# oraclefina/MSPI

Hardware: AMD Instinct MI355X
Metric: clips_per_sec (higher is better)
Workload: dtype f32 storage/accumulate; GEMMs as f16x3 split products on the f16 MFMA pipe; 1 GPU; x3dl motion encoder + ConvNeXt-T + ResNet18 audio + SyncBlock + decoder (AudioVisualSaliencyModel forward), batch 8/GPU, clips 3x16x224x224, spectrogram 1x257x300, inputs resident in HBM; global_batch=8, launch=hipGraph replay (mspi_amd.runtime.GraphPipeline), 2 batches in flight, stream_layout=2, parallelism=single GPU

## Files before the change

### mspi_amd/_lib.py

```python
import ctypes as C
import os

_HERE = os.path.dirname(os.path.abspath(__file__))
LIB_PATH = os.environ.get("MSPI_LIB_PATH") or os.path.join(_HERE, "csrc", "libmspi_hip.so")

ACT_NONE, ACT_RELU, ACT_GELU, ACT_SIGMOID, ACT_SWISH = range(5)
PREC_F32, PREC_F16X3 = 0, 1


class MspiError(RuntimeError):
    pass


class ConvDesc(C.Structure):
    _fields_ = [
        ("N", C.c_int32), ("T", C.c_int32), ("H", C.c_int32), ("W", C.c_int32), ("C", C.c_int32),
        ("sN", C.c_int64), ("sT", C.c_int64), ("sH", C.c_int64), ("sW", C.c_int64), ("sC", C.c_int64),
        ("kT", C.c_int32), ("kH", C.c_int32), ("kW", C.c_int32),
        ("strT", C.c_int32), ("strH", C.c_int32), ("strW", C.c_int32),
        ("padT", C.c_int32), ("padH", C.c_int32), ("padW", C.c_int32),
        ("To", C.c_int32), ("Ho", C.c_int32), ("Wo", C.c_int32),
        ("Cout", C.c_int32),
        ("ldy", C.c_int64), ("ldw", C.c_int64), ("ldr", C.c_int64),
        ("act", C.c_int32),
        ("prec", C.c_int32),
        ("w_scale", C.c_float),
        ("tile", C.c_int32),
        ("w_blocked", C.c_void_p),
    ]


class DwConvDesc(C.Structure):
    _fields_ = [
        ("N", C.c_int32), ("T", C.c_int32), ("H", C.c_int32), ("W", C.c_int32), ("C", C.c_int32),
        ("ldx", C.c_int64), ("ldy", C.c_int64),
        ("kT", C.c_int32), ("kH", C.c_int32), ("kW", C.c_int32),
        ("strT", C.c_int32), ("strH", C.c_int32), ("strW", C.c_int32),
        ("padT", C.c_int32), ("padH", C.c_int32), ("padW", C.c_int32),
        ("To", C.c_int32), ("Ho", C.c_int32), ("Wo", C.c_int32),
        ("act", C.c_int32),
    ]


class AttnDesc(C.Structure):
    _fields_ = [
        ("B", C.c_int32), ("Hh", C.c_int32), ("Nq", C.c_int32), ("Nk", C.c_int32), ("D", C.c_int32),
        ("Dv", C.c_int32), ("nmask", C.c_int32), ("nwin", C.c_int32),
        ("q_sB", C.c_int64), ("q_sH", C.c_int64), ("q_sT", C.c_int64),
        ("k_sB", C.c_int64), ("k_sH", C.c_int64), ("k_sT", C.c_int64),
        ("v_sB", C.c_int64), ("v_sH", C.c_int64), ("v_sT", C.c_int64),
        ("o_sB", C.c_int64), ("o_sH", C.c_int64), ("o_sT", C.c_int64),
        ("scale", C.c_float), ("prec", C.c_int32),
    ]


class MvitAugDesc(C.Structure):
    _fields_ = [
        ("B", C.c_int32), ("heads", C.c_int32), ("Dh", C.c_int32), ("DA", C.c_int32),
        ("qT", C.c_int32), ("qH", C.c_int32), ("qW", C.c_int32), ("kT", C.c_int32), ("kH", C.c_int32), ("kW", C.c_int32),
        ("ldq", C.c_int64), ("ldk", C.c_int64),
        ("scale", C.c_float),
    ]


class MlpDesc(C.Structure):
    _fields_ = [
        ("M", C.c_int64), ("C", C.c_int32), ("hidden", C.c_int32),
        ("ldx", C.c_int64), ("ldr", C.c_int64), ("ldy", C.c_int64),
        ("ln", C.c_int32), ("act", C.c_int32), ("eps", C.c_float),
        ("w1_scale", C.c_float), ("w2_scale", C.c_float),
    ]


class RowGemmDesc(C.Structure):
    _fields_ = [
        ("M", C.c_int64), ("K", C.c_int32), ("N", C.c_int32),
        ("ldx", C.c_int64), ("ldr", C.c_int64), ("ldy", C.c_int64), ("ldg", C.c_int64),
        ("act", C.c_int32), ("rows_per_sample", C.c_int32), ("w_scale", C.c_float),
    ]


class X3dCaDesc(C.Structure):
    _fields_ = [
        ("M", C.c_int64), ("D", C.c_int32), ("Cx", C.c_int32),
        ("ldu", C.c_int64), ("ldr", C.c_int64), ("ldy", C.c_int64), ("ldt", C.c_int64), ("ldg", C.c_int64),
        ("rows_per_sample", C.c_int32), ("wc_scale", C.c_float), ("wa_scale", C.c_float),
    ]


class X3dAbDesc(C.Structure):
    _fields_ = [
        ("N", C.c_int32), ("T", C.c_int32), ("H", C.c_int32), ("W", C.c_int32),
        ("Cin", C.c_int32), ("Cmid", C.c_int32),
        ("ldx", C.c_int64), ("ldu", C.c_int64),
        ("act", C.c_int32), ("wa_scale", C.c_float),
    ]


class X3dAbS2Desc(C.Structure):
    _fields_ = list(X3dAbDesc._fields_)


class X3dStemDesc(C.Structure):
    _fields_ = [
        ("N", C.c_int32), ("T", C.c_int32), ("H", C.c_int32), ("W", C.c_int32),
        ("sN", C.c_int64), ("sC", C.c_int64), ("sT", C.c_int64), ("sH", C.c_int64), ("sW", C.c_int64),
        ("ldy", C.c_int64),
    ]


class PermuteDesc(C.Structure):
    _fields_ = [("dims", C.c_int32 * 6), ("strides", C.c_int64 * 6), ("src_elems", C.c_int64)]


class JpegDesc(C.Structure):
    _fields_ = [
        ("B", C.c_int32), ("H", C.c_int32), ("W", C.c_int32), ("quality", C.c_int32),
        ("pitch", C.c_int64), ("map_stride", C.c_int64), ("file_stride", C.c_int64), ("cap", C.c_int64),
        ("div", C.c_uint16 * 64),
        ("header", C.c_void_p), ("header_len", C.c_int32),
    ]


class JpegDecTables(C.Structure):
    _fields_ = [
        ("scan_len", C.c_int32), ("reserved", C.c_int32),
        ("quant", (C.c_uint16 * 64) * 3),
        ("comp_dc", C.c_uint8 * 4), ("comp_ac", C.c_uint8 * 4),
        ("counts", (C.c_uint8 * 16) * 4),
        ("vals", (C.c_uint8 * 256) * 4),
    ]


class JpegDecInfo(C.Structure):
    _fields_ = [
        ("H", C.c_int32), ("W", C.c_int32), ("ncomp", C.c_int32), ("hs", C.c_int32), ("vs", C.c_int32),
        ("scan_off", C.c_int32), ("scan_len", C.c_int32), ("reserved", C.c_int32),
        ("tables", JpegDecTables),
    ]


class JpegDecDesc(C.Structure):
    _fields_ = [
        ("B", C.c_int32), ("H", C.c_int32), ("W", C.c_int32), ("ncomp", C.c_int32), ("hs", C.c_int32), ("vs", C.c_int32),
        ("S", C.c_int32), ("reserved", C.c_int32),
        ("scan_stride", C.c_int64), ("scan_cap", C.c_int64), ("pitch", C.c_int64), ("img_stride", C.c_int64),
    ]


_P = C.c_void_p
_SIGNATURES = {
    "mspi_version": (C.c_int, []),
    "mspi_last_error": (C.c_char_p, []),
    "mspi_device_count": (C.c_int, []),
    "mspi_set_status_word": (C.c_int, [_P]),
    "mspi_conv_splitk_ws_bytes": (C.c_size_t, [C.POINTER(ConvDesc), C.c_int32]),
    "mspi_conv_splitk_fwd": (C.c_int, [C.POINTER(ConvDesc), _P, _P, _P, _P, _P, _P, C.c_int32, _P]),
    "mspi_conv_fwd": (C.c_int, [C.POINTER(ConvDesc), _P, _P, _P, _P, _P, _P, _P]),
    "mspi_conv_variant": (C.c_int, [C.POINTER(ConvDesc), _P, _P, C.c_int32]),
    "mspi_conv_halo_fwd": (C.c_int, [C.POINTER(ConvDesc), _P, _P, _P, _P, _P, _P]),
    "mspi_conv_halo_supported": (C.c_int, [C.POINTER(ConvDesc)]),
    "mspi_conv_halo_variant": (C.c_int, [C.POINTER(ConvDesc), _P]),
    "mspi_dwconv_fwd": (C.c_int, [C.POINTER(DwConvDesc), _P, _P, _P, _P, _P, _P]),
    "mspi_dwconv_pool_rows": (C.c_int, [C.POINTER(DwConvDesc)]),
    "mspi_dwconv_variant": (C.c_int, [C.POINTER(DwConvDesc)]),
    "mspi_se_gate": (C.c_int, [_P, C.c_int32, C.c_float, _P, _P, _P, _P, _P, C.c_int32, C.c_int32, C.c_int32, _P]),
    "mspi_se_gate_variant": (C.c_int, [C.c_int32, C.c_int32]),
    "mspi_layernorm_variant": (C.c_int, [C.c_int32, C.c_int32]),
    "mspi_layernorm_fwd": (C.c_int, [_P, C.c_int64, C.c_int64, _P, C.c_int64, C.c_int64, _P, _P, C.c_float, C.c_int32,
                                      C.c_int32, C.c_int32, C.c_int32, _P, _P]),
    "mspi_attn_fwd": (C.c_int, [C.POINTER(AttnDesc), _P, _P, _P, _P, _P, _P, _P, _P, _P]),
    "mspi_attn_ws_bytes": (C.c_size_t, [C.POINTER(AttnDesc)]),
    "mspi_attn_fwd_ws": (C.c_int, [C.POINTER(AttnDesc), _P, _P, _P, _P, _P, _P, _P, _P, _P, _P]),
    "mspi_attn_variant": (C.c_int, [C.POINTER(AttnDesc), C.c_int32, C.c_int32, C.c_int32, C.c_int32]),
    "mspi_space_to_depth": (C.c_int, [_P, C.c_int64, _P, C.c_int64, C.c_int32, C.c_int32, C.c_int32, C.c_int32, _P]),
    "mspi_mvit_qk_augment": (C.c_int, [C.POINTER(MvitAugDesc), _P, _P, _P, _P, _P, _P, _P, _P]),
    "mspi_mvit_qk_augment_p": (C.c_int, [C.POINTER(MvitAugDesc), _P, _P, _P, C.c_int64, _P, _P, _P, _P, _P, _P]),
    "mspi_maxpool_fwd": (C.c_int, [C.POINTER(DwConvDesc), _P, _P, _P]),
    "mspi_upsample_fwd": (C.c_int, [_P, C.c_int64, _P, C.c_int64, C.c_int32, C.c_int32, C.c_int32, C.c_int32,
                                     C.c_int32, C.c_int32, C.c_int32, _P]),
    "mspi_upsample_sum_fwd": (C.c_int, [_P, _P, _P, C.c_int32, _P, C.c_int64, C.c_int32, C.c_int32, C.c_int32, C.c_int32,
                                         C.c_int32, C.c_int32, _P]),
    "mspi_rowgate": (C.c_int, [_P, C.c_int64, _P, C.c_int64, C.c_int32, _P]),
    "mspi_logsumexp_sub": (C.c_int, [_P, C.c_int32, C.c_int32, _P]),
    "mspi_mean_rows": (C.c_int, [_P, C.c_int64, C.c_int64, _P, C.c_int32, C.c_int32, C.c_int32, _P]),
    "mspi_mean_rows_slices": (C.c_int, [C.c_int32]),
    "mspi_mean_rows_ws": (C.c_int, [_P, C.c_int64, C.c_int64, _P, _P, C.c_int32, C.c_int32, C.c_int32, _P]),
    "mspi_neg_cosine": (C.c_int, [_P, _P, _P, C.c_int32, C.c_int32, C.c_float, C.c_int32, _P]),
    "mspi_add": (C.c_int, [_P, _P, _P, C.c_int64, _P]),
    "mspi_permute_fwd": (C.c_int, [C.POINTER(PermuteDesc), _P, _P, _P]),
    "mspi_permute_variant": (C.c_int, [C.POINTER(PermuteDesc), _P, _P]),
    "mspi_gated_sum_fwd": (C.c_int, [_P, _P, _P, _P, _P, C.c_int32, C.c_int64, C.c_int32, C.c_int32, _P]),
    "mspi_logspec_fwd": (C.c_int, [_P, C.c_int64, _P, _P, C.c_int32, _P, _P, C.c_int32, _P]),
    "mspi_resize_norm_fwd": (C.c_int, [_P, C.c_int32, C.c_int32, _P, _P, C.c_int64, C.c_int32, C.c_int32, _P, _P, C.c_int32,
                                        _P, _P, C.c_int32, _P, _P, _P]),
    "mspi_clip_resize_plan": (C.c_int, [_P, C.c_int32, C.c_int32, C.c_int32, C.c_int32, C.c_int32, _P]),
    "mspi_clip_resize_norm_fwd": (C.c_int, [_P, C.c_int32, C.c_int32, C.c_int32, _P, _P, _P, C.c_int32, C.c_int32, C.c_int64,
                                             C.c_int64, C.c_int64, C.c_int64, C.c_int32, C.c_int32, _P, _P, _P, C.c_int32, _P, _P,
                                             _P, C.c_int32, _P, _P, _P]),
    "mspi_layernorm_sp_fwd": (C.c_int, [_P, C.c_int64, C.c_int64, _P, C.c_int64, C.c_int64, _P, _P, C.c_float, C.c_int32,
                                         C.c_int32, C.c_int32, C.c_int32, _P]),
    "mspi_split_planes_fwd": (C.c_int, [_P, C.c_int64, C.c_int64, C.c_int32, _P, C.c_int64, C.c_int64, _P]),
    "mspi_join_planes_fwd": (C.c_int, [_P, C.c_int64, C.c_int64, C.c_int64, C.c_int32, _P, C.c_int64, _P]),
    "mspi_gemm_sp_fwd": (C.c_int, [C.POINTER(ConvDesc), _P, C.c_int64, C.c_int64, _P, _P, _P, _P, _P, C.c_int64, C.c_int64, _P]),
    "mspi_gemm_sp_variant": (C.c_int, [C.POINTER(ConvDesc), _P]),
    "mspi_saliency_metrics": (C.c_int, [_P, _P, _P, _P, C.c_int32, C.c_int32, C.c_int32, _P]),
    "mspi_saliency_auc_ws_bytes": (C.c_size_t, [C.c_int32, C.c_int32]),
    "mspi_saliency_auc_judd": (C.c_int, [_P, C.c_int32, _P, _P, _P, _P, C.c_int32, C.c_int32, _P]),
    "mspi_saliency_sauc_counts": (C.c_int, [_P, _P, _P, _P, C.c_int32, C.c_int32, C.c_int32, _P]),
    "mspi_saliency_ig": (C.c_int, [_P, _P, _P, _P, C.c_int32, C.c_int32, _P]),
    "mspi_saliency_loss_ws_bytes": (C.c_size_t, [C.c_int32, C.c_int32]),
    "mspi_saliency_loss_fwd": (C.c_int, [_P, _P, _P, _P, _P, C.c_int32, C.c_int32, _P]),
    "mspi_saliency_loss_bwd": (C.c_int, [_P, _P, _P, _P, _P, C.c_float, C.c_float, C.c_float, _P, C.c_int32, C.c_int32, _P]),
    "mspi_logsumexp_sub_bwd": (C.c_int, [_P, _P, _P, C.c_int32, C.c_int32, _P]),
    "mspi_conv_c1_bwd_ws_bytes": (C.c_size_t, [C.c_int32, C.c_int32, C.c_int32]),
    "mspi_conv_c1_bwd": (C.c_int, [_P, C.c_int64, _P, _P, _P, C.c_int64, _P, _P, _P, C.c_int32, C.c_int32, C.c_int32, C.c_int32, _P]),
    "mspi_conv_wgrad_supported": (C.c_int, [C.POINTER(ConvDesc)]),
    "mspi_conv_wgrad_ws_bytes": (C.c_size_t, [C.POINTER(ConvDesc)]),
    "mspi_conv_wgrad_variant": (C.c_int, [C.POINTER(ConvDesc), _P, _P]),
    "mspi_conv_wgrad_fwd": (C.c_int, [C.POINTER(ConvDesc), _P, _P, _P, _P, _P, _P]),
    "mspi_upsample_bwd": (C.c_int, [_P, C.c_int64, _P, C.c_int64, _P, C.c_int64, C.c_int32, C.c_int32, C.c_int32, C.c_int32,
                                     C.c_int32, C.c_int32, _P]),
    "mspi_conv_wgrad_wide_supported": (C.c_int, [C.POINTER(ConvDesc)]),
    "mspi_conv_wgrad_wide_ws_bytes": (C.c_size_t, [C.POINTER(ConvDesc)]),
    "mspi_conv_wgrad_wide_variant": (C.c_int, [C.POINTER(ConvDesc), _P, _P]),
    "mspi_conv_wgrad_wide_fwd": (C.c_int, [C.POINTER(ConvDesc), _P, _P, _P, _P, _P, _P]),
    "mspi_bn_ws_bytes": (C.c_size_t, [C.c_int64, C.c_int32]),
    "mspi_bn_stats": (C.c_int, [_P, C.c_int64, C.c_int64, C.c_int32, C.c_float, _P, _P, _P, _P, _P]),
    "mspi_bn_apply": (C.c_int, [_P, C.c_int64, _P, _P, _P, _P, _P, C.c_int64, C.c_int64, C.c_int32, C.c_int32, _P]),
    "mspi_bn_bwd": (C.c_int, [_P, C.c_int64, _P, C.c_int64, _P, C.c_int64, _P, _P, _P, _P, C.c_int64, _P, _P, _P, C.c_int64,
                              C.c_int32, _P]),
    "mspi_resize_bilinear_fwd": (C.c_int, [_P, C.c_int32, _P, C.c_int32, C.c_int32, C.c_int32, C.c_int32, C.c_int32, _P]),
    "mspi_resize_fixation_fwd": (C.c_int, [_P, _P, C.c_int32, C.c_int32, C.c_int32, C.c_int32, C.c_int32, _P]),
    "mspi_rowgemm_packed_bytes": (C.c_size_t, [C.c_int32, C.c_int32]),
    "mspi_rowgemm_supported": (C.c_int, [C.c_int32, C.c_int32]),
    "mspi_rowgemm_fwd": (C.c_int, [C.POINTER(RowGemmDesc), _P, _P, _P, _P, _P, _P, _P]),
    "mspi_rowgemm_variant": (C.c_int, [C.POINTER(RowGemmDesc), C.c_int32]),
    "mspi_x3d_ca_packed_bytes": (C.c_size_t, [C.c_int32, C.c_int32]),
    "mspi_x3d_ca_supported": (C.c_int, [C.c_int32, C.c_int32]),
    "mspi_x3d_ca_fwd": (C.c_int, [C.POINTER(X3dCaDesc), _P, _P, _P, _P, _P, _P, _P, _P, _P]),
    "mspi_x3d_ca_variant": (C.c_int, [C.POINTER(X3dCaDesc), C.c_int32]),
    "mspi_x3d_ab_supported": (C.c_int, [C.POINTER(X3dAbDesc)]),
    "mspi_x3d_ab_pool_rows": (C.c_int, [C.POINTER(X3dAbDesc)]),
    "mspi_x3d_ab_packed_bytes": (C.c_size_t, [C.c_int32, C.c_int32]),
    "mspi_x3d_ab_fwd": (C.c_int, [C.POINTER(X3dAbDesc), _P, _P, _P, _P, _P, _P, _P, _P]),
    "mspi_x3d_ab_variant": (C.c_int, [C.POINTER(X3dAbDesc)]),
    "mspi_x3d_ab_s2_supported": (C.c_int, [C.POINTER(X3dAbS2Desc)]),
    "mspi_x3d_ab_s2_pool_rows": (C.c_int, [C.POINTER(X3dAbS2Desc)]),
    "mspi_x3d_ab_s2_fwd": (C.c_int, [C.POINTER(X3dAbS2Desc), _P, _P, _P, _P, _P, _P, _P, _P]),
    "mspi_x3d_ab_s2_variant": (C.c_int, [C.POINTER(X3dAbS2Desc)]),
    "mspi_x3d_stem_supported": (C.c_int, [C.POINTER(X3dStemDesc)]),
    "mspi_x3d_stem_variant": (C.c_int, [C.POINTER(X3dStemDesc)]),
    "mspi_x3d_stem_fwd": (C.c_int, [C.POINTER(X3dStemDesc), _P, _P, _P, _P, _P, _P]),
    "mspi_mlp_packed_bytes": (C.c_size_t, [C.c_int32, C.c_int32]),
    "mspi_mlp_fwd": (C.c_int, [C.POINTER(MlpDesc), _P, _P, _P, _P, _P, _P, _P, _P, _P]),
    "mspi_mlp_variant": (C.c_int, [C.POINTER(MlpDesc)]),
    "mspi_postprocess_workspace": (C.c_size_t, [C.c_int32, C.c_int32, C.c_int32, C.c_int32, C.c_int32]),
    "mspi_postprocess_u8": (C.c_int, [_P, _P, _P, C.c_int32, C.c_int32, C.c_int32, C.c_int32, C.c_int32, _P]),
    "mspi_jpeg_gray_header": (C.c_int, [C.c_int32, C.c_int32, C.c_int32, _P, C.c_int64]),
    "mspi_jpeg_gray_bound": (C.c_size_t, [C.c_int32, C.c_int32]),
    "mspi_jpeg_gray_ws_bytes": (C.c_size_t, [C.c_int32, C.c_int32, C.c_int32]),
    "mspi_jpeg_gray_fwd": (C.c_int, [C.POINTER(JpegDesc), _P, _P, _P, _P, _P]),
    "mspi_jpeg_dec_parse": (C.c_int, [_P, C.c_int64, C.POINTER(JpegDecInfo)]),
    "mspi_jpeg_dec_ws_bytes": (C.c_size_t, [C.POINTER(JpegDecDesc)]),
    "mspi_jpeg_dec_fwd": (C.c_int, [C.POINTER(JpegDecDesc), _P, _P, _P, _P, _P, _P, _P]),
}

EXPORTS = tuple(_SIGNATURES)

_TRAIN_SIGNATURES = {
    "mspi_rowgate_bwd": (C.c_int, [_P, C.c_int64, _P, C.c_int64, _P, _P, C.c_int64, _P, C.c_int64, C.c_int32, _P]),
    "mspi_upsample_sum_bwd": (C.c_int, [_P, _P, _P, C.c_int32, _P, C.c_int64, C.c_int32, C.c_int32, C.c_int32, C.c_int32,
                                         C.c_int32, _P]),
}

TRAIN_EXPORTS = tuple(_TRAIN_SIGNATURES)

_BLOCK_SIGNATURES = {
    "mspi_gelu_bwd": (C.c_int, [_P, C.c_int64, _P, C.c_int64, _P, C.c_int64, _P, C.c_int64, C.c_int64, C.c_int32, _P]),
    "mspi_layernorm_bwd_ws_bytes": (C.c_size_t, [C.c_int64, C.c_int32]),
    "mspi_layernorm_bwd": (C.c_int, [_P, C.c_int64, _P, C.c_int64, _P, C.c_float, _P, C.c_int64, _P, _P, _P, C.c_int64, C.c_int32, _P]),
    "mspi_dwconv_wgrad_supported": (C.c_int, [C.POINTER(DwConvDesc)]),
    "mspi_dwconv_wgrad_ws_bytes": (C.c_size_t, [C.POINTER(DwConvDesc)]),
    "mspi_dwconv_wgrad": (C.c_int, [C.POINTER(DwConvDesc), _P, _P, _P, _P, _P, _P]),
}

BLOCK_EXPORTS = tuple(_BLOCK_SIGNATURES)

_ENTRY_SIGNATURES = {
    "mspi_conv_wgrad_entry_supported": (C.c_int, [C.POINTER(ConvDesc)]),
    "mspi_conv_wgrad_entry_ws_bytes": (C.c_size_t, [C.POINTER(ConvDesc)]),
    "mspi_conv_wgrad_entry_variant": (C.c_int, [C.POINTER(ConvDesc), _P, _P]),
    "mspi_conv_wgrad_entry": (C.c_int, [C.POINTER(ConvDesc), _P, _P, _P, _P, _P, _P]),
}

ENTRY_EXPORTS = tuple(_ENTRY_SIGNATURES)

_ADAPTER_SIGNATURES = {
    "mspi_conv_wgrad_t16_supported": (C.c_int, [C.POINTER(ConvDesc)]),
    "mspi_conv_wgrad_t16_ws_bytes": (C.c_size_t, [C.POINTER(ConvDesc)]),
    "mspi_conv_wgrad_t16_variant": (C.c_int, [C.POINTER(ConvDesc), _P, _P]),
    "mspi_conv_wgrad_t16": (C.c_int, [C.POINTER(ConvDesc), _P, _P, _P, _P, _P, _P]),
}

ADAPTER_EXPORTS = tuple(_ADAPTER_SIGNATURES)

_SYNC_SIGNATURES = {
    "mspi_attn_bwd_ws_bytes": (C.c_size_t, [C.POINTER(AttnDesc)]),
    "mspi_attn_bwd_variant": (C.c_int, [C.POINTER(AttnDesc)]),
    "mspi_attn_bwd": (C.c_int, [C.POINTER(AttnDesc), _P, _P, _P, _P, _P, _P, _P, _P, _P, _P]),
    "mspi_layernorm_bwd_wide_ws_bytes": (C.c_size_t, [C.c_int64, C.c_int32]),
    "mspi_layernorm_bwd_wide": (C.c_int, [_P, C.c_int64, _P, C.c_int64, _P, C.c_float, _P, C.c_int64, _P, _P, _P, C.c_int64, C.c_int32,
                                          _P]),
}

SYNC_EXPORTS = tuple(_SYNC_SIGNATURES)

_LINEAR_SIGNATURES = {
    "mspi_linear_wgrad_ws_bytes": (C.c_size_t, [C.c_int64, C.c_int32, C.c_int32]),
    "mspi_linear_wgrad_variant": (C.c_int, [_P, C.c_int64, _P, C.c_int64, C.c_int64, C.c_int32, C.c_int32]),
    "mspi_linear_wgrad": (C.c_int, [_P, C.c_int64, _P, C.c_int64, _P, _P, _P, C.c_int64, C.c_int32, C.c_int32, _P]),
}

LINEAR_EXPORTS = tuple(_LINEAR_SIGNATURES)

_CONTRAST_SIGNATURES = {
    "mspi_neg_cosine_bwd": (C.c_int, [_P, _P, _P, _P, C.c_int32, C.c_int32, C.c_float, _P]),
    "mspi_layernorm_act_bwd_ws_bytes": (C.c_size_t, [C.c_int64, C.c_int32]),
    "mspi_layernorm_act_bwd": (C.c_int, [_P, C.c_int64, _P, C.c_int64, _P, C.c_int64, _P, C.c_float, _P, C.c_int64, _P, _P, _P, C.c_int64,
                                         C.c_int32, _P]),
    "mspi_mean_rows_bwd": (C.c_int, [_P, _P, C.c_int64, C.c_int64, C.c_int32, C.c_int32, C.c_int32, C.c_int32, _P]),
}

CONTRAST_EXPORTS = tuple(_CONTRAST_SIGNATURES)

_X3D_SIGNATURES = {
    "mspi_dwconv3_wgrad_supported": (C.c_int, [C.POINTER(DwConvDesc)]),
    "mspi_dwconv3_wgrad_ws_bytes": (C.c_size_t, [C.POINTER(DwConvDesc)]),
    "mspi_dwconv3_wgrad": (C.c_int, [C.POINTER(DwConvDesc), _P, _P, _P, _P, _P, _P]),
    "mspi_bn_gate_act_fwd": (C.c_int, [_P, C.c_int64, _P, _P, _P, _P, _P, _P, C.c_int64, _P, C.c_int64, C.c_int64, C.c_int32, C.c_int32,
                                       C.c_int32, _P]),
    "mspi_gate_swish_bwd_ws_bytes": (C.c_size_t, [C.c_int32, C.c_int32, C.c_int32]),
    "mspi_gate_swish_bwd": (C.c_int, [_P, C.c_int64, _P, C.c_int64, _P, _P, _P, _P, _P, _P, C.c_int64, _P, _P, C.c_int32, C.c_int32,
                                      C.c_int32, _P]),
    "mspi_se_train_fwd": (C.c_int, [_P, _P, _P, _P, _P, _P, _P, _P, _P, _P, _P, _P, C.c_int32, C.c_int32, C.c_int32, _P]),
    "mspi_se_train_bwd_ws_bytes": (C.c_size_t, [C.c_int32, C.c_int32, C.c_int32]),
    "mspi_se_train_bwd": (C.c_int, [_P, _P, _P, _P, _P, _P, _P, _P, _P, _P, _P, _P, C.c_int32, C.c_int32, C.c_int32, _P]),
    "mspi_relu_mask_add": (C.c_int, [_P, C.c_int64, _P, C.c_int64, _P, C.c_int64, C.c_int64, C.c_int32, _P]),
}

X3D_EXPORTS = tuple(_X3D_SIGNATURES)

_lib = None


def load():
    global _lib
    if _lib is not None:
        return _lib
    if not os.path.exists(LIB_PATH):
        raise MspiError(
            "libmspi_hip.so not found at %s -- run `python -c 'import __graft_entry__ as g; g.build()'` "
            "(mspi_amd has no CPU fallback)" % LIB_PATH)
    import torch
    lib = C.CDLL(LIB_PATH)
    for name, (res, args) in list(_SIGNATURES.items()) + list(_TRAIN_SIGNATURES.items()) + list(_BLOCK_SIGNATURES.items()) + \
            list(_ENTRY_SIGNATURES.items()) + list(_ADAPTER_SIGNATURES.items()) + list(_SYNC_SIGNATURES.items()) + list(_LINEAR_SIGNATURES.items()) + \
            list(_CONTRAST_SIGNATURES.items()) + list(_X3D_SIGNATURES.items()):
        fn = getattr(lib, name)
        fn.restype = res
        fn.argtypes = args
    if lib.mspi_version() != 2:
        raise MspiError("libmspi_hip.so ABI version %d != 2" % lib.mspi_version())
    _lib = lib
    return lib


def check(rc, what):
    if rc != 0:
        msg = load().mspi_last_error().decode("utf-8", "replace")
        raise MspiError("%s failed (%d): %s" % (what, rc, msg))
```

### mspi_amd/backbones/convnext.py

```python
import torch
import torch.nn as nn

from .. import engine as E
from ..module import HipModule

DEPTHS = (3, 3, 9, 3)
DIMS = (96, 192, 384, 768)


class _Mlp(nn.Module):
    def __init__(self, dim):
        super().__init__()
        self.fc1 = nn.Linear(dim, 4 * dim)
        self.act = nn.GELU()
        self.fc2 = nn.Linear(4 * dim, dim)


class ConvNeXtBlock(HipModule):
    def __init__(self, dim, ls_init_value=1e-6):
        super().__init__()
        self.conv_dw = nn.Conv2d(dim, dim, 7, 1, 3, groups=dim)
        self.norm = nn.LayerNorm(dim, eps=1e-6)
        self.mlp = _Mlp(dim)
        self.gamma = nn.Parameter(ls_init_value * torch.ones(dim))

    def _pack(self):
        return {"dw": E.pack_dwconv(self.conv_dw.weight, self.conv_dw.bias, None, (1, 1, 1), (0, 3, 3)),
                "ln": (self.norm.weight.detach().float().contiguous(), self.norm.bias.detach().float().contiguous()),
                "mlp": E.pack_mlp_tail(self.mlp.fc1, self.mlp.fc2, out_scale=self.gamma)}

    def run(self, x):
        pk = self.pk
        return E.mlp_tail(E.dwconv(x, pk["dw"]), pk["mlp"], pk["ln"], 1e-6, res=x)


class ConvNeXtStage(HipModule):
    def __init__(self, dim_in, dim_out, depth, downsample):
        super().__init__()
        if downsample:
            self.downsample = nn.Sequential(nn.LayerNorm(dim_in, eps=1e-6), nn.Conv2d(dim_in, dim_out, 2, 2))
        else:
            self.downsample = nn.Identity()
        self.blocks = nn.Sequential(*[ConvNeXtBlock(dim_out) for _ in range(depth)])

    def _pack(self):
        if isinstance(self.downsample, nn.Identity):
            return None
        ln, cv = self.downsample[0], self.downsample[1]
        return (ln.weight.detach().float().contiguous(), ln.bias.detach().float().contiguous(),
                E.pack_conv(cv.weight, cv.bias, None, (1, 2, 2), (0, 0, 0)))

    def run(self, x):
        if self.pk is not None:
            g, b, cv = self.pk
            x = E.conv(E.layernorm(x, g, b, 1e-6), cv)
        for blk in self.blocks:
            x = blk.run(x)
        return x


class ConvNeXtTinyFeatures(HipModule):

    def __init__(self):
        super().__init__()
        self.stem_0 = nn.Conv2d(3, DIMS[0], 4, 4)
        self.stem_1 = nn.LayerNorm(DIMS[0], eps=1e-6)
        prev = DIMS[0]
        for i, (d, n) in enumerate(zip(DIMS, DEPTHS)):
            self.add_module("stages_%d" % i, ConvNeXtStage(prev, d, n, downsample=i > 0))
            prev = d
        for m in self.modules():
            if isinstance(m, (nn.Conv2d, nn.Linear)):
                nn.init.trunc_normal_(m.weight, std=0.02)
                nn.init.zeros_(m.bias)

    def _pack(self):
        return (E.pack_conv(self.stem_0.weight, self.stem_0.bias, None, (1, 4, 4), (0, 0, 0)),
                self.stem_1.weight.detach().float().contiguous(), self.stem_1.bias.detach().float().contiguous())

    @torch.no_grad()
    def forward_cl(self, clips):
        self._check_eval()
        stem, g, b = self.pk
        x = E.conv(clips, stem)
        x = x.reshape(x.N * x.T, 1, x.H, x.W)
        x = E.layernorm(x, g, b, 1e-6)
        outs = []
        for i in range(4):
            x = getattr(self, "stages_%d" % i).run(x)
            outs.append(x)
        return outs

    def forward(self, x):
        return [o.as_ncdhw().squeeze(2) for o in self.forward_cl(x)]
```

### mspi_amd/csrc/mlp_fused.hip

```cpp
#include "common.h"
#include <stdlib.h>
#include <type_traits>

namespace mspi {

typedef _Float16 v8h __attribute__((ext_vector_type(8)));
typedef float v16f __attribute__((ext_vector_type(16)));
typedef __attribute__((address_space(3))) void lds_void;

struct MlpArgs {
  const float* x; const float* gamma; const float* beta; const unsigned char* wp; const float* b1; const float* b2;
  const float* res; float* y;
  long M, ldx, ldr, ldy;
  int nch;
  int ln, act;
  float eps, inv_s1, inv_s2;
  int* status;
};

template <int C, int TM, int NS, int NWV = 4>
__global__ __launch_bounds__(64 * NWV, (C == 96 && TM == 1 && NWV == 4) ? 2 : 1) void mlp_fused_kernel(const MlpArgs p) {
  constexpr int KS = C / 16, CT = C / 32;
  constexpr int W1B = KS * 2048, W2B = 2 * CT * 2048, SB = W1B + W2B;
  constexpr int DPW = SB / (1024 * NWV);
  constexpr int BM = NWV * 32 * TM;
  static_assert(SB % (1024 * NWV) == 0, "a stage is dealt in whole 1-KB pieces to the waves");
  static_assert(C % 32 == 0 && SB % 4096 == 0, "C: multiple of 32");
  __shared__ __attribute__((aligned(16))) unsigned char smem[NS * SB + (C == 96 ? 2048 : 4096)];
  float* b1s = reinterpret_cast<float*>(smem + NS * SB);

  const int tid = threadIdx.x, lane = tid & 63, wave = tid >> 6;
  const int li = lane & 31, lh = lane >> 5;
  const long row0 = (long)blockIdx.x * BM + wave * (32 * TM);

  static_assert(W1B % (DPW * 1024) == 0, "the W1 / W2 boundary of a stage falls between waves");
  auto issue_stage = [&](int j) {
    const bool w1 = wave * DPW * 1024 < W1B;
    const int jc = w1 ? (j + 2 < p.nch ? j + 2 : 0) : j;
    const unsigned char* src = p.wp + (long)jc * SB + (wave * DPW) * 1024 + lane * 16;
    unsigned char* dst = smem + (j % NS) * SB + (wave * DPW) * 1024;
#pragma unroll
    for (int d = 0; d < DPW; ++d)
      __builtin_amdgcn_global_load_lds(reinterpret_cast<const float*>(src + d * 1024), (lds_void*)(dst + d * 1024), 16, 0, 0);
  };
  static_assert(W1B == W2B, "the prologue parks W1 of chunk 1 in a W2 half");
  constexpr int DP0 = W1B / (1024 * NWV);
  static_assert(W1B % (1024 * NWV) == 0, "W1 of a chunk is dealt in whole pieces");
  auto issue_w1_01 = [&]() {
#pragma unroll
    for (int c = 0; c < 2; ++c) {
      const int jc = c < p.nch ? c : 0;
#pragma unroll
      for (int d = 0; d < DP0; ++d)
        __builtin_amdgcn_global_load_lds(reinterpret_cast<const float*>(p.wp + (long)jc * SB + (wave * DP0 + d) * 1024 + lane * 16),
                                         (lds_void*)(smem + (NS - 1) * SB + c * W1B + (wave * DP0 + d) * 1024), 16, 0, 0);
    }
  };

  float xr[TM][KS][8];
#pragma unroll
  for (int t = 0; t < TM; ++t) {
    long row = row0 + t * 32 + li;
    if (row >= p.M) row = p.M - 1;
    const float* xp = p.x + row * p.ldx + 8 * lh;
#pragma unroll
    for (int ks = 0; ks < KS; ++ks) {
      const float4 a = *reinterpret_cast<const float4*>(xp + 16 * ks);
      const float4 b = *reinterpret_cast<const float4*>(xp + 16 * ks + 4);
      xr[t][ks][0] = a.x; xr[t][ks][1] = a.y; xr[t][ks][2] = a.z; xr[t][ks][3] = a.w;
      xr[t][ks][4] = b.x; xr[t][ks][5] = b.y; xr[t][ks][6] = b.z; xr[t][ks][7] = b.w;
    }
  }
  static_assert(NS >= 3, "the pipeline keeps stage j-1 in use while stage j is in flight and the prologue's slot is live");
  issue_w1_01();
  for (int j = 0; j < NS - 1; ++j) issue_stage(j < p.nch ? j : 0);
  for (int i = tid; i < p.nch * 32; i += 64 * NWV) b1s[i] = p.b1[i];

  if (p.ln) {
#pragma unroll
    for (int t = 0; t < TM; ++t) {
      float s = 0.f;
#pragma unroll
      for (int ks = 0; ks < KS; ++ks)
#pragma unroll
        for (int e = 0; e < 8; ++e) s += xr[t][ks][e];
      s += __shfl_xor(s, 32, 64);
      const float mean = s / (float)C;
      float q = 0.f;
#pragma unroll
      for (int ks = 0; ks < KS; ++ks)
#pragma unroll
        for (int e = 0; e < 8; ++e) { const float d = xr[t][ks][e] - mean; q = fmaf(d, d, q); }
      q += __shfl_xor(q, 32, 64);
      const float rstd = rsqrtf(q / (float)C + p.eps);
#pragma unroll
      for (int ks = 0; ks < KS; ++ks)
#pragma unroll
        for (int e = 0; e < 8; ++e) xr[t][ks][e] = (xr[t][ks][e] - mean) * rstd;
    }
#pragma unroll
    for (int ks = 0; ks < KS; ++ks) {
      const float4 g0 = *reinterpret_cast<const float4*>(p.gamma + 16 * ks + 8 * lh);
      const float4 g1 = *reinterpret_cast<const float4*>(p.gamma + 16 * ks + 8 * lh + 4);
      const float4 c0 = *reinterpret_cast<const float4*>(p.beta + 16 * ks + 8 * lh);
      const float4 c1 = *reinterpret_cast<const float4*>(p.beta + 16 * ks + 8 * lh + 4);
      const float g8[8] = {g0.x, g0.y, g0.z, g0.w, g1.x, g1.y, g1.z, g1.w};
      const float c8[8] = {c0.x, c0.y, c0.z, c0.w, c1.x, c1.y, c1.z, c1.w};
#pragma unroll
      for (int t = 0; t < TM; ++t)
#pragma unroll
        for (int e = 0; e < 8; ++e) xr[t][ks][e] = fmaf(xr[t][ks][e], g8[e], c8[e]);
    }
  }
  v8h xh[TM][KS], xl[TM][KS];
#pragma unroll
  for (int t = 0; t < TM; ++t)
#pragma unroll
    for (int ks = 0; ks < KS; ++ks)
#pragma unroll
      for (int e = 0; e < 8; ++e) {
        _Float16 h, l;
        split_f16(xr[t][ks][e], h, l);
        xh[t][ks][e] = h; xl[t][ks][e] = l;
      }

  v16f o[TM][CT];
#pragma unroll
  for (int t = 0; t < TM; ++t)
#pragma unroll
    for (int ct = 0; ct < CT; ++ct)
#pragma unroll
      for (int i = 0; i < 16; ++i) o[t][ct][i] = 0.f;

  auto phase1 = [&](const unsigned char* w1, v16f (&h)[TM]) {
#pragma unroll
    for (int t = 0; t < TM; ++t)
#pragma unroll
      for (int i = 0; i < 16; ++i) h[t][i] = 0.f;
#pragma unroll
    for (int ks = 0; ks < KS; ++ks) {
      const v8h wh = *reinterpret_cast<const v8h*>(w1 + (ks * 2 + 0) * 1024);
      const v8h wl = *reinterpret_cast<const v8h*>(w1 + (ks * 2 + 1) * 1024);
#pragma unroll
      for (int t = 0; t < TM; ++t) {
        if (!kSingleProduct) {
          h[t] = __builtin_amdgcn_mfma_f32_32x32x16_f16(wl, xh[t][ks], h[t], 0, 0, 0);
          h[t] = __builtin_amdgcn_mfma_f32_32x32x16_f16(wh, xl[t][ks], h[t], 0, 0, 0);
        }
        h[t] = __builtin_amdgcn_mfma_f32_32x32x16_f16(wh, xh[t][ks], h[t], 0, 0, 0);
      }
    }
  };
  v16f h[TM], hn[TM];
  v8h hh[TM][2], hl[TM][2], gh[TM][2], gl[TM][2];
  auto body = [&](auto has_p2, auto has_p1, int j, const unsigned char* st) {
    constexpr bool P2 = decltype(has_p2)::value, P1 = decltype(has_p1)::value;
    constexpr int T0 = P2 ? 0 : 2 * CT, T1 = P1 ? 2 * CT + KS : 2 * CT, NTR = T1 - T0;
    auto frag = [&](int tr, int plane) {
      const unsigned char* base = tr < 2 * CT ? st + W1B + (tr * 2) * 1024 : st + ((tr - 2 * CT) * 2) * 1024;
      return *reinterpret_cast<const v8h*>(base + plane * 1024);
    };
    float bv[16];
#pragma unroll
    for (int q = 0; q < 4; ++q) {
      const float4 b = *reinterpret_cast<const float4*>(b1s + j * 32 + q * 8 + 4 * lh);
      bv[q * 4 + 0] = b.x; bv[q * 4 + 1] = b.y; bv[q * 4 + 2] = b.z; bv[q * 4 + 3] = b.w;
    }
    v8h wh, wl, nh, nl;
    if (NTR > 0) { wh = frag(T0, 0); wl = frag(T0, 1); }
#pragma unroll
    for (int g = 0; g < 16; ++g) {
#pragma unroll
      for (int tr = T0 + g * NTR / 16; tr < T0 + (g + 1) * NTR / 16; ++tr) {
        if (tr + 1 < T1) { nh = frag(tr + 1, 0); nl = frag(tr + 1, 1); }
        __builtin_amdgcn_sched_barrier(0);
#pragma unroll
        for (int t = 0; t < TM; ++t) {
          if (tr < 2 * CT) {
            const int s = tr / CT, ct = tr % CT;
            if (!kSingleProduct) {
              o[t][ct] = __builtin_amdgcn_mfma_f32_32x32x16_f16(wl, hh[t][s], o[t][ct], 0, 0, 0);
              o[t][ct] = __builtin_amdgcn_mfma_f32_32x32x16_f16(wh, hl[t][s], o[t][ct], 0, 0, 0);
            }
            o[t][ct] = __builtin_amdgcn_mfma_f32_32x32x16_f16(wh, hh[t][s], o[t][ct], 0, 0, 0);
          } else {
            const int ks = tr - 2 * CT;
            const v16f zero = {0.f, 0.f, 0.f, 0.f, 0.f, 0.f, 0.f, 0.f, 0.f, 0.f, 0.f, 0.f, 0.f, 0.f, 0.f, 0.f};
            if (!kSingleProduct) {
              hn[t] = __builtin_amdgcn_mfma_f32_32x32x16_f16(wl, xh[t][ks], ks == 0 ? zero : hn[t], 0, 0, 0);
              hn[t] = __builtin_amdgcn_mfma_f32_32x32x16_f16(wh, xl[t][ks], hn[t], 0, 0, 0);
              hn[t] = __builtin_amdgcn_mfma_f32_32x32x16_f16(wh, xh[t][ks], hn[t], 0, 0, 0);
            } else {
              hn[t] = __builtin_amdgcn_mfma_f32_32x32x16_f16(wh, xh[t][ks], ks == 0 ? zero : hn[t], 0, 0, 0);
            }
          }
        }
        wh = nh; wl = nl;
      }
#pragma unroll
      for (int t = 0; t < TM; ++t) {
        const float u = fmaf(h[t][g], p.inv_s1, bv[g]);
        const float v = gelu_erf(u);
        _Float16 f, l;
        split_f16(v, f, l);
        gh[t][g >> 3][g & 7] = f;
        gl[t][g >> 3][g & 7] = l;
      }
      __builtin_amdgcn_sched_barrier(0);
    }
#pragma unroll
    for (int t = 0; t < TM; ++t) {
      if (P1) h[t] = hn[t];
#pragma unroll
      for (int s = 0; s < 2; ++s) { hh[t][s] = gh[t][s]; hl[t][s] = gl[t][s]; }
    }
  };
  using yes = std::true_type;
  using no = std::false_type;

  asm volatile("s_waitcnt vmcnt(%0)" ::"n"((NS - 1) * DPW) : "memory");
  asm volatile("s_waitcnt lgkmcnt(0)" ::: "memory");
  __builtin_amdgcn_s_barrier();
  phase1(smem + (NS - 1) * SB + lane * 16, h);
  if (p.nch > 1) body(no(), yes(), 0, smem + (NS - 1) * SB + W1B + lane * 16);
  else body(no(), no(), 0, smem + lane * 16);

  auto top = [&](int j) {
    if (j + NS - 3 < p.nch) asm volatile("s_waitcnt vmcnt(%0)" ::"n"((NS - 2) * DPW) : "memory");
    else asm volatile("s_waitcnt vmcnt(0)" ::: "memory");
    asm volatile("s_waitcnt lgkmcnt(0)" ::: "memory");
    __builtin_amdgcn_s_barrier();
    if (j + NS - 2 < p.nch) issue_stage(j + NS - 2);
  };
  int j = 1;
  for (; j + 1 < p.nch; ++j) {
    top(j);
    body(yes(), yes(), j, smem + ((j - 1) % NS) * SB + lane * 16);
  }
  if (j < p.nch) {
    top(j);
    body(yes(), no(), j, smem + ((j - 1) % NS) * SB + lane * 16);
    ++j;
  }
  top(j);
  {
    const unsigned char* w2 = smem + ((j - 1) % NS) * SB + lane * 16 + W1B;
#pragma unroll
    for (int s = 0; s < 2; ++s)
#pragma unroll
      for (int ct = 0; ct < CT; ++ct) {
        const v8h wh = *reinterpret_cast<const v8h*>(w2 + ((s * CT + ct) * 2 + 0) * 1024);
        const v8h wl = *reinterpret_cast<const v8h*>(w2 + ((s * CT + ct) * 2 + 1) * 1024);
#pragma unroll
        for (int t = 0; t < TM; ++t) {
          if (!kSingleProduct) {
            o[t][ct] = __builtin_amdgcn_mfma_f32_32x32x16_f16(wl, hh[t][s], o[t][ct], 0, 0, 0);
            o[t][ct] = __builtin_amdgcn_mfma_f32_32x32x16_f16(wh, hl[t][s], o[t][ct], 0, 0, 0);
          }
          o[t][ct] = __builtin_amdgcn_mfma_f32_32x32x16_f16(wh, hh[t][s], o[t][ct], 0, 0, 0);
        }
      }
  }

  bool bad = false;
#pragma unroll
  for (int t = 0; t < TM; ++t) {
    const long row = row0 + t * 32 + li;
    const bool ok = row < p.M;
    const long rr = ok ? row : 0;
#pragma unroll
    for (int ct = 0; ct < CT; ++ct) {
      float4 rv[4];
#pragma unroll
      for (int q = 0; q < 4; ++q) {
        const int c = ct * 32 + q * 8 + 4 * lh;
        rv[q] = p.res ? *reinterpret_cast<const float4*>(p.res + rr * p.ldr + c) : make_float4(0.f, 0.f, 0.f, 0.f);
      }
#pragma unroll
      for (int q = 0; q < 4; ++q) {
        const int c = ct * 32 + q * 8 + 4 * lh;
        const float4 b = *reinterpret_cast<const float4*>(p.b2 + c);
        float4 v;
        v.x = fmaf(o[t][ct][q * 4 + 0], p.inv_s2, b.x) + rv[q].x;
        v.y = fmaf(o[t][ct][q * 4 + 1], p.inv_s2, b.y) + rv[q].y;
        v.z = fmaf(o[t][ct][q * 4 + 2], p.inv_s2, b.z) + rv[q].z;
        v.w = fmaf(o[t][ct][q * 4 + 3], p.inv_s2, b.w) + rv[q].w;
        bad |= nonfinite(v.x) | nonfinite(v.y) | nonfinite(v.z) | nonfinite(v.w);
        if (ok) *reinterpret_cast<float4*>(p.y + row * p.ldy + c) = v;
      }
    }
  }
  report_nonfinite(p.status, bad);
}

template <int C, int TM, int NS, int NWV = 4>
static int launch_mlp(const MlpArgs& a, hipStream_t s) {
  constexpr int BM = 32 * NWV * TM;
  const long nb = (a.M + BM - 1) / BM;
  hipLaunchKernelGGL((mlp_fused_kernel<C, TM, NS, NWV>), dim3((unsigned)nb), dim3(64 * NWV), 0, s, a);
  return 0;
}

}

using namespace mspi;

extern "C" size_t mspi_mlp_packed_bytes(int C, int hidden) {
  return (size_t)(hidden / 32) * ((size_t)(C / 16) * 2048 + 2 * (size_t)(C / 32) * 2048);
}

static int mlp_select(const MspiMlpDesc* d, bool ln_params) {
  MSPI_REQUIRE(d->C == 96 || d->C == 192, "mspi_mlp_fwd: C = %d not supported (96, 192)", d->C);
  MSPI_REQUIRE(d->hidden % 32 == 0 && d->hidden >= 32 && d->hidden <= 1024, "mspi_mlp_fwd: hidden = %d", d->hidden);
  MSPI_REQUIRE(d->M >= 1 && d->M < (1L << 31), "mspi_mlp_fwd: M = %ld", (long)d->M);
  MSPI_REQUIRE(d->ldx >= d->C && d->ldy >= d->C && d->ldx % 4 == 0 && d->ldy % 4 == 0,
               "mspi_mlp_fwd: row strides must be >= C and multiples of 4 floats");
  MSPI_REQUIRE(d->act == MSPI_ACT_GELU, "mspi_mlp_fwd: only MSPI_ACT_GELU between the layers (act = %d)", d->act);
  MSPI_REQUIRE(!d->ln || ln_params, "mspi_mlp_fwd: LayerNorm needs gamma and beta");
  MSPI_REQUIRE(d->w1_scale > 0.f && d->w2_scale > 0.f, "mspi_mlp_fwd: weight scales must be positive");
  MSPI_REQUIRE(d->C != 96 || d->hidden <= 512, "mspi_mlp_fwd: hidden = %d > 512 with C = 96", d->hidden);
  static const int variant = getenv("MSPI_MLP_TM") ? atoi(getenv("MSPI_MLP_TM")) : 0;
  if (d->C == 96) return variant == 2 ? 96244 : 96134;
  return (variant == 8 || (variant != 4 && d->M >= 256L * 256)) ? 192138 : 192134;
}

extern "C" int mspi_mlp_variant(const MspiMlpDesc* d) {
  MSPI_REQUIRE(d, "mspi_mlp_variant: null descriptor");
  return mlp_select(d, true);
}

extern "C" int mspi_mlp_fwd(const MspiMlpDesc* d, const void* x, const void* gamma, const void* beta, const void* w_packed,
                            const void* b1, const void* b2, const void* res, void* y, void* stream) {
  MSPI_REQUIRE(d && x && w_packed && b1 && b2 && y, "mspi_mlp_fwd: null argument");
  const int variant = mlp_select(d, gamma && beta);
  if (variant < 0) return variant;
  MSPI_REQUIRE(!res || (d->ldr >= d->C && d->ldr % 4 == 0), "mspi_mlp_fwd: row strides must be >= C and multiples of 4 floats");
  MlpArgs a;
  a.x = (const float*)x; a.gamma = (const float*)gamma; a.beta = (const float*)beta; a.wp = (const unsigned char*)w_packed;
  a.b1 = (const float*)b1; a.b2 = (const float*)b2; a.res = (const float*)res; a.y = (float*)y;
  a.M = d->M; a.ldx = d->ldx; a.ldr = d->ldr; a.ldy = d->ldy;
  a.nch = d->hidden / 32; a.ln = d->ln; a.act = d->act; a.eps = d->eps;
  a.inv_s1 = 1.0f / d->w1_scale; a.inv_s2 = 1.0f / d->w2_scale;
  a.status = g_status_word;
  hipStream_t s = (hipStream_t)stream;
  switch (variant) {
    case 96244: launch_mlp<96, 2, 4>(a, s); break;
    case 96134: launch_mlp<96, 1, 3>(a, s); break;
    case 192138: launch_mlp<192, 1, 3, 8>(a, s); break;
    default: launch_mlp<192, 1, 3>(a, s); break;
  }
  return check_launch("mspi_mlp_fwd");
}

namespace mspi {

struct RowGemmArgs {
  const float* x; const unsigned char* wp; const float* bias; const float* res; const float* gate; float* y;
  long M, ldx, ldr, ldy, ldg;
  int K, N;
  int nch;
  int cps;
  int act;
  float inv_s;
  int rows_per_sample;
  int* status;
};

constexpr int RG_LDS = 64 * 1024;

template <int KSB, bool GATE>
__global__ __launch_bounds__(256, 2) void rowgemm_kernel(const RowGemmArgs p) {
  constexpr int SB = KSB * 2048;
  extern __shared__ __attribute__((aligned(16))) unsigned char rg_smem[];
  const int j0 = blockIdx.y * p.cps;
  const int nj = min(p.cps, p.nch - j0);
  float* bs = reinterpret_cast<float*>(rg_smem + (size_t)p.cps * SB);
  const int tid = threadIdx.x, lane = tid & 63, wave = tid >> 6;
  const int li = lane & 31, lh = lane >> 5;
  const long row = (long)blockIdx.x * 128 + wave * 32 + li;
  const bool rok = row < p.M;
  const long rr = rok ? row : p.M - 1;

  const int pieces = nj * (SB / 1024);
  for (int i = wave; i < pieces; i += 4)
    __builtin_amdgcn_global_load_lds(reinterpret_cast<const float*>(p.wp + (long)j0 * SB + (long)i * 1024 + lane * 16),
                                     (lds_void*)(rg_smem + (long)i * 1024), 16, 0, 0);
  float xr[KSB][8];
  const float* xp = p.x + rr * p.ldx + 8 * lh;
#pragma unroll
  for (int ks = 0; ks < KSB; ++ks) {
    const int k = 16 * ks + 8 * lh;
    const bool k0 = k < p.K, k1 = k + 4 < p.K;
    const float4 a = *reinterpret_cast<const float4*>(xp + (k0 ? 16 * ks : -8 * lh));
    const float4 b = *reinterpret_cast<const float4*>(xp + (k1 ? 16 * ks + 4 : -8 * lh));
    xr[ks][0] = k0 ? a.x : 0.f; xr[ks][1] = k0 ? a.y : 0.f; xr[ks][2] = k0 ? a.z : 0.f; xr[ks][3] = k0 ? a.w : 0.f;
    xr[ks][4] = k1 ? b.x : 0.f; xr[ks][5] = k1 ? b.y : 0.f; xr[ks][6] = k1 ? b.z : 0.f; xr[ks][7] = k1 ? b.w : 0.f;
  }
  if (GATE) {
    const float* gp = p.gate + (long)((unsigned)rr / (unsigned)p.rows_per_sample) * p.ldg + 8 * lh;
#pragma unroll
    for (int ks = 0; ks < KSB; ++ks) {
      const int k = 16 * ks + 8 * lh;
      const bool k0 = k < p.K, k1 = k + 4 < p.K;
      const float4 a = *reinterpret_cast<const float4*>(gp + (k0 ? 16 * ks : -8 * lh));
      const float4 b = *reinterpret_cast<const float4*>(gp + (k1 ? 16 * ks + 4 : -8 * lh));
      const float g8[8] = {a.x, a.y, a.z, a.w, b.x, b.y, b.z, b.w};
#pragma unroll
      for (int e = 0; e < 8; ++e) {
        const float v = xr[ks][e] * g8[e];
        xr[ks][e] = fast_swish(v);
      }
    }
  }
  for (int i = tid; i < nj * 32; i += 256) bs[i] = (p.bias && j0 * 32 + i < p.N) ? p.bias[j0 * 32 + i] : 0.f;
  v8h xh[KSB], xl[KSB];
#pragma unroll
  for (int ks = 0; ks < KSB; ++ks)
#pragma unroll
    for (int e = 0; e < 8; ++e) {
      _Float16 h, l;
      split_f16(xr[ks][e], h, l);
      xh[ks][e] = h; xl[ks][e] = l;
    }
  asm volatile("s_waitcnt vmcnt(0)" ::: "memory");
  __syncthreads();

  bool bad = false;
  for (int jl = 0; jl < nj; ++jl) {
    const int j = j0 + jl;
    const unsigned char* st = rg_smem + (long)jl * SB + lane * 16;
    v16f h;
#pragma unroll
    for (int i = 0; i < 16; ++i) h[i] = 0.f;
#pragma unroll
    for (int ks = 0; ks < KSB; ++ks) {
      const v8h wh = *reinterpret_cast<const v8h*>(st + (ks * 2 + 0) * 1024);
      const v8h wl = *reinterpret_cast<const v8h*>(st + (ks * 2 + 1) * 1024);
      if (!kSingleProduct) {
        h = __builtin_amdgcn_mfma_f32_32x32x16_f16(wl, xh[ks], h, 0, 0, 0);
        h = __builtin_amdgcn_mfma_f32_32x32x16_f16(wh, xl[ks], h, 0, 0, 0);
      }
      h = __builtin_amdgcn_mfma_f32_32x32x16_f16(wh, xh[ks], h, 0, 0, 0);
    }
    float4 rv[4];
#pragma unroll
    for (int q = 0; q < 4; ++q) {
      const int c = j * 32 + q * 8 + 4 * lh;
      rv[q] = (p.res && c < p.N) ? *reinterpret_cast<const float4*>(p.res + rr * p.ldr + c) : make_float4(0.f, 0.f, 0.f, 0.f);
    }
#pragma unroll
    for (int q = 0; q < 4; ++q) {
      const int c = j * 32 + q * 8 + 4 * lh;
      const float4 b = *reinterpret_cast<const float4*>(bs + c - j0 * 32);
      float4 v;
      v.x = fmaf(h[q * 4 + 0], p.inv_s, b.x) + rv[q].x;
      v.y = fmaf(h[q * 4 + 1], p.inv_s, b.y) + rv[q].y;
      v.z = fmaf(h[q * 4 + 2], p.inv_s, b.z) + rv[q].z;
      v.w = fmaf(h[q * 4 + 3], p.inv_s, b.w) + rv[q].w;
      bad |= nonfinite(v.x) | nonfinite(v.y) | nonfinite(v.z) | nonfinite(v.w);
      if (p.act == MSPI_ACT_RELU) {
        v.x = fmaxf(v.x, 0.f); v.y = fmaxf(v.y, 0.f); v.z = fmaxf(v.z, 0.f); v.w = fmaxf(v.w, 0.f);
      } else if (p.act != MSPI_ACT_NONE) {
        v.x = act_apply(v.x, p.act); v.y = act_apply(v.y, p.act); v.z = act_apply(v.z, p.act); v.w = act_apply(v.w, p.act);
      }
      if (rok && c < p.N) *reinterpret_cast<float4*>(p.y + row * p.ldy + c) = v;
    }
  }
  report_nonfinite(p.status, bad);
}

template <int KSB>
static int launch_rowgemm(const RowGemmArgs& a, size_t lds, hipStream_t s) {
  const dim3 grid((unsigned)((a.M + 127) / 128), (unsigned)((a.nch + a.cps - 1) / a.cps));
  if (a.gate) hipLaunchKernelGGL((rowgemm_kernel<KSB, true>), grid, dim3(256), lds, s, a);
  else hipLaunchKernelGGL((rowgemm_kernel<KSB, false>), grid, dim3(256), lds, s, a);
  return 0;
}

}

static int rowgemm_ksb(int K) { return K <= 32 ? 2 : K <= 64 ? 4 : K <= 128 ? 8 : K <= 224 ? 14 : 0; }

extern "C" size_t mspi_rowgemm_packed_bytes(int32_t K, int32_t N) {
  const int ksb = rowgemm_ksb(K);
  return ksb ? (size_t)((N + 31) / 32) * ksb * 2048 : 0;
}

static int rowgemm_cps(long M, int nch, int ksb) {
  const long row_tiles = (M + 127) / 128;
  int split = 1;
  if (row_tiles < 512) split = (int)((512 + row_tiles - 1) / row_tiles);
  if (split > nch) split = nch;
  int cps = (nch + split - 1) / split;
  const int cap = RG_LDS / (ksb * 2048 + 128);
  if (cps > cap) cps = cap;
  return cps < 1 ? 1 : cps;
}

extern "C" int mspi_rowgemm_supported(int32_t K, int32_t N) {
  return rowgemm_ksb(K) != 0 && N >= 4 && N <= 1024;
}

static int rowgemm_select(const MspiRowGemmDesc* d, bool gate) {
  MSPI_REQUIRE(d->M >= 1 && d->M < (1L << 31) && d->K >= 4 && d->N >= 4 && d->K % 4 == 0 && d->N % 4 == 0,
               "mspi_rowgemm_fwd: M = %ld, K = %d, N = %d (K, N: storage columns, multiples of 4)", (long)d->M, d->K, d->N);
  MSPI_REQUIRE(mspi_rowgemm_supported(d->K, d->N), "mspi_rowgemm_fwd: K = %d / N = %d outside the thin-GEMM range", d->K, d->N);
  MSPI_REQUIRE(d->ldx >= d->K && d->ldy >= d->N && d->ldx % 4 == 0 && d->ldy % 4 == 0,
               "mspi_rowgemm_fwd: row strides must cover the row and be multiples of 4 floats");
  MSPI_REQUIRE(!gate || (d->rows_per_sample > 0 && d->ldg >= d->K && d->ldg % 4 == 0), "mspi_rowgemm_fwd: gate needs rows_per_sample and ldg");
  MSPI_REQUIRE(d->w_scale > 0.f, "mspi_rowgemm_fwd: w_scale must be positive");
  return rowgemm_ksb(d->K) * 10 + (gate ? 1 : 0);
}

extern "C" int mspi_rowgemm_variant(const MspiRowGemmDesc* d, int32_t has_gate) {
  MSPI_REQUIRE(d, "mspi_rowgemm_variant: null descriptor");
  return rowgemm_select(d, has_gate != 0);
}

extern "C" int mspi_rowgemm_fwd(const MspiRowGemmDesc* d, const void* x, const void* w_packed, const void* bias, const void* res,
                                const void* gate, void* y, void* stream) {
  MSPI_REQUIRE(d && x && w_packed && y, "mspi_rowgemm_fwd: null argument");
  const int variant = rowgemm_select(d, gate != nullptr);
  if (variant < 0) return variant;
  MSPI_REQUIRE(!res || (d->ldr >= d->N && d->ldr % 4 == 0), "mspi_rowgemm_fwd: row strides must cover the row and be multiples of 4 floats");
  RowGemmArgs a;
  a.x = (const float*)x; a.wp = (const unsigned char*)w_packed; a.bias = (const float*)bias; a.res = (const float*)res;
  a.gate = (const float*)gate; a.y = (float*)y;
  a.M = d->M; a.ldx = d->ldx; a.ldr = d->ldr; a.ldy = d->ldy; a.ldg = d->ldg;
  a.K = d->K; a.N = d->N; a.nch = (d->N + 31) / 32; a.act = d->act; a.inv_s = 1.0f / d->w_scale;
  a.rows_per_sample = d->rows_per_sample;
  a.status = g_status_word;
  const int ksb = variant / 10;
  a.cps = rowgemm_cps(d->M, a.nch, ksb);
  const size_t lds = (size_t)a.cps * (ksb * 2048 + 128);
  int rc;
  switch (ksb) {
    case 2: rc = launch_rowgemm<2>(a, lds, (hipStream_t)stream); break;
    case 4: rc = launch_rowgemm<4>(a, lds, (hipStream_t)stream); break;
    case 8: rc = launch_rowgemm<8>(a, lds, (hipStream_t)stream); break;
    default: rc = launch_rowgemm<14>(a, lds, (hipStream_t)stream); break;
  }
  MSPI_REQUIRE(rc == 0, "mspi_rowgemm_fwd: could not reserve %zu bytes of LDS", lds);
  return check_launch("mspi_rowgemm_fwd");
}

namespace mspi {

struct CaArgs {
  const float* u; const float* gate; const unsigned char* wp; const float* b1; const float* b2; const float* res;
  float* y; float* t;
  long M, ldu, ldg, ldr, ldy, ldt;
  int D, Cx;
  int nch;
  int rows_per_sample;
  float inv_s1, inv_s2;
  int* status;
};

template <int C, bool GATE>
__global__ __launch_bounds__(256, 1) void x3d_ca_kernel(const CaArgs p) {
  constexpr int NS = 2;
  constexpr int KS = C / 16, CT = C / 32;
  constexpr int W1B = KS * 2048, W2B = 2 * CT * 2048, SB = W1B + W2B;
  constexpr int DPW = SB / 4096;
  static_assert(C % 32 == 0 && SB % 4096 == 0, "C: multiple of 32");
  __shared__ __attribute__((aligned(16))) unsigned char smem[NS * SB + 1024];
  float* b1s = reinterpret_cast<float*>(smem + NS * SB);

  const int tid = threadIdx.x, lane = tid & 63, wave = tid >> 6;
  const int li = lane & 31, lh = lane >> 5;
  const long row = (long)blockIdx.x * 128 + wave * 32 + li;
  const bool rok = row < p.M;
  const long rr = rok ? row : p.M - 1;

  auto issue_stage = [&](int j) {
    const unsigned char* src = p.wp + (long)j * SB + (wave * DPW) * 1024 + lane * 16;
    unsigned char* dst = smem + (j % NS) * SB + (wave * DPW) * 1024;
#pragma unroll
    for (int d = 0; d < DPW; ++d)
      __builtin_amdgcn_global_load_lds(reinterpret_cast<const float*>(src + d * 1024), (lds_void*)(dst + d * 1024), 16, 0, 0);
  };
  for (int j = 0; j < NS - 1 && j < p.nch; ++j) issue_stage(j);

  float xr[KS][8];
  const float* xp = p.u + rr * p.ldu + 8 * lh;
#pragma unroll
  for (int ks = 0; ks < KS; ++ks) {
    const int k = 16 * ks + 8 * lh;
    const bool k0 = k < p.D, k1 = k + 4 < p.D;
    const float4 a = *reinterpret_cast<const float4*>(xp + (k0 ? 16 * ks : -8 * lh));
    const float4 b = *reinterpret_cast<const float4*>(xp + (k1 ? 16 * ks + 4 : -8 * lh));
    xr[ks][0] = k0 ? a.x : 0.f; xr[ks][1] = k0 ? a.y : 0.f; xr[ks][2] = k0 ? a.z : 0.f; xr[ks][3] = k0 ? a.w : 0.f;
    xr[ks][4] = k1 ? b.x : 0.f; xr[ks][5] = k1 ? b.y : 0.f; xr[ks][6] = k1 ? b.z : 0.f; xr[ks][7] = k1 ? b.w : 0.f;
  }
  if (GATE) {
    const float* gp = p.gate + (long)((unsigned)rr / (unsigned)p.rows_per_sample) * p.ldg + 8 * lh;
#pragma unroll
    for (int ks = 0; ks < KS; ++ks) {
      const int k = 16 * ks + 8 * lh;
      const bool k0 = k < p.D, k1 = k + 4 < p.D;
      const float4 a = *reinterpret_cast<const float4*>(gp + (k0 ? 16 * ks : -8 * lh));
      const float4 b = *reinterpret_cast<const float4*>(gp + (k1 ? 16 * ks + 4 : -8 * lh));
      const float g8[8] = {a.x, a.y, a.z, a.w, b.x, b.y, b.z, b.w};
#pragma unroll
      for (int e = 0; e < 8; ++e) {
        const float v = xr[ks][e] * g8[e];
        xr[ks][e] = fast_swish(v);
      }
    }
  }
  for (int i = tid; i < p.nch * 32; i += 256) b1s[i] = i < p.Cx ? p.b1[i] : 0.f;
  v8h xh[KS], xl[KS];
#pragma unroll
  for (int ks = 0; ks < KS; ++ks)
#pragma unroll
    for (int e = 0; e < 8; ++e) {
      _Float16 h, l;
      split_f16(xr[ks][e], h, l);
      xh[ks][e] = h; xl[ks][e] = l;
    }

  v16f o[CT];
#pragma unroll
  for (int ct = 0; ct < CT; ++ct)
#pragma unroll
    for (int i = 0; i < 16; ++i) o[ct][i] = 0.f;

  bool bad = false;
  for (int j = 0; j < p.nch; ++j) {
    asm volatile("s_waitcnt vmcnt(0)" ::: "memory");
    asm volatile("s_waitcnt lgkmcnt(0)" ::: "memory");
    __builtin_amdgcn_s_barrier();
    if (j + NS - 1 < p.nch) issue_stage(j + NS - 1);
    float4 rv[4];
#pragma unroll
    for (int q = 0; q < 4; ++q) {
      const int c = j * 32 + q * 8 + 4 * lh;
      rv[q] = c < p.Cx ? *reinterpret_cast<const float4*>(p.res + rr * p.ldr + c) : make_float4(0.f, 0.f, 0.f, 0.f);
    }

// ... 122 lines not shown
```

### mspi_amd/engine.py

```python
import ctypes as C
import os as _os
from functools import partial

import numpy as np
import torch

from . import _lib
from ._lib import (ACT_GELU, ACT_NONE, ACT_RELU, ACT_SIGMOID, ACT_SWISH, PREC_F16X3, PREC_F32, AttnDesc, ConvDesc,
                   DwConvDesc, MspiError, MvitAugDesc, check)
from .packs import (DEFAULT_PREC, SP_ENABLED, PackedConv, PackedDw, PackedMlp, PackedX3dAb, PackedX3dCa, PackedX3dStem,
                    _pack_rowgemm, _pad_vec, fold_bn, mlp_supported, pack_conv, pack_dwconv, pack_mlp, pack_mlp_tail,
                    pack_x3d_ab, pack_x3d_ab_s2, pack_x3d_ca, pack_x3d_stem, rowgemm_ksb, rowgemm_supported, rup4,
                    sp_supported, sp_weights, x3d_ca_supported)

__all__ = ["CL", "SP", "alloc", "alloc_sp", "pack_conv", "pack_dwconv", "PackedConv", "PackedDw", "conv", "dwconv", "maxpool",
           "layernorm", "attention", "upsample", "upsample_sum", "rowgate", "logsumexp_sub", "mean_rows", "neg_cosine", "se_gate",
           "add", "fold_bn", "conv_wgrad", "conv_c1_bwd", "upsample_bwd", "logsumexp_sub_bwd", "conv_wgrad_wide",
           "conv_wgrad_wide_variant", "bn_stats", "bn_apply", "bn_bwd", "rowgate_bwd", "upsample_sum_bwd", "gelu_bwd",
           "layernorm_bwd", "dwconv_wgrad", "conv_wgrad_entry", "conv_wgrad_entry_variant", "conv_wgrad_t16",
           "conv_wgrad_t16_variant", "attention_bwd", "layernorm_bwd_wide", "linear_wgrad",
           "linear_wgrad_variant", "neg_cosine_bwd", "layernorm_act_bwd", "mean_rows_bwd", "dwconv3_wgrad", "bn_gate_act",
           "gate_swish_bwd", "se_train_fwd", "se_train_bwd", "relu_mask_add", "ACT_NONE", "ACT_RELU", "ACT_GELU", "ACT_SIGMOID", "ACT_SWISH"]


AUTOTUNE = {"on": _os.environ.get("MSPI_AUTOTUNE", "0") == "1", "cache": {}, "reps": 3}


def autotune(on=True):
    AUTOTUNE["on"] = bool(on)


def save_autotune(path):
    import json
    with open(path, "w") as f:
        json.dump({repr(k): v for k, v in AUTOTUNE["cache"].items()}, f, indent=0, sort_keys=True)


def load_autotune(path):
    import ast
    import json
    with open(path) as f:
        AUTOTUNE["cache"].update({ast.literal_eval(k): int(v) for k, v in json.load(f).items()})
    return len(AUTOTUNE["cache"])


THIN = 100
SPLITK = 200
SPLITK_ENABLED = _os.environ.get("MSPI_SPLITK", "1") != "0"
HALO = 300
HALO_ENABLED = _os.environ.get("MSPI_CONV_HALO", "1") != "0"
THIN_DEFAULT = True
THIN_ENABLED = _os.environ.get("MSPI_THIN", "1") != "0"


_TUNE_LOG = _os.environ.get("MSPI_TUNE_LOG") == "1"


def _tune_conv(launch, key, candidates):
    best, best_t, times = -1, float("inf"), []
    e0, e1 = torch.cuda.Event(enable_timing=True), torch.cuda.Event(enable_timing=True)
    for tile in candidates:
        if launch(tile) != 0:
            continue
        e0.record()
        for _ in range(AUTOTUNE["reps"]):
            launch(tile)
        e1.record()
        e1.synchronize()
        t = e0.elapsed_time(e1)
        times.append((tile, t / AUTOTUNE["reps"]))
        if t < best_t:
            best, best_t = tile, t
    AUTOTUNE["cache"][key] = best
    if _TUNE_LOG:
        import sys
        print("[tune] %s -> %d  %s" % (key, best, " ".join("%d:%.4f" % tt for tt in times)), file=sys.stderr)
    return best


def _choose(key, tile, default, candidates, launch, *call):
    if tile is not None:
        return tile
    choice = AUTOTUNE["cache"].get(key)
    if choice is None and AUTOTUNE["on"] and not torch.cuda.is_current_stream_capturing():
        return _tune_conv(launch, key, candidates(*call))
    return default if choice is None else choice


class Profiler:
    active = None

    def __init__(self):
        self.records = []

    def __enter__(self):
        Profiler.active = self
        return self

    def __exit__(self, *a):
        Profiler.active = None

    def summary(self):
        out = {}
        for name, fl, by, e0, e1, _ in self.records:
            d = out.setdefault(name, {"calls": 0, "ms": 0.0, "flops": 0.0, "bytes": 0.0})
            d["calls"] += 1
            d["ms"] += e0.elapsed_time(e1)
            d["flops"] += fl
            d["bytes"] += by
        return out


class _Timed:
    __slots__ = ("name", "flops", "bytes", "e0", "detail")

    def __init__(self, name, flops=0.0, nbytes=0.0, detail=""):
        self.name, self.flops, self.bytes, self.detail = name, flops, nbytes, detail

    def __enter__(self):
        if Profiler.active is not None:
            self.e0 = torch.cuda.Event(enable_timing=True)
            self.e0.record()
        return self

    def __exit__(self, *a):
        p = Profiler.active
        if p is not None:
            e1 = torch.cuda.Event(enable_timing=True)
            e1.record()
            p.records.append((self.name, self.flops, self.bytes, self.e0, e1, self.detail))


def _stream():
    return C.c_void_p(torch.cuda.current_stream().cuda_stream)


def _need_gpu(t):
    if not t.is_cuda:
        raise MspiError("mspi_amd runs on the GPU only (tensor on %s); there is no CPU fallback" % t.device)
    cur = torch.cuda.current_device()
    if t.device.index != cur:
        raise MspiError("tensor on %s, but the current device is cuda:%d: the launch would go to the wrong device's stream; "
                        "call under torch.cuda.device(%d)" % (t.device, cur, t.device.index))
    if _STATUS["word"] is None:
        _register_status_word()


_STATUS = {"word": None}
RANGE_CHECK = {"on": _os.environ.get("MSPI_RANGE_CHECK", "1") != "0", "lo": 2.0 ** -5, "hi": 2.0 ** 15, "moved": []}


def _register_status_word():
    w = torch.zeros(1, dtype=torch.int32).pin_memory()
    check(_lib.load().mspi_set_status_word(w.data_ptr()), "mspi_set_status_word")
    _STATUS["word"] = w


def range_flag(reset=True):
    w = _STATUS["word"]
    if w is None:
        return False
    bad = bool(int(w[0]))
    if bad and reset:
        w[0] = 0
    return bad


def check_range(sync=True):
    if sync and torch.cuda.is_available():
        torch.cuda.synchronize()
    if range_flag():
        raise MspiError("a GEMM or attention produced inf/NaN: an activation left the f16x3 range (|x| >= 65504; attention: "
                        "|q| >= 1023, |k|, |v| >= 4094) or the input was not finite; "
                        "let the first forward see representative data (engine.autotune(True): out-of-range layers move to the "
                        "fp32 path) or run with MSPI_GEMM_PREC=f32")


def _range_check(pk, amax_fn, what):
    if pk.checked:
        return
    pk.checked = True
    amax = float(amax_fn())
    if not (amax == amax) or amax >= RANGE_CHECK["hi"] or 0.0 < amax < RANGE_CHECK["lo"]:
        pk.w, pk.ldw, pk.prec, pk.thin, pk.w_scale = pk.w32, pk.ldw32, PREC_F32, None, 1.0
        RANGE_CHECK["moved"].append((what, amax))


class CL:
    __slots__ = ("buf", "off", "N", "T", "H", "W", "C", "ld", "sN")

    def __init__(self, buf, off, N, T, H, W, Cc, ld, sN=None):
        self.buf, self.off, self.N, self.T, self.H, self.W, self.C, self.ld = buf, off, N, T, H, W, Cc, ld
        self.sN = T * H * W * ld if sN is None else sN

    @property
    def dense(self):
        return self.sN == self.T * self.H * self.W * self.ld

    @property
    def Cs(self):
        return rup4(self.C) if self.C > 1 else 1

    @property
    def M(self):
        return self.N * self.T * self.H * self.W

    @property
    def ptr(self):
        return self.buf.data_ptr() + 4 * self.off

    def slice(self, c0, c):
        assert c0 % 4 == 0 and c0 + c <= self.ld
        return CL(self.buf, self.off + c0, self.N, self.T, self.H, self.W, c, self.ld, self.sN)

    def reshape(self, N, T, H, W):
        assert N * T * H * W == self.M and self.dense
        return CL(self.buf, self.off, N, T, H, W, self.C, self.ld)

    def tokens(self, r0, T, H, W):
        assert r0 + T * H * W <= self.T * self.H * self.W
        return CL(self.buf, self.off + r0 * self.ld, self.N, T, H, W, self.C, self.ld, self.sN)

    def as_ncdhw(self, channels=None):
        c = self.C if channels is None else channels
        ld, T, H, W = self.ld, self.T, self.H, self.W
        return self.buf.as_strided((self.N, c, T, H, W), (self.sN, 1, H * W * ld, W * ld, ld),
                                   self.buf.storage_offset() + self.off)

    def as_nthwc(self):
        ld, H, W = self.ld, self.H, self.W
        return self.buf.as_strided((self.N, self.T, H, W, self.C), (self.sN, H * W * ld, W * ld, ld, 1),
                                   self.buf.storage_offset() + self.off)

    def as_rows(self, channels=None):
        c = self.C if channels is None else channels
        assert self.dense
        return self.buf.as_strided((self.M, c), (self.ld, 1), self.buf.storage_offset() + self.off)


def alloc(N, T, H, W, Cc, device, ld=None):
    if ld is None:
        ld = rup4(Cc) if Cc > 1 else 1
    buf = torch.empty(N * T * H * W * ld, dtype=torch.float32, device=device)
    return CL(buf, 0, N, T, H, W, Cc, ld)


class SP:
    __slots__ = ("buf", "N", "T", "H", "W", "C", "ld")

    def __init__(self, buf, N, T, H, W, Cc, ld):
        self.buf, self.N, self.T, self.H, self.W, self.C, self.ld = buf, N, T, H, W, Cc, ld

    @property
    def M(self):
        return self.N * self.T * self.H * self.W

    @property
    def plane(self):
        return (self.M + 15) // 16 * 16 * self.ld

    @property
    def ptr(self):
        return self.buf.data_ptr()


def alloc_sp(N, T, H, W, Cc, device):
    assert Cc % 32 == 0
    m = N * T * H * W
    mp = (m + 15) // 16 * 16
    buf = torch.empty(2 * mp * Cc, dtype=torch.float16, device=device)
    if mp != m:
        buf.view(2, mp * Cc)[:, (mp - 16) * Cc:].zero_()
    return SP(buf, N, T, H, W, Cc, Cc)


def join_planes(sp):
    out = alloc(sp.N, sp.T, sp.H, sp.W, sp.C, sp.buf.device)
    check(_lib.load().mspi_join_planes_fwd(sp.ptr, sp.ld, sp.plane, sp.M, sp.C, out.ptr, out.ld, _stream()), "mspi_join_planes_fwd")
    return out


def from_rows(t2d):
    assert t2d.dim() == 2 and t2d.stride(1) == 1 and t2d.stride(0) % 4 == 0
    return CL(t2d, 0, t2d.shape[0], 1, 1, 1, t2d.shape[1], t2d.stride(0))


def _tuning():
    return AUTOTUNE["on"] and RANGE_CHECK["on"] and DEFAULT_PREC == PREC_F16X3 and not torch.cuda.is_current_stream_capturing()


def range_check_input(pk, x):
    if _tuning() and pk.prec == PREC_F16X3:
        _range_check(pk, lambda: (x.as_rows()[:, : x.C] if x.dense else x.buf).abs().max(), "conv %s %d -> %d" % (pk.k, pk.cin, pk.cout))
    return pk.prec == PREC_F16X3


def _x3d_ab_desc(x, pk, out_ld, act, cls=_lib.X3dAbDesc):
    d = cls()
    d.N, d.T, d.H, d.W = x.N, x.T, x.H, x.W
    d.Cin, d.Cmid, d.ldx, d.ldu, d.act, d.wa_scale = pk.cin_s, pk.cmid_s, x.ld, out_ld, act, pk.wa_scale
    return d


_x3d_ab_s2_desc = partial(_x3d_ab_desc, cls=_lib.X3dAbS2Desc)


def x3d_ab_supported(x, pk):
    return pk is not None and x.dense and x.Cs == pk.cin_s and bool(_lib.load().mspi_x3d_ab_supported(C.byref(_x3d_ab_desc(x, pk, pk.cmid_s, ACT_NONE))))


def x3d_ab_s2_supported(x, pk):
    return pk is not None and x.dense and x.Cs == pk.cin_s and bool(_lib.load().mspi_x3d_ab_s2_supported(C.byref(_x3d_ab_s2_desc(x, pk, pk.cmid_s, ACT_NONE))))


_AB = (1, _lib.X3dAbDesc, "x3d_ab", "x3d_ab_pool", "mspi_x3d_ab_fwd")
_AB_S2 = (2, _lib.X3dAbS2Desc, "x3d_ab_s2", "x3d_ab_s2_pool", "mspi_x3d_ab_s2_fwd")


def _x3d_ab(rec, fwd, pool_rows, x, pk, pool, out):
    s, desc, name, pooled, entry = rec
    _need_gpu(x.buf)
    if out is None:
        out = alloc(x.N, x.T, x.H // s, x.W // s, pk.cmid, x.buf.device)
    elif (out.N, out.T, out.H, out.W, out.Cs) != (x.N, x.T, x.H // s, x.W // s, pk.cmid_s) or not out.dense:
        raise MspiError("%s: the output tensor does not match the layer" % name)
# ... 163 lines not shown
    return cands


def conv(x, pk, out=None, res=None, gate=None, act=None, tile=None, sp_out=False):
    lib = _lib.load()
    tuning = AUTOTUNE["on"] and RANGE_CHECK["on"] and pk.prec == PREC_F16X3 and not torch.cuda.is_current_stream_capturing()
    if isinstance(x, SP):
        if tuning:
            _range_check(pk, lambda: x.buf[: x.plane].abs().max(), "planes -> %dx%d" % (pk.cin, pk.cout))
        if pk.prec == PREC_F16X3:
            return _conv_sp(x, pk, out, res, act, tile, sp_out)
        x, sp_out = join_planes(x), False
    if tuning:
        _range_check(pk, (lambda: (x.as_rows()[:, : x.C] if x.dense else x.buf).abs().max()) if isinstance(x, CL) else (lambda: x.abs().max()),
                     "conv %s %d -> %d" % (pk.k, pk.cin, pk.cout))
    if sp_out:
        raise MspiError("conv: split-plane output needs a split-plane input (mspi_gemm_sp_fwd)")
    d = ConvDesc()
    if isinstance(x, CL):
        _need_gpu(x.buf)
        N, T, H, W, Cin = x.N, x.T, x.H, x.W, x.Cs
        d.sN, d.sT, d.sH, d.sW, d.sC = x.sN, H * W * x.ld, W * x.ld, x.ld, 1
        xptr, dev = x.ptr, x.buf.device
    else:
        _need_gpu(x)
        if x.dim() == 4:
            x = x[:, :, None]
        if x.dtype != torch.float32:
            raise MspiError("conv: input must be fp32")
        N, Cin, T, H, W = x.shape
        sN, sC, sT, sH, sW = x.stride()
        d.sN, d.sT, d.sH, d.sW, d.sC = sN, sT, sH, sW, sC
        xptr, dev = x.data_ptr(), x.device
    if Cin != pk.cin_s:
        raise MspiError("conv: input has %d stored channels, weights were packed for %d" % (Cin, pk.cin_s))
    if pk.w.device != dev:
        raise MspiError("conv: packed weights live on %s, the input on %s" % (pk.w.device, dev))
    To, Ho, Wo = _out_extent(T, H, W, pk.k, pk.stride, pk.pad)
    if out is None:
        out = alloc(N, To, Ho, Wo, pk.cout, dev)
    if (out.N, out.T, out.H, out.W) != (N, To, Ho, Wo) or out.Cs != pk.cout_s or not out.dense:
        raise MspiError("conv: output CL %s does not match %s" % ((out.N, out.T, out.H, out.W, out.C), (N, To, Ho, Wo, pk.cout)))
    d.N, d.T, d.H, d.W, d.C = N, T, H, W, Cin
    d.kT, d.kH, d.kW = pk.k
    d.strT, d.strH, d.strW = pk.stride
    d.padT, d.padH, d.padW = pk.pad
    d.To, d.Ho, d.Wo = To, Ho, Wo
    d.Cout = pk.cout_s
    d.ldy, d.ldw = out.ld, pk.ldw
    d.ldr = res.ld if res is not None else 0
    d.act = pk.act if act is None else act
    d.prec, d.w_scale = pk.prec, pk.w_scale
    d.w_blocked = sp_weights(pk).data_ptr() if (pk.prec == PREC_F16X3 and W_BLOCKED) else None
    if res is not None and (res.M != out.M or not res.dense):
        raise MspiError("conv: residual rows %d != output rows %d (or residual not dense)" % (res.M, out.M))
    M = N * To * Ho * Wo
    taps = pk.k[0] * pk.k[1] * pk.k[2]
    tm = _Timed("conv_gemm", 2.0 * M * taps * pk.cin * pk.cout,
                4.0 * (N * T * H * W * pk.cin + M * pk.cout * (2 if res is not None else 1) + pk.cout * taps * pk.cin),
                "M=%d K=%d(%dx%d) N=%d s=%s%s%s" % (M, taps * pk.cin, taps, pk.cin, pk.cout, pk.stride,
                                                  " +res" if res is not None else "", " +gate" if gate is not None else ""))
    args = (xptr, pk.w.data_ptr(), pk.bias.data_ptr() if pk.bias is not None else None,
            res.ptr if res is not None else None, gate.data_ptr() if gate is not None else None, out.ptr, _stream())
    rg = None
    if THIN_ENABLED and pk.thin is not None and isinstance(x, CL) and x.dense:
        rg = _lib.RowGemmDesc()
        rg.M, rg.K, rg.N = M, pk.cin_s, pk.cout_s
        rg.ldx, rg.ldy, rg.ldr, rg.ldg = x.ld, out.ld, d.ldr, pk.cin_s
        rg.act, rg.rows_per_sample, rg.w_scale = d.act, To * Ho * Wo, pk.w_scale
        rg_args = (xptr, pk.thin.data_ptr(), args[2], args[3], args[4], out.ptr, args[6])

    halo = bool(HALO_ENABLED and gate is None and d.w_blocked and pk.k[1:] == (3, 3) and xptr % 16 == 0 and
                lib.mspi_conv_halo_supported(C.byref(d)))

    def launch(t):
        if t == THIN:
            return lib.mspi_rowgemm_fwd(C.byref(rg), *rg_args)
        if t == HALO:
            return lib.mspi_conv_halo_fwd(C.byref(d), args[0], args[2], args[3], None, out.ptr, args[6])
        if t >= SPLITK:
            S = t - SPLITK
            ws = torch.empty(S * M * pk.cout_s, dtype=torch.float32, device=dev)
            d.tile = 3
            return lib.mspi_conv_splitk_fwd(C.byref(d), args[0], args[1], args[2], args[3], args[5], ws.data_ptr(), S, args[6])
        d.tile = t
        return lib.mspi_conv_fwd(C.byref(d), *args)

    key = (M, taps * pk.cin_s, pk.cout_s, pk.k, pk.stride, pk.prec, d.sC == 1, res is not None, gate is not None, rg is not None, halo)
    choice = _choose(key, tile, None, _conv_kernels, launch, pk, d, M, rg, halo, gate)
    if choice is None:
        choice = THIN if rg is not None and THIN_DEFAULT else -1
    if choice == THIN and rg is None:
        raise MspiError("conv: the thin-GEMM kernel does not cover this call")
    if choice == HALO and not halo:
        raise MspiError("conv: the halo-staged kernel does not cover this call")
    with tm:
        check(launch(choice), "mspi_rowgemm_fwd" if choice == THIN else "mspi_conv_halo_fwd" if choice == HALO else
              "mspi_conv_splitk_fwd" if choice >= SPLITK else "mspi_conv_fwd")
        if Profiler.active is not None:
            if choice == THIN:
                tm.name = "rowgemm<%d,f16x3>" % rowgemm_ksb(pk.cin_s)
            elif choice == HALO:
                v = lib.mspi_conv_halo_variant(C.byref(d), xptr)
                tm.name = "conv_halo<%d,%d,f16x3>" % (v // 1000, v % 1000)
            elif choice >= SPLITK:
                tm.name = "conv_gemm<64,64,splitk%d>" % (choice - SPLITK)
            else:
                tm.name = gemm_kernel_name(lib.mspi_conv_variant(C.byref(d), xptr, args[4], 1))
    return out


def _dw_desc(x, k, s, p, out_ld):
    d = DwConvDesc()
    assert x.dense
    d.N, d.T, d.H, d.W, d.C = x.N, x.T, x.H, x.W, x.Cs
    d.ldx, d.ldy = x.ld, out_ld
    d.kT, d.kH, d.kW = k
    d.strT, d.strH, d.strW = s
    d.padT, d.padH, d.padW = p
    d.To, d.Ho, d.Wo = _out_extent(x.T, x.H, x.W, k, s, p)
    return d


def dwconv_variant(x, pk):
    return _lib.load().mspi_dwconv_variant(C.byref(_dw_desc(x, pk.k, pk.stride, pk.pad, x.ld)))


def dwconv(x, pk, out=None, pool=False, act=None):
    lib = _lib.load()
    _need_gpu(x.buf)
    if x.Cs != pk.c_s:
        raise MspiError("dwconv: input has %d channels, weights packed for %d" % (x.C, pk.c_s))
    if pk.w.device != x.buf.device:
        raise MspiError("dwconv: packed weights live on %s, the input on %s" % (pk.w.device, x.buf.device))
    To, Ho, Wo = _out_extent(x.T, x.H, x.W, pk.k, pk.stride, pk.pad)
    if out is None:
        out = alloc(x.N, To, Ho, Wo, x.C, x.buf.device)
    d = _dw_desc(x, pk.k, pk.stride, pk.pad, out.ld)
    d.act = pk.act if act is None else act
    part = None
    if pool:
        rows = lib.mspi_dwconv_pool_rows(C.byref(d))
        if rows <= 0:
            raise MspiError("dwconv: squeeze-excite pooling is not supported for kernel %s stride %s" % (pk.k, pk.stride))
        part = torch.empty(x.N, rows, pk.c_s, dtype=torch.float32, device=x.buf.device)
    taps = pk.k[0] * pk.k[1] * pk.k[2]
    with _Timed("dwconv_pool" if pool else "dwconv", 2.0 * out.M * taps * pk.c, 4.0 * (x.M + out.M) * pk.c,
                "in=%s C=%d k=%s s=%s" % ((x.N, x.T, x.H, x.W), pk.c, pk.k, pk.stride)):
        check(lib.mspi_dwconv_fwd(C.byref(d), x.ptr, pk.w.data_ptr(), pk.bias.data_ptr(), out.ptr,
                                  part.data_ptr() if pool else None, _stream()), "mspi_dwconv_fwd")
    return (out, part) if pool else out


def maxpool(x, k, s, p, out=None):
    lib = _lib.load()
    _need_gpu(x.buf)
    To, Ho, Wo = _out_extent(x.T, x.H, x.W, k, s, p)
    if out is None:
        out = alloc(x.N, To, Ho, Wo, x.C, x.buf.device)
    d = _dw_desc(x, k, s, p, out.ld)
    d.act = ACT_NONE
    with _Timed("maxpool", 0.0, 4.0 * (x.M + x.N * To * Ho * Wo) * x.C):
        check(lib.mspi_maxpool_fwd(C.byref(d), x.ptr, out.ptr, _stream()), "mspi_maxpool_fwd")
    return out


def se_gate(pool, inv_count, w1, b1, w2, b2, gate=None):
    lib = _lib.load()
    N, rows, Cc = pool.shape
    if gate is None:
        gate = torch.empty(N, Cc, dtype=torch.float32, device=pool.device)
    check(lib.mspi_se_gate(pool.data_ptr(), rows, float(inv_count), w1.data_ptr(), b1.data_ptr(), w2.data_ptr(),
                           b2.data_ptr(), gate.data_ptr(), N, Cc, w1.shape[0], _stream()), "mspi_se_gate")
    return gate


def layernorm(x, gamma, beta, eps, out=None, act=ACT_NONE, table=None, sp=False):
    lib = _lib.load()
    _need_gpu(x.buf)
    if sp:
        assert out is None and table is None and x.C % 32 == 0
        o = alloc_sp(x.N, x.T, x.H, x.W, x.C, x.buf.device)
        with _Timed("layernorm", 8.0 * x.M * x.C, 8.0 * x.M * x.C, "M=%d C=%d ->planes" % (x.M, x.C)):
            check(lib.mspi_layernorm_sp_fwd(x.ptr, x.ld, x.sN, o.ptr, o.ld, o.plane, gamma.data_ptr(), beta.data_ptr(), float(eps),
                                            x.N, x.T * x.H * x.W, x.C, act, _stream()), "mspi_layernorm_sp_fwd")
        return o
    if out is None:
        out = alloc(x.N, x.T, x.H, x.W, x.C, x.buf.device)
    R = x.T * x.H * x.W
    assert out.N == x.N and out.T * out.H * out.W == R and out.C == x.C
    P = 0 if table is None else table.shape[0]
    assert table is None or P == R
    with _Timed("layernorm", 8.0 * x.M * x.C, 8.0 * x.M * x.C, "M=%d C=%d" % (x.M, x.C)):
        check(lib.mspi_layernorm_fwd(x.ptr, x.ld, x.sN, out.ptr, out.ld, out.sN, gamma.data_ptr(), beta.data_ptr(),
                                     float(eps), x.N, R, x.C, act, table.data_ptr() if table is not None else None,
                                     _stream()), "mspi_layernorm_fwd")
    return out


def attention(qkv, B, Ntok, heads, hd, scale, out=None, biasT=None, maskT=None, tok_idx=None, rows_per_sample=None, slot=None):
    lib = _lib.load()
    _need_gpu(qkv.buf)
    Cc = heads * hd
    assert qkv.C == 3 * Cc and qkv.dense and (rows_per_sample is not None or qkv.M == B * Ntok)
    if out is None:
        out = alloc(qkv.N, qkv.T, qkv.H, qkv.W, Cc, qkv.buf.device)
    d = AttnDesc()
    d.B, d.Hh, d.Nq, d.Nk, d.D, d.Dv = B, heads, Ntok, Ntok, hd, hd
    d.nmask = 0 if maskT is None else maskT.shape[0]
    d.nwin = 0 if tok_idx is None else tok_idx.shape[0]
    if rows_per_sample is None:
        rows_per_sample = Ntok * max(d.nwin, 1)
    d.q_sB = d.k_sB = d.v_sB = rows_per_sample * qkv.ld
    d.q_sH = d.k_sH = d.v_sH = hd
    d.q_sT = d.k_sT = d.v_sT = qkv.ld
    d.o_sB, d.o_sH, d.o_sT = rows_per_sample * out.ld, hd, out.ld
    d.scale = float(scale)
    d.prec = _attn_prec(("qkv", heads, hd, Ntok, d.nwin), lambda: qkv.as_rows()[:, :Cc].abs().max() * abs(float(scale)),
                        lambda: qkv.as_rows()[:, Cc:].abs().max(), slot)
    base = qkv.ptr
    with _Timed("attention", 4.0 * B * heads * Ntok * Ntok * hd, 16.0 * B * Ntok * Cc, "B=%d h=%d N=%d d=%d" % (B, heads, Ntok, hd)):
        _attn_launch(lib, d, base, base + 4 * Cc, base + 8 * Cc, None,
                     biasT.data_ptr() if biasT is not None else None, maskT.data_ptr() if maskT is not None else None,
                     tok_idx.data_ptr() if tok_idx is not None else None, out.ptr, qkv.buf.device)
    return out


ATTN_PLANES = _os.environ.get("MSPI_ATTN_PLANES", "1") != "0"
ATTN_PREC = {}
LAST_ATTN = [None]


def attn_slot(pk):
    return pk.setdefault("attn_prec", {})


def _attn_prec(key, amax_q, amax_kv, slot=None):
    if DEFAULT_PREC != PREC_F16X3:
        return DEFAULT_PREC
    table = ATTN_PREC if slot is None else slot
    prec = table.get(key)
    if prec is None:
        if not _tuning():
            return PREC_F16X3
        aq, akv = float(amax_q()), float(amax_kv())
        bad = not (aq == aq and akv == akv) or aq >= 256.0 or akv >= 1024.0
        prec = table[key] = PREC_F32 if bad else PREC_F16X3
        if bad:
            RANGE_CHECK["moved"].append(("attention %s" % (key,), max(aq, akv)))
    return prec


def attn_variant():
    if LAST_ATTN[0] is None:
        return None
    return _lib.load().mspi_attn_variant(C.byref(LAST_ATTN[0][0]), *LAST_ATTN[0][1:])


def _attn_launch(lib, d, q, k, v, res, biasT, maskT, tok_idx, o, dev):
    nbytes = lib.mspi_attn_ws_bytes(C.byref(d)) if ATTN_PLANES else 0
    LAST_ATTN[0] = (d, biasT is not None, maskT is not None, tok_idx is not None, nbytes > 0)
    if nbytes:
        ws = torch.empty(nbytes, dtype=torch.uint8, device=dev)
        check(lib.mspi_attn_fwd_ws(C.byref(d), q, k, v, res, biasT, maskT, tok_idx, o, ws.data_ptr(), _stream()), "mspi_attn_fwd_ws")
    else:
        check(lib.mspi_attn_fwd(C.byref(d), q, k, v, res, biasT, maskT, tok_idx, o, _stream()), "mspi_attn_fwd")


def mlp(x, pk, res=None, ln=None, eps=1e-6, out=None, split=None):
    lib = _lib.load()
    _need_gpu(x.buf)
    if pk.fallback is None and not pk.checked and _tuning():
        pk.checked = True
        if split is None:
            w1, b1, w2, b2, osc = pk.src
            split = (pack_conv(w1, b1, act=pk.act, device=pk.w.device), pack_conv(w2, b2, out_scale=osc, device=pk.w.device))
        y = conv(conv(layernorm(x, ln[0], ln[1], eps) if ln is not None else x, split[0]), split[1], res=res, out=out)
        if split[0].prec != PREC_F16X3 or split[1].prec != PREC_F16X3:
            pk.fallback = split
        return y
    if pk.fallback is not None:
        return conv(conv(layernorm(x, ln[0], ln[1], eps) if ln is not None else x, pk.fallback[0]), pk.fallback[1], res=res, out=out)
    if x.C != pk.c or not x.dense:
        raise MspiError("mlp: input has %d channels (dense=%s), packed for %d" % (x.C, x.dense, pk.c))
    if pk.w.device != x.buf.device:
        raise MspiError("mlp: packed weights live on %s, the input on %s" % (pk.w.device, x.buf.device))
    if out is None:
        out = alloc(x.N, x.T, x.H, x.W, pk.c, x.buf.device)
    if res is not None and (res.M != x.M or not res.dense):
        raise MspiError("mlp: residual rows %d != rows %d (or residual not dense)" % (res.M, x.M))
    d = _lib.MlpDesc()
    d.M, d.C, d.hidden = x.M, pk.c, pk.hidden
    d.ldx, d.ldy, d.ldr = x.ld, out.ld, (res.ld if res is not None else 0)
    d.ln, d.act, d.eps = (1 if ln is not None else 0), pk.act, eps
    d.w1_scale, d.w2_scale = pk.s1, pk.s2
    with _Timed("mlp_fused", 4.0 * x.M * pk.c * pk.hidden, 4.0 * x.M * pk.c * (3 if res is not None else 2),
                "M=%d C=%d hidden=%d" % (x.M, pk.c, pk.hidden)):
        check(lib.mspi_mlp_fwd(C.byref(d), x.ptr, ln[0].data_ptr() if ln is not None else None,
                               ln[1].data_ptr() if ln is not None else None, pk.w.data_ptr(), pk.b1.data_ptr(),
                               pk.b2.data_ptr(), res.ptr if res is not None else None, out.ptr, _stream()), "mspi_mlp_fwd")
    return out


def layernorm_for_gemm(x, gamma, beta, eps, *packs):
    if sp_supported(x.C) and x.C >= 256 and all(p.k == (1, 1, 1) and p.stride == (1, 1, 1) and p.ldw == x.C and p.prec == PREC_F16X3
                                                 for p in packs):
        return layernorm(x, gamma, beta, eps, sp=True)
    return layernorm(x, gamma, beta, eps)


def mlp_tail(x, packed, ln, eps, res):
    if packed[0] == "fused":
        return mlp(x, packed[1], res=res, ln=ln, eps=eps)
    if sp_supported(x.C) and sp_supported(packed[1].cout_s) and packed[1].ldw == x.C and packed[2].ldw == packed[1].cout_s \
            and packed[1].prec == PREC_F16X3 and packed[2].prec == PREC_F16X3:
        return conv(conv(layernorm(x, ln[0], ln[1], eps, sp=True), packed[1], sp_out=True), packed[2], res=res)
    return conv(conv(layernorm(x, ln[0], ln[1], eps), packed[1]), packed[2], res=res)


def space_to_depth(x, out=None):
    lib = _lib.load()
    assert x.dense and x.C % 4 == 0
    if out is None:
        out = alloc(x.N, x.T, x.H // 2, x.W // 2, 4 * x.C, x.buf.device)
    with _Timed("space_to_depth", 0.0, 8.0 * x.M * x.C):
        check(lib.mspi_space_to_depth(x.ptr, x.ld, out.ptr, out.ld, x.N * x.T, x.H, x.W, x.C, _stream()), "mspi_space_to_depth")
    return out


def mvit_attention(q, k, v, B, heads, hd, scale, q_thw, k_thw, Rh, Rw, Rt, out=None, rel_gemm=None, slot=None):
    lib = _lib.load()
    _need_gpu(q.buf)
    Nq, Nk = q_thw[0] * q_thw[1] * q_thw[2], k_thw[0] * k_thw[1] * k_thw[2]
    J = k_thw[0] + k_thw[1] + k_thw[2]
    DA = 128 if hd + J <= 128 else (144 if hd + J <= 144 else 160)
    if hd != 96 or hd + J > DA:
        raise MspiError("mvit_attention: head_dim %d with %d relative-position columns is not instantiated" % (hd, J))
    dev = q.buf.device
    qa = torch.empty(B * heads * Nq * DA, dtype=torch.float32, device=dev)
    ka = torch.empty(B * heads * Nk * DA, dtype=torch.float32, device=dev)
    a = MvitAugDesc()
    a.B, a.heads, a.Dh, a.DA = B, heads, hd, DA
    a.qT, a.qH, a.qW = q_thw
    a.kT, a.kH, a.kW = k_thw
    a.ldq, a.ldk, a.scale = q.ld, k.ld, float(scale)
    if rel_gemm is not None and q.dense and q.ld == heads * hd:
        pkT, idx_h, idx_w, idx_t = rel_gemm
        rows = CL(q.buf, q.off, q.M * heads, 1, 1, 1, hd, hd)
        P = conv(rows, pkT)
        with _Timed("mvit_qk_augment", 0.0, 4.0 * B * heads * (Nq + Nk) * (hd + DA)):
            check(lib.mspi_mvit_qk_augment_p(C.byref(a), q.ptr, k.ptr, P.ptr, P.ld, idx_h.data_ptr(), idx_w.data_ptr(),
                                             idx_t.data_ptr(), qa.data_ptr(), ka.data_ptr(), _stream()), "mspi_mvit_qk_augment_p")
    else:
        with _Timed("mvit_qk_augment", 2.0 * B * heads * Nq * J * hd, 4.0 * B * heads * (Nq + Nk) * (hd + DA)):
            check(lib.mspi_mvit_qk_augment(C.byref(a), q.ptr, k.ptr, Rh.data_ptr(), Rw.data_ptr(), Rt.data_ptr(),
                                           qa.data_ptr(), ka.data_ptr(), _stream()), "mspi_mvit_qk_augment")
    if out is None:
        out = alloc(q.N, q.T, q.H, q.W, heads * hd, dev)
    d = AttnDesc()
    d.B, d.Hh, d.Nq, d.Nk, d.D, d.Dv, d.nmask = B, heads, Nq, Nk, DA, hd, 0
    d.q_sB, d.q_sH, d.q_sT = heads * Nq * DA, Nq * DA, DA
    d.k_sB, d.k_sH, d.k_sT = heads * Nk * DA, Nk * DA, DA
    d.v_sB, d.v_sH, d.v_sT = Nk * v.ld, hd, v.ld
    d.o_sB, d.o_sH, d.o_sT = Nq * out.ld, hd, out.ld
    d.scale = 1.0
    d.prec = _attn_prec(("mvit", heads, hd, Nq, Nk), lambda: qa.abs().max(), lambda: torch.maximum(ka.abs().max(), v.buf.abs().max()),
                        slot)
    assert q.ld == out.ld and q.dense and out.dense
    with _Timed("attention", 2.0 * B * heads * Nq * Nk * (DA + hd), 4.0 * B * heads * (Nq * (DA + 2 * hd) + Nk * (DA + hd)),
                "B=%d h=%d Nq=%d Nk=%d d=%d+%d" % (B, heads, Nq, Nk, DA, hd)):
        _attn_launch(lib, d, qa.data_ptr(), ka.data_ptr(), v.ptr, q.ptr, None, None, None, out.ptr, dev)
    return out


def upsample(src, factor, dst=None, accumulate=False, act=ACT_NONE):
    lib = _lib.load()
    assert src.dense
    if dst is None:
        assert not accumulate
        dst = alloc(src.N, src.T, src.H * factor, src.W * factor, src.C, src.buf.device)
    assert (dst.N, dst.T, dst.H, dst.W) == (src.N, src.T, src.H * factor, src.W * factor) and dst.C == src.C
    assert dst.dense
    with _Timed("upsample", 0.0, 4.0 * (src.M + dst.M * (2 if accumulate else 1)) * src.C):
        check(lib.mspi_upsample_fwd(src.ptr, src.ld, dst.ptr, dst.ld, src.N * src.T, src.H, src.W, src.Cs, factor,
                                    1 if accumulate else 0, act, _stream()), "mspi_upsample_fwd")
    return dst


def upsample_sum(dst, srcs, accumulate=True, act=ACT_NONE):
    lib = _lib.load()
    J = len(srcs)
    for s, k in srcs:
        assert s.dense and s.C == dst.C and (dst.N, dst.T) == (s.N, s.T)
        assert k >= 1 and (dst.H, dst.W) == (s.H * k, s.W * k)
    assert dst.dense
    ptrs = (C.c_void_p * max(J, 1))(*[s.ptr for s, _ in srcs])
    lds = (C.c_int64 * max(J, 1))(*[s.ld for s, _ in srcs])
    ks = (C.c_int32 * max(J, 1))(*[k for _, k in srcs])
    with _Timed("upsample_sum", 0.0, 4.0 * (sum(s.M for s, _ in srcs) + dst.M * (2 if accumulate else 1)) * dst.C):
        check(lib.mspi_upsample_sum_fwd(ptrs, lds, ks, J, dst.ptr, dst.ld, dst.N * dst.T, dst.H, dst.W, dst.Cs,
                                        1 if accumulate else 0, act, _stream()), "mspi_upsample_sum_fwd")
    return dst


def rowgate(x, mask):
    lib = _lib.load()
    assert mask.M == x.M and mask.ld == 1
    assert x.dense and mask.dense
    with _Timed("rowgate", 0.0, 8.0 * x.M * x.C):
        check(lib.mspi_rowgate(x.ptr, x.ld, mask.ptr, x.M, x.Cs, _stream()), "mspi_rowgate")
    return x


def logsumexp_sub(t, N, L):
    lib = _lib.load()
    check(lib.mspi_logsumexp_sub(t.data_ptr(), N, L, _stream()), "mspi_logsumexp_sub")
    return t


WGRAD_SLICES = (256, 2048)
WGRAD_BIG_M = 65536
C1_BWD_ROWS = 1024


def logsumexp_sub_bwd(logp, g, dz=None):
    lib = _lib.load()
    _need_gpu(logp)
    if logp.shape != g.shape or logp.dim() < 2 or logp.dtype != torch.float32 or g.dtype != torch.float32 or g.device != logp.device:
        raise MspiError("logsumexp_sub_bwd: logp %s / g %s must be fp32 tensors of one shape on one device" % (tuple(logp.shape), tuple(g.shape)))
    logp, g = logp.contiguous(), g.contiguous()
    N = logp.shape[0]
    if dz is None:
        dz = torch.empty_like(logp)
    with _Timed("logsumexp_sub_bwd", 0.0, 12.0 * logp.numel()):
        check(lib.mspi_logsumexp_sub_bwd(logp.data_ptr(), g.data_ptr(), dz.data_ptr(), N, logp.numel() // N, _stream()),
              "mspi_logsumexp_sub_bwd")
    return dz


def conv_c1_bwd(y, dz, weight):
    lib = _lib.load()
    _need_gpu(y.buf)
    Cc = y.Cs
    if y.T != 1 or not y.dense or tuple(dz.shape) != (y.N, y.H, y.W) or dz.dtype != torch.float32 or dz.device != y.buf.device:
        raise MspiError("conv_c1_bwd: y %s and dz %s do not match" % ((y.N, y.T, y.H, y.W, y.C), tuple(dz.shape)))
    if tuple(weight.shape) != (1, y.C, 1, 3, 3) or Cc != y.C or Cc > 64:
        raise MspiError("conv_c1_bwd: weight %s is not a (1,3,3) conv from %d channels (a multiple of 4, at most 64) to 1"
                        % (tuple(weight.shape), y.C))
    dev = y.buf.device
    dz = dz.contiguous()
    w = weight.detach().float().reshape(Cc, 9).t().contiguous().to(dev)
    d = alloc(y.N, 1, y.H, y.W, y.C, dev)
    dW = torch.empty(9, Cc, dtype=torch.float32, device=dev)
    db = torch.empty(1, dtype=torch.float32, device=dev)
    ws = torch.empty(lib.mspi_conv_c1_bwd_ws_bytes(y.N, y.H, y.W) // 4, dtype=torch.float32, device=dev)
    with _Timed("conv_c1_bwd", 4.0 * y.M * 9 * Cc, 8.0 * y.M * Cc, "M=%d C=%d" % (y.M, Cc)):
        check(lib.mspi_conv_c1_bwd(y.ptr, y.ld, dz.data_ptr(), w.data_ptr(), d.ptr, d.ld, dW.data_ptr(), db.data_ptr(),
                                   ws.data_ptr(), y.N, y.H, y.W, Cc, _stream()), "mspi_conv_c1_bwd")
    return d, dW.t().reshape(1, Cc, 1, 3, 3), db


def _wgrad_desc(x, dy, pk):
    To, Ho, Wo = _out_extent(x.T, x.H, x.W, pk.k, pk.stride, pk.pad)
    d = ConvDesc()
    d.N, d.T, d.H, d.W, d.C = x.N, x.T, x.H, x.W, x.Cs
    d.sN, d.sT, d.sH, d.sW, d.sC = x.sN, x.H * x.W * x.ld, x.W * x.ld, x.ld, 1
    d.kT, d.kH, d.kW = pk.k
    d.strT, d.strH, d.strW = pk.stride
    d.padT, d.padH, d.padW = pk.pad
    d.To, d.Ho, d.Wo = To, Ho, Wo
    d.Cout, d.ldy = pk.cout_s, dy.ld
    return d


def conv_wgrad_variant(x, dy, pk):
    return _lib.load().mspi_conv_wgrad_variant(C.byref(_wgrad_desc(x, dy, pk)), x.ptr, dy.ptr)


def conv_wgrad(x, dy, pk):
    lib = _lib.load()
    _need_gpu(x.buf)
    if x.Cs != pk.cin_s or dy.Cs != pk.cout_s:
        raise MspiError("conv_wgrad: x has %d / dy %d stored channels, the layer %d -> %d" % (x.Cs, dy.Cs, pk.cin_s, pk.cout_s))
    d = _wgrad_desc(x, dy, pk)
    if not dy.dense or dy.M != x.N * d.To * d.Ho * d.Wo or dy.buf.device != x.buf.device:
        raise MspiError("conv_wgrad: dy has %d rows, the layer's output %d (or dy is not dense)" % (dy.M, x.N * d.To * d.Ho * d.Wo))
    if lib.mspi_conv_wgrad_variant(C.byref(d), x.ptr, dy.ptr) < 0:
        raise MspiError("conv_wgrad: %s" % lib.mspi_last_error().decode("utf-8", "replace"))
    dev = x.buf.device
    kt, kh, kw = pk.k
    dW = torch.empty(pk.cout_s, kt, kh, kw, pk.cin_s, dtype=torch.float32, device=dev)
    db = torch.empty(pk.cout_s, dtype=torch.float32, device=dev)
    ws = torch.empty(lib.mspi_conv_wgrad_ws_bytes(C.byref(d)) // 4, dtype=torch.float32, device=dev)
    taps = kt * kh * kw
    with _Timed("conv_wgrad", 2.0 * dy.M * taps * pk.cin * pk.cout, 4.0 * (x.M * pk.cin + dy.M * pk.cout),
                "M=%d K=%d(%dx%d) N=%d" % (dy.M, taps * pk.cin, taps, pk.cin, pk.cout)):
        check(lib.mspi_conv_wgrad_fwd(C.byref(d), x.ptr, dy.ptr, dW.data_ptr(), db.data_ptr(), ws.data_ptr(), _stream()),
              "mspi_conv_wgrad_fwd")
    return dW[:pk.cout, :, :, :, :pk.cin].permute(0, 4, 1, 2, 3), db[:pk.cout]


def upsample_bwd(dy, factor, u=None, act=ACT_NONE, dx=None):
    lib = _lib.load()
    _need_gpu(dy.buf)
    if factor not in (2, 4, 8) or dy.H % factor or dy.W % factor or not dy.dense:
        raise MspiError("upsample_bwd: factor %s must be 2, 4 or 8 and divide the dense gradient's %d x %d" % (factor, dy.H, dy.W))
    if act not in (ACT_NONE, ACT_RELU) or (act == ACT_RELU) != (u is not None):
        raise MspiError("upsample_bwd: act is ACT_NONE without u, or ACT_RELU with the forward's output u")
    if u is not None and ((u.N, u.T, u.H, u.W, u.Cs) != (dy.N, dy.T, dy.H, dy.W, dy.Cs) or not u.dense or u.buf.device != dy.buf.device):
        raise MspiError("upsample_bwd: u does not match the gradient")
    if dx is None:
        dx = alloc(dy.N, dy.T, dy.H // factor, dy.W // factor, dy.C, dy.buf.device)
    elif (dx.N, dx.T, dx.H, dx.W, dx.C) != (dy.N, dy.T, dy.H // factor, dy.W // factor, dy.C) or not dx.dense or dx.buf.device != dy.buf.device:
        raise MspiError("upsample_bwd: dx does not match the gradient divided by the factor")
    with _Timed("upsample_bwd", 0.0, 4.0 * (dx.M + dy.M * (2 if u is not None else 1)) * dy.C):
        check(lib.mspi_upsample_bwd(dy.ptr, dy.ld, u.ptr if u is not None else None, u.ld if u is not None else 0, dx.ptr, dx.ld,
                                    dy.N * dy.T, dx.H, dx.W, dy.Cs, factor, act, _stream()), "mspi_upsample_bwd")
    return dx


WGRAD_WIDE_BOX_ROWS = 128
WGRAD_WIDE_SLICES = (4, 32)
WGRAD_WIDE_BIG_BOXES = 512
BN_ROWS = 512


def conv_wgrad_wide_variant(x, dy, pk):
    return _lib.load().mspi_conv_wgrad_wide_variant(C.byref(_wgrad_desc(x, dy, pk)), x.ptr, dy.ptr)


def conv_wgrad_wide(x, dy, pk):
    lib = _lib.load()
    _need_gpu(x.buf)
    if x.Cs != pk.cin_s or dy.Cs != pk.cout_s:
        raise MspiError("conv_wgrad_wide: x has %d / dy %d stored channels, the layer %d -> %d" % (x.Cs, dy.Cs, pk.cin_s, pk.cout_s))
    d = _wgrad_desc(x, dy, pk)
    if not dy.dense or dy.M != x.N * d.To * d.Ho * d.Wo or dy.buf.device != x.buf.device:
        raise MspiError("conv_wgrad_wide: dy has %d rows, the layer's output %d (or dy is not dense)"
                        % (dy.M, x.N * d.To * d.Ho * d.Wo))
    if lib.mspi_conv_wgrad_wide_variant(C.byref(d), x.ptr, dy.ptr) < 0:
        raise MspiError("conv_wgrad_wide: %s" % lib.mspi_last_error().decode("utf-8", "replace"))
    dev = x.buf.device
    kt, kh, kw = pk.k
    dW = torch.empty(pk.cout_s, kt, kh, kw, pk.cin_s, dtype=torch.float32, device=dev)
    db = torch.empty(pk.cout_s, dtype=torch.float32, device=dev)
    ws = torch.empty(lib.mspi_conv_wgrad_wide_ws_bytes(C.byref(d)) // 4, dtype=torch.float32, device=dev)
    taps = kt * kh * kw
    with _Timed("conv_wgrad_wide", 2.0 * dy.M * taps * pk.cin * pk.cout, 4.0 * (x.M * pk.cin + dy.M * pk.cout),
                "M=%d K=%d(%dx%d) N=%d" % (dy.M, taps * pk.cin, taps, pk.cin, pk.cout)):
        check(lib.mspi_conv_wgrad_wide_fwd(C.byref(d), x.ptr, dy.ptr, dW.data_ptr(), db.data_ptr(), ws.data_ptr(), _stream()),
              "mspi_conv_wgrad_wide_fwd")
    return dW[:pk.cout, :, :, :, :pk.cin].permute(0, 4, 1, 2, 3), db[:pk.cout]


def _bn_rows(name, x):
    if not x.dense or x.Cs != x.C:
        raise MspiError("%s: rows must be dense with a channel count that is a multiple of 4" % name)
    return x.M, x.C


def _bn_vec(name, what, t, Cc, dev):
    if t.dtype != torch.float32 or t.numel() != Cc or t.device != dev or not t.is_contiguous():
        raise MspiError("%s: %s must be a contiguous fp32 [%d] tensor on %s" % (name, what, Cc, dev))
    return t.data_ptr()


def bn_stats(x, eps=1e-5):
    lib = _lib.load()
    _need_gpu(x.buf)
    M, Cc = _bn_rows("bn_stats", x)
    dev = x.buf.device
    out = torch.empty(3, Cc, dtype=torch.float32, device=dev)
    ws = torch.empty(lib.mspi_bn_ws_bytes(M, Cc) // 4, dtype=torch.float32, device=dev)
    with _Timed("bn_stats", 4.0 * M * Cc, 4.0 * M * Cc, "M=%d C=%d" % (M, Cc)):
        check(lib.mspi_bn_stats(x.ptr, x.ld, M, Cc, eps, out[0].data_ptr(), out[1].data_ptr(), out[2].data_ptr(), ws.data_ptr(),
                                _stream()), "mspi_bn_stats")
    return out[0], out[1], out[2]


def bn_apply(x, mean, rstd, gamma, beta, act=ACT_NONE, out=None):
    lib = _lib.load()
    _need_gpu(x.buf)
    M, Cc = _bn_rows("bn_apply", x)
    dev = x.buf.device
    if out is None:
        out = alloc(x.N, x.T, x.H, x.W, x.C, dev)
    ptrs = [_bn_vec("bn_apply", n, t, Cc, dev) for n, t in (("mean", mean), ("rstd", rstd), ("gamma", gamma), ("beta", beta))]
    with _Timed("bn_apply", 3.0 * M * Cc, 8.0 * M * Cc, "M=%d C=%d" % (M, Cc)):
        check(lib.mspi_bn_apply(x.ptr, x.ld, ptrs[0], ptrs[1], ptrs[2], ptrs[3], out.ptr, out.ld, M, Cc, act, _stream()),
              "mspi_bn_apply")
    return out


def bn_bwd(dy, x, mean, rstd, gamma, y=None, dx=None):
    lib = _lib.load()
    _need_gpu(x.buf)
    M, Cc = _bn_rows("bn_bwd", x)
    dev = x.buf.device
    for t in (dy, y):
        if t is not None and ((t.M, t.C) != (M, Cc) or not t.dense or t.buf.device != dev):
            raise MspiError("bn_bwd: dy and y must match x (%d rows x %d channels, dense)" % (M, Cc))
    ptrs = [_bn_vec("bn_bwd", n, t, Cc, dev) for n, t in (("mean", mean), ("rstd", rstd), ("gamma", gamma))]
    if dx is None:
        dx = alloc(x.N, x.T, x.H, x.W, x.C, dev)
    elif (dx.M, dx.C) != (M, Cc) or not dx.dense or dx.buf.device != dev:
        raise MspiError("bn_bwd: dx must match x (%d rows x %d channels, dense)" % (M, Cc))
# ... 657 lines not shown
```

### mspi_amd/model/model_utils.py

```python
import os

import numpy as np
import torch
import torch.nn as nn

from .. import engine as E
from .._lib import MspiError
from ..autograd import Adapter as AdapterTrain
from ..autograd import (STAGE_NAMES, STAGES, SYNC_PREFIXES, ContrastHead, Fusion, LateralBlock, LateralEntry, ReadoutHead,
                        ReadoutTail, compose_lateral, convnext_block_forward, pack_convnext_block, pack_lateral_entry,
                        pack_readout_tail, r0_parts, reaches, readout_tail_forward, stage_rank, stages_upto, sync_block)
from ..backbones.convnext import ConvNeXtTinyFeatures
from ..backbones.resnet import get_resnet18
from ..module import HipModule, to_cl
from .get_video_backbones import video_motion_extractor


def get_sinusoid_encoding_table(n_position, d_hid):
    pos = np.arange(n_position, dtype=np.float64).reshape(-1, 1)
    hid = np.arange(d_hid).reshape(1, -1)
    ang = pos / np.power(10000, 2 * (hid // 2) / d_hid)
    ang[:, 0::2] = np.sin(ang[:, 0::2])
    ang[:, 1::2] = np.cos(ang[:, 1::2])
    return torch.tensor(ang, dtype=torch.float, requires_grad=False).unsqueeze(0)


def _f(t):
    return t.detach().float().contiguous()


class Mlp(nn.Module):
    def __init__(self, in_features, hidden_features):
        super().__init__()
        self.fc1 = nn.Linear(in_features, hidden_features)
        self.act = nn.GELU()
        self.fc2 = nn.Linear(hidden_features, in_features)


class Attention(nn.Module):
    def __init__(self, dim, num_heads=8, qkv_bias=False):
        super().__init__()
        assert dim % num_heads == 0, "dim should be divisible by num_heads"
        self.num_heads = num_heads
        self.scale = (dim // num_heads) ** -0.5
        self.qkv = nn.Linear(dim, dim * 3, bias=qkv_bias)
        self.proj = nn.Linear(dim, dim)


class Block(HipModule):

    def __init__(self, dim, num_heads, mlp_ratio=4.0):
        super().__init__()
        self.norm1 = nn.LayerNorm(dim)
        self.attn = Attention(dim, num_heads=num_heads)
        self.norm2 = nn.LayerNorm(dim)
        self.mlp = Mlp(dim, int(dim * mlp_ratio))

    def _pack(self):
        a, m = self.attn, self.mlp
        return {"n1": (_f(self.norm1.weight), _f(self.norm1.bias)), "n2": (_f(self.norm2.weight), _f(self.norm2.bias)),
                "qkv": E.pack_conv(a.qkv.weight, a.qkv.bias), "proj": E.pack_conv(a.proj.weight, a.proj.bias),
                "fc1": E.pack_conv(m.fc1.weight, m.fc1.bias, act=E.ACT_GELU), "fc2": E.pack_conv(m.fc2.weight, m.fc2.bias)}

    def run(self, x, B, R):
        pk = self.pk
        dim = self.norm1.normalized_shape[0]
        h = E.layernorm_for_gemm(x, *pk["n1"], 1e-5, pk["qkv"])
        o = E.attention(E.conv(h, pk["qkv"]), B, R, self.attn.num_heads, dim // self.attn.num_heads, self.attn.scale,
                        slot=E.attn_slot(pk))
        x = E.conv(o, pk["proj"], res=x)
        return E.mlp_tail(x, ("split", pk["fc1"], pk["fc2"]), pk["n2"], 1e-5, res=x)

    def tensors(self):
        a, m = self.attn, self.mlp
        return (self.norm1.weight, self.norm1.bias, a.qkv.weight, a.proj.weight, a.proj.bias, self.norm2.weight, self.norm2.bias,
                m.fc1.weight, m.fc1.bias, m.fc2.weight, m.fc2.bias)


class SyncBlock(HipModule):
    def __init__(self, num_blocks=3, num_vis_tokens=336, num_aud_tokens=36, vis_in_embed=1024, embed_dim=512):
        super().__init__()
        self.vis_pos_embed = get_sinusoid_encoding_table(num_vis_tokens, 512)
        self.aud_pos_embed = get_sinusoid_encoding_table(num_aud_tokens, 512)
        self.vis_proj = nn.Linear(vis_in_embed, 512)
        self.vis_norm = nn.LayerNorm(512)
        self.aud_norm = nn.LayerNorm(512)
        self.blocks = nn.ModuleList([Block(dim=embed_dim, num_heads=4) for _ in range(num_blocks)])
        for m in self.modules():
            if isinstance(m, nn.Linear):
                nn.init.xavier_uniform_(m.weight)
                if m.bias is not None:
                    nn.init.constant_(m.bias, 0)
            elif isinstance(m, nn.LayerNorm):
                nn.init.constant_(m.bias, 0)
                nn.init.constant_(m.weight, 1.0)

    def _pack(self):
        dev = self.vis_proj.weight.device
        return {"proj": E.pack_conv(self.vis_proj.weight, self.vis_proj.bias),
                "vn": (_f(self.vis_norm.weight), _f(self.vis_norm.bias)),
                "an": (_f(self.aud_norm.weight), _f(self.aud_norm.bias)),
                "vpos": self.vis_pos_embed[0].to(dev).contiguous(), "apos": self.aud_pos_embed[0].to(dev).contiguous()}

    def run(self, vis, aud):
        pk = self.pk
        B, Rv, Ra = vis.N, vis.T * vis.H * vis.W, aud.T * aud.H * aud.W
        if Rv != pk["vpos"].shape[0] or Ra != pk["apos"].shape[0]:
            raise MspiError("SyncBlock: got %d visual / %d audio tokens but the positional tables hold %d / %d rows "
                            "-- set cfg.MODEL.NUM_VIS_TOKENS[name] / cfg.MODEL.NUM_AUD_TOKENS (reference: the add at "
                            "model/model_utils.py:273-274 fails the same way)" % (Rv, Ra, pk["vpos"].shape[0], pk["apos"].shape[0]))
        x = E.alloc(B, Rv + Ra, 1, 1, 512, vis.buf.device)
        E.layernorm(E.conv(vis, pk["proj"]), *pk["vn"], 1e-5, out=x.tokens(0, vis.T, vis.H, vis.W), table=pk["vpos"])
        E.layernorm(aud, *pk["an"], 1e-5, out=x.tokens(Rv, aud.T, aud.H, aud.W), table=pk["apos"])
        for blk in self.blocks:
            x = blk.run(x, B, Rv + Ra)
        return x

    def tensors(self):
        return (self.vis_proj.weight, self.vis_proj.bias, self.vis_norm.weight, self.vis_norm.bias, self.aud_norm.weight,
                self.aud_norm.bias)

    def forward(self, vis_fea, aud_fea):
        a = aud_fea[:, :, None] if aud_fea.dim() == 4 else aud_fea
        x = self.run(to_cl(vis_fea), to_cl(a))
        return x.as_rows().view(x.N, x.T, 512)


class BasicConv3d(nn.Module):
    def __init__(self, in_planes, out_planes, kernel_size, stride, padding=0):
        super().__init__()
        self.conv = nn.Conv3d(in_planes, out_planes, kernel_size=kernel_size, stride=stride, padding=padding, bias=False)
        self.bn = nn.BatchNorm3d(out_planes, eps=1e-3, momentum=0.001, affine=True)
        self.relu = nn.ReLU()

    def packed(self):
        c = self.conv
        return E.pack_conv(c.weight, None, self.bn, c.stride, c.padding, E.ACT_RELU)


class SepConv3d(nn.Module):
    def __init__(self, in_planes, out_planes, kernel_size, stride, padding=0):
        super().__init__()
        k, s, p = kernel_size, stride, padding
        self.conv_s = nn.Conv3d(in_planes, out_planes, (1, k, k), (1, s, s), (0, p, p), bias=False)
        self.bn_s = nn.BatchNorm3d(out_planes, eps=1e-3, momentum=0.001, affine=True)
        self.relu_s = nn.ReLU()
        self.conv_t = nn.Conv3d(out_planes, out_planes, (k, 1, 1), (s, 1, 1), (p, 0, 0), bias=False)
        self.bn_t = nn.BatchNorm3d(out_planes, eps=1e-3, momentum=0.001, affine=True)
        self.relu_t = nn.ReLU()

    def packed(self):
        cs, ct = self.conv_s, self.conv_t
        return (E.pack_conv(cs.weight, None, self.bn_s, cs.stride, cs.padding, E.ACT_RELU),
                E.pack_conv(ct.weight, None, self.bn_t, ct.stride, ct.padding, E.ACT_RELU))


class SA(HipModule):

    def __init__(self, in_embed_dim=512, k=2):
        super().__init__()
        self.k = k
        self.up = nn.Upsample(scale_factor=(1, k, k), align_corners=False, mode="trilinear") if k != 1 else nn.Identity()
        self.conv_mask = nn.Sequential(
            BasicConv3d(in_embed_dim, in_embed_dim // 16, kernel_size=3, stride=1, padding=1),
            self.up,
            nn.Conv3d(in_embed_dim // 16, 1, kernel_size=(1, 3, 3), stride=1, padding=(0, 1, 1)),
            nn.Sigmoid(),
        )

    def tensors(self):
        b, c = self.conv_mask[0], self.conv_mask[2]
        return [b.conv.weight, b.bn.weight, b.bn.bias, c.weight, c.bias], (b.bn.running_mean, b.bn.running_var, b.bn.num_batches_tracked)

    def _pack(self):
        c = self.conv_mask[2]
        return self.conv_mask[0].packed(), E.pack_conv(c.weight, c.bias, None, (1, 1, 1), (0, 1, 1), E.ACT_SIGMOID)

    def run(self, x, mask, premask=None):
        p0, p2 = self.pk
        m = E.conv(mask, p0) if premask is None else premask
        if self.k != 1:
            m = E.upsample(m, self.k)
        return E.rowgate(x, E.conv(m, p2))


class Inception(HipModule):
    def __init__(self, embed_dim=320 + 96):
        super().__init__()
        self.branch0 = nn.Sequential(BasicConv3d(embed_dim, 192, kernel_size=1, stride=1))
        self.branch1 = nn.Sequential(BasicConv3d(embed_dim, 96, kernel_size=1, stride=1),
                                     SepConv3d(96, 208, kernel_size=3, stride=1, padding=1))
        self.branch2 = nn.Sequential(BasicConv3d(embed_dim, 16, kernel_size=1, stride=1),
                                     SepConv3d(16, 48, kernel_size=3, stride=1, padding=1))
        self.branch3 = nn.Sequential(nn.MaxPool3d(kernel_size=(3, 3, 3), stride=1, padding=1),
                                     BasicConv3d(embed_dim, 64, kernel_size=1, stride=1))

    def _pack(self):
        return {"b0": self.branch0[0].packed(), "b1": (self.branch1[0].packed(),) + self.branch1[1].packed(),
                "b2": (self.branch2[0].packed(),) + self.branch2[1].packed(), "b3": self.branch3[1].packed()}

    def run(self, x):
        pk = self.pk
        out = E.alloc(x.N, x.T, x.H, x.W, 512, x.buf.device)
        E.conv(x, pk["b0"], out=out.slice(0, 192))
        E.conv(E.conv(E.conv(x, pk["b1"][0]), pk["b1"][1]), pk["b1"][2], out=out.slice(192, 208))
        E.conv(E.conv(E.conv(x, pk["b2"][0]), pk["b2"][1]), pk["b2"][2], out=out.slice(400, 48))
        E.conv(E.maxpool(x, (3, 3, 3), (1, 1, 1), (1, 1, 1)), pk["b3"], out=out.slice(448, 64))
        return out


class Adapter(HipModule):
    def __init__(self, embed_dim=320 + 96, num_frames=32, stride=8):
        super().__init__()
        self.num_frames = num_frames
        self.stride = stride
        self.pool_time = nn.MaxPool3d(kernel_size=(stride, 1, 1), stride=(stride, 1, 1))
        self.conv = Inception(embed_dim=embed_dim)
        self.up = nn.Upsample(scale_factor=(1, 2, 2), align_corners=False, mode="trilinear")

    def tensors(self):
        ts, bns = [], []
        for conv, bn in self.layers().values():
            ts += [conv.weight, bn.weight, bn.bias]
            bns.append((bn.running_mean, bn.running_var, bn.num_batches_tracked))
        return ts, bns

    def layers(self):
        c = self.conv
        b1, b2 = c.branch1, c.branch2
        return {"conv.branch0.0.bn": (c.branch0[0].conv, c.branch0[0].bn), "conv.branch1.0.bn": (b1[0].conv, b1[0].bn),
                "conv.branch1.1.bn_s": (b1[1].conv_s, b1[1].bn_s), "conv.branch1.1.bn_t": (b1[1].conv_t, b1[1].bn_t),
                "conv.branch2.0.bn": (b2[0].conv, b2[0].bn), "conv.branch2.1.bn_s": (b2[1].conv_s, b2[1].bn_s),
                "conv.branch2.1.bn_t": (b2[1].conv_t, b2[1].bn_t), "conv.branch3.1.bn": (c.branch3[1].conv, c.branch3[1].bn)}

    def run(self, o3, o2, features=False):
        T, s = self.num_frames, self.stride
        B = o3.N // T
        o3 = o3.reshape(B, T, o3.H, o3.W)
        o2 = o2.reshape(B, T, o2.H, o2.W)
        cat = E.alloc(B, T // s, o3.H, o3.W, o3.C + o2.C, o3.buf.device)
        E.maxpool(o3, (s, 1, 1), (s, 1, 1), (0, 0, 0), out=cat.slice(0, o3.C))
        E.upsample(E.maxpool(o2, (s, 1, 1), (s, 1, 1), (0, 0, 0)), 2, dst=cat.slice(o3.C, o2.C))
        return cat if reaches(features, "adapter") else self.conv.run(cat)


class LayerNorm3d(nn.Module):
    def __init__(self, dim):
        super().__init__()
        self.norm = nn.LayerNorm(dim)


class ConvNextBlock(HipModule):

    def __init__(self, dim, drop_path=0.0):
        super().__init__()
        self.dwconv_t = nn.Conv3d(dim, dim, kernel_size=(7, 1, 1), padding=(3, 0, 0), groups=dim)
        self.dwconv_s = nn.Conv3d(dim, dim, kernel_size=(1, 7, 7), padding=(0, 3, 3), groups=dim)
        self.norm = LayerNorm3d(dim)
        self.pwconv1 = nn.Conv3d(dim, 4 * dim, 1)
        self.act = nn.GELU()
        self.pwconv2 = nn.Conv3d(4 * dim, dim, 1)
        self.drop_path = nn.Identity()
        for m in self.modules():
            if isinstance(m, (nn.Conv3d, nn.Linear)):
                nn.init.trunc_normal_(m.weight, std=0.02)
                nn.init.constant_(m.bias, 0)

    def tensors(self):
        return (self.dwconv_t.weight, self.dwconv_t.bias, self.dwconv_s.weight, self.dwconv_s.bias, self.norm.norm.weight,
                self.norm.norm.bias, self.pwconv1.weight, self.pwconv1.bias, self.pwconv2.weight, self.pwconv2.bias)

    def _pack(self):
        return pack_convnext_block(*self.tensors())

    def run(self, x, out=None):
        return convnext_block_forward(x, self.pk, out=out)[0]


class StaticSaliencyModelConvNext(HipModule):

    def __init__(self):
        super().__init__()
        self.encoder = ConvNeXtTinyFeatures()
        self.up = nn.Upsample(scale_factor=2, mode="bilinear", align_corners=False)
        self.up4 = nn.Upsample(scale_factor=4, mode="bilinear", align_corners=False)
        self.up8 = nn.Upsample(scale_factor=8, mode="bilinear", align_corners=False)
        self.smooth_0 = nn.Sequential(nn.Conv2d(768, 320, 3, 1, 1), nn.BatchNorm2d(320), nn.ReLU())
        self.smooth_1 = nn.Sequential(nn.Conv2d(384, 96, 3, 1, 1), nn.BatchNorm2d(96), nn.ReLU())

    def _pack(self):
        return tuple(E.pack_conv(s[0].weight, s[0].bias, s[1], (1, 1, 1), (0, 1, 1), E.ACT_RELU)
                     for s in (self.smooth_0, self.smooth_1))

    def run(self, clips):
        s0, s1 = self.pk
        _, _, o1, o0 = self.encoder.forward_cl(clips)
        return E.conv(o1, s1), E.conv(o0, s0)

    def forward(self, x):
        o1, o0 = self.run(x)
        return o1.as_ncdhw().squeeze(2), o0.as_ncdhw().squeeze(2)


class _Fork:
    ENABLED = os.environ.get("MSPI_STREAMS", "1") != "0"

    def __init__(self, owner, device):
        self.main = torch.cuda.current_stream(device)
        d = owner.__dict__
        if "_side_streams" not in d or d["_side_streams"][0].device != device:
            d["_side_streams"] = [torch.cuda.Stream(device) for _ in range(2)]
        self.side = d["_side_streams"]
        self.used = []
        self.kept = []

    def __enter__(self):
        self.start = torch.cuda.Event()
        self.start.record(self.main)
        return self

    def branch(self, i, refork=False):
        if not self.ENABLED:
            return torch.cuda.stream(self.main)
        s = self.side[i]
        if refork:
            ev = torch.cuda.Event()
            ev.record(self.main)
            s.wait_event(ev)
        else:
            s.wait_event(self.start)
        if s not in self.used:
            self.used.append(s)
        return torch.cuda.stream(s)

    def keep(self, *objs):
        self.kept.extend(objs)

    def join(self, i):
        s = self.side[i]
        if self.ENABLED and s in self.used:
            ev = torch.cuda.Event()
            ev.record(s)
            self.main.wait_event(ev)
            self.used.remove(s)

    def __exit__(self, *exc):
        for s in list(self.used):
            ev = torch.cuda.Event()
            ev.record(s)
            self.main.wait_event(ev)
        self.used = []
        self.kept = []
        return False


DECODER_FUSED = os.environ.get("MSPI_DECODER_FUSED", "1") != "0"


def _compose_lateral(c0, c1):
    return compose_lateral(c0.weight, c0.bias, c1.weight)


class _SaliencyBase(HipModule):

    def _build_decoder(self, cfg, vis_embed_dims, extra_c4, de_embed_dim=192):
        d = de_embed_dim
        for k in range(4):
            cin = vis_embed_dims[k] + (extra_c4 if k == 3 else 0)
            layers = [nn.Conv3d(cin, d, 1, 1, 0)]
            if cfg.MODEL.LATERAL_BOOL[k]:
                s = cfg.MODEL.LATERAL_STRIDE[k]
                layers.append(nn.Conv3d(d, d, kernel_size=(s, 1, 1), stride=(s, 1, 1), bias=False))
            layers.append(ConvNextBlock(dim=d))
            setattr(self, "latlayer_%d" % k, nn.Sequential(*layers))
        self.upsample = nn.Upsample(scale_factor=(1, 2, 2), mode="trilinear", align_corners=False)
        self.upsample_4 = nn.Upsample(scale_factor=(1, 4, 4), mode="trilinear", align_corners=False)
        self.upsample_8 = nn.Upsample(scale_factor=(1, 8, 8), mode="trilinear", align_corners=False)
        self.readout = nn.Sequential(
            nn.Conv3d(d * 4, d, 1, 1, 0),
            nn.Conv3d(d, d, kernel_size=3, stride=1, padding=1),
            nn.BatchNorm3d(d),
            nn.ReLU(inplace=True),
            nn.Conv3d(d, 64, kernel_size=(1, 3, 3), stride=(1, 1, 1), padding=(0, 1, 1)),
            nn.BatchNorm3d(64),
            nn.ReLU(inplace=True),
            nn.Upsample(scale_factor=(1, 4, 4), mode="trilinear", align_corners=False),
            nn.Conv3d(64, 32, kernel_size=(4, 1, 1), stride=(4, 1, 1), padding=0),
            nn.ReLU(inplace=True),
            nn.Conv3d(32, 32, kernel_size=(1, 3, 3), stride=(1, 1, 1), padding=(0, 1, 1)),
            nn.ReLU(inplace=True),
            nn.Conv3d(32, 1, kernel_size=(1, 3, 3), stride=(1, 1, 1), padding=(0, 1, 1)),
        )
        self.adapter = Adapter(num_frames=cfg.DATA.NUM_FRAMES, stride=cfg.DATA.NUM_FRAMES // 4)
        self.sa_0 = SA(512, k=4)
        self.sa_1 = SA(512, k=2)
        self.sa_2 = SA(512, k=1)

    def _pack_lateral(self, k, split=None):
        seq = getattr(self, "latlayer_%d" % k)
        if len(seq) == 3:
            return pack_lateral_entry(seq[0].weight, seq[0].bias, seq[1].weight, tuple(seq[1].stride), split)
        return pack_lateral_entry(seq[0].weight, seq[0].bias, None, (1, 1, 1), split)

    def _pack_decoder(self, split=None):
        r = self.readout
        return {
            "sa_cat": self._pack_sa_cat(),
            "lat": [self._pack_lateral(k, split if k == 3 else None) for k in range(4)],
            "r0": E.pack_conv(r[0].weight, r[0].bias),
            "r0_parts": self._pack_r0_parts(r[0]),
            "r1": E.pack_conv(r[1].weight, r[1].bias, r[2], (1, 1, 1), (1, 1, 1), E.ACT_RELU),
            "r4": E.pack_conv(r[4].weight, r[4].bias, r[5], (1, 1, 1), (0, 1, 1), E.ACT_RELU),
            "r8": E.pack_conv(r[8].weight, r[8].bias, None, (4, 1, 1), (0, 0, 0), E.ACT_NONE),
            "r10": E.pack_conv(r[10].weight, r[10].bias, None, (1, 1, 1), (0, 1, 1), E.ACT_RELU),
            "r12": E.pack_conv(r[12].weight, r[12].bias, None, (1, 1, 1), (0, 1, 1), E.ACT_NONE),
            "tail_key": self._tail_key(),
            "head_key": self._head_key(),
            "sa_key": self._sa_key(),
        }

    def _pack_sa_cat(self):
        sa_w, sa_b = zip(*[E.fold_bn(m.conv_mask[0].conv.weight, None, m.conv_mask[0].bn) for m in (self.sa_0, self.sa_1, self.sa_2)])
        return E.pack_conv(torch.cat(sa_w, 0), torch.cat(sa_b, 0), None, (1, 1, 1), (1, 1, 1), E.ACT_RELU)

    _r0_parts = staticmethod(r0_parts)

    def _pack_r0_parts(self, conv):
        return [E.pack_conv(w, b) for w, b in self._r0_parts(conv.weight, conv.bias)]

    def _lateral(self, pk, k, xs, out=None, features=False):
        if reaches(features, "lateral_entries"):
            return [E.join_planes(x) if isinstance(x, E.SP) else x for x in xs]
        y = E.conv(xs[0], pk["lat"][k][0])
        if len(xs) == 2:
            y = E.conv(xs[1], pk["lat"][k][1], res=y)
        if reaches(features, "lateral_blocks"):
            return y
        return getattr(self, "latlayer_%d" % k)[-1].run(y, out=out)

    def _laterals_012(self, pk, v1, v2, v3, features=False):
        if DECODER_FUSED:
            return (None,) + tuple(self._lateral(pk, k, [v], features=features) for k, v in enumerate((v1, v2, v3)))
        B = v1.N
        cat = E.alloc(B, max(1, v1.T // (self.cfg.MODEL.LATERAL_STRIDE[0] if self.cfg.MODEL.LATERAL_BOOL[0] else 1)),
                      v1.H, v1.W, 4 * 192, v1.buf.device)
        s0 = self._lateral(pk, 0, [v1], out=cat.slice(0, 192))
        return cat, s0, self._lateral(pk, 1, [v2]), self._lateral(pk, 2, [v3])

    @torch.no_grad()
    def encode_frames(self, frames):
        self._check_eval()
        with self.plans_checked():
            o1, o0 = self.image_encoder.run(frames.float()[:, :, None])
        return (o1.buf.view(o1.N, o1.H, o1.W, o1.ld)[..., :o1.C], o0.buf.view(o0.N, o0.H, o0.W, o0.ld)[..., :o0.C])

    @staticmethod
    def _wrap_frame_feats(frame_feats):
        outs = []
        for f in frame_feats:
            f = f.float().contiguous()
            n, h, w, c = f.shape
            outs.append(E.CL(f.view(-1), 0, n, 1, h, w, c, c))
        return outs

    def _premask(self, pk, masks):
        self._refresh_sa(pk)
        return E.conv(masks, pk["sa_cat"])

    def _fuse_readout(self, pk, cat, s0, s1, s2, s3, masks, pm, features=False):
        if reaches(features, "fusion"):
            return s0, s1, s2, s3, masks
        if not reaches(features, "readout"):
            self._refresh_head(pk)
        self.sa_2.run(s2, masks, pm.slice(64, 32))
        E.upsample(s3, 2, dst=s2, accumulate=True)
        self.sa_1.run(s1, masks, pm.slice(32, 32))
        if cat is None:
            E.upsample_sum(s1, [(s2, 2), (s3, 4)])
            self.sa_0.run(s0, masks, pm.slice(0, 32))
            if reaches(features, "readout"):
                return s0, s1, s2, s3
            p0, p1, p2, p3 = pk["r0_parts"]
            y = E.conv(s0, p0)
            E.upsample_sum(y, [(E.conv(s1, p1), 2), (E.conv(s2, p2), 4), (E.conv(s3, p3), 8)])
        else:
            E.upsample(s2, 2, dst=s1, accumulate=True)
            E.upsample(s3, 4, dst=s1, accumulate=True)
            self.sa_0.run(s0, masks, pm.slice(0, 32))
            E.upsample(s1, 2, dst=s0, accumulate=True)
            E.upsample(s2, 4, dst=s0, accumulate=True)
            E.upsample(s3, 8, dst=s0, accumulate=True)
            E.upsample(s1, 2, dst=cat.slice(192, 192))
            E.upsample(s2, 4, dst=cat.slice(384, 192))
            E.upsample(s3, 8, dst=cat.slice(576, 192))
            y = E.conv(cat, pk["r0"])
        y4 = E.conv(E.conv(y, pk["r1"]), pk["r4"])
        return y4 if features else self._readout_tail(pk, y4)

    def _readout_tail(self, pk, y4):
        self._refresh_tail(pk)
        return readout_tail_forward(y4, pk["r8"], pk["r10"], pk["r12"])[0]

    _PK_SELF_KEYED = ("readout", "sa_0", "sa_1", "sa_2")

    def _refresh_sa(self, pk):
        key = self._sa_key()
        if pk["sa_key"] != key:
            pk["sa_cat"] = self._pack_sa_cat()
            pk["sa_key"] = key

    def _refresh_head(self, pk):
        key = self._head_key()
        if pk["head_key"] != key:
            r = self.readout
            pk["r0"], pk["r0_parts"] = E.pack_conv(r[0].weight, r[0].bias), self._pack_r0_parts(r[0])
            pk["r1"] = E.pack_conv(r[1].weight, r[1].bias, r[2], (1, 1, 1), (1, 1, 1), E.ACT_RELU)
            pk["r4"] = E.pack_conv(r[4].weight, r[4].bias, r[5], (1, 1, 1), (0, 1, 1), E.ACT_RELU)
            pk["head_key"] = key

    def _refresh_tail(self, pk):
        key = self._tail_key()
        if pk["tail_key"] != key:
            r = self.readout
            pk["r8"], pk["r10"], pk["r12"] = pack_readout_tail(r[8].weight, r[8].bias, r[10].weight, r[10].bias,
                                                               r[12].weight, r[12].bias)
            pk["tail_key"] = key

    def _pk_refresh(self, pk):
        grad_tail = self._training_tail()
        if [p for p, _ in self._sa_key()] != [p for p, _ in pk["sa_key"]]:
            self.__dict__.pop("_pk", None)
            return
        with torch.no_grad():
            if not reaches(grad_tail, "fusion"):
                self._refresh_sa(pk)
            if not reaches(grad_tail, "readout"):
                self._refresh_head(pk)
            if not grad_tail:
                self._refresh_tail(pk)

    def _tail_key(self):
        r = self.readout
        return tuple((p.data_ptr(), p._version) for i in (8, 10, 12) for p in (r[i].weight, r[i].bias))

    def _head_key(self):
        r = self.readout
        ts = [t for i in (0, 1, 4) for t in (r[i].weight, r[i].bias)]
        ts += [t for i in (2, 5) for t in (r[i].weight, r[i].bias, r[i].running_mean, r[i].running_var)]
        return tuple((t.data_ptr(), t._version) for t in ts)

    def _sa_key(self):
        ts = []
        for m in (self.sa_0, self.sa_1, self.sa_2):
            b = m.conv_mask[0]
            ts += [b.conv.weight, b.bn.weight, b.bn.bias, b.bn.running_mean, b.bn.running_var]
        return tuple((t.data_ptr(), t._version) for t in ts)

    TAIL_PARAMS = STAGES[0].params

    def trainable(self, what, sync=False):
        d = self.__dict__
        if sync:
            if not hasattr(self, "aud_vis_sync_block"):
                raise MspiError("trainable(%r, sync=True): %s has neither a SyncBlock nor a contrastive head; sync=True is for "
                                "AudioVisualSaliencyModel" % (what, type(self).__name__))
            if what is None or (what in STAGE_NAMES and not reaches(what, "lateral_entries")):
                raise MspiError("trainable(%r, sync=True): the SyncBlock reaches the map only through latlayer_3's entry conv, so "
                                "sync=True needs a stage that trains it: %s" % (what, " or ".join(repr(n) for n in STAGE_NAMES[4:])))
        if what is None:
            for p, flag in d.pop("_trainable_saved", []):
                p.requires_grad_(flag)
            d["_trainable"] = None
            d["_trainable_sync"] = False
            return self
        if what not in STAGE_NAMES:
            raise MspiError("trainable: %r is not a trainable part of this model (only %s and %r are)"
                            % (what, ", ".join(repr(n) for n in STAGE_NAMES[:-1]), STAGE_NAMES[-1]))
        if reaches(what, "readout") and not DECODER_FUSED:
            raise MspiError("trainable(%r) needs the fused decoder path: it is switched off by MSPI_DECODER_FUSED=0" % (what,))
        if d.get("_trainable") is None:
            d["_trainable_saved"] = [(p, p.requires_grad) for p in self.parameters()]
        d["_trainable"] = what
        d["_trainable_sync"] = bool(sync)
        prefixes = tuple(p.format(k=k, last=len(getattr(self, "latlayer_%d" % k)) - 1)
                         for st in stages_upto(what) for p in st.params for k in range(4)) + (SYNC_PREFIXES if sync else ())
        for name, p in self.named_parameters():
            p.requires_grad_(name.startswith(prefixes))
        return self

    def _batch_stat_modules(self):
        return {n: self.get_submodule(n) for st in stages_upto(self.__dict__.get("_trainable")) for n in st.batch_stat}

    def _training_tail(self):
        what = self.__dict__.get("_trainable")
        return STAGES[stage_rank(what)].stop if what is not None and torch.is_grad_enabled() else False

    def _check_eval(self):
        super()._check_eval()
        what = self.__dict__.get("_trainable")
# ... 238 lines not shown
```

Before: 689.8 clips/s.

## Fuse the next stage's downsample LayerNorm into the last ConvNeXt block MLP

Adds an LN2 variant of the fused MLP kernel. At the end of ConvNeXt stages 0 and 1, it computes the downsample LayerNorm of the block output in the epilogue and writes the normalized tensor directly. When the caller does not need a stage's output (the static model only uses stages 2 and 3), the plain output write is skipped. This removes a separate LayerNorm launch and a full read/write pass of the activations at two stage seams, at the cost of extra register pressure in the epilogue.

```diff
diff --git a/include/mspi_cnx_hip.h b/include/mspi_cnx_hip.h
--- /dev/null
+++ b/include/mspi_cnx_hip.h
@@ -0,0 +1,26 @@
+#ifndef MSPI_CNX_HIP_H
+#define MSPI_CNX_HIP_H
+
+#include "mspi_hip.h"
+
+#ifdef __cplusplus
+extern "C" {
+#endif
+
+typedef struct {
+  int64_t M;
+  int32_t C, hidden;
+  int64_t ldx, ldr, ldy, ldn;
+  int32_t ln;
+  float eps, eps2;
+  float w1_scale, w2_scale;
+} MspiCnxMlpLnDesc;
+
+int mspi_cnx_mlp_ln_fwd(const MspiCnxMlpLnDesc* d, const void* x, const void* gamma, const void* beta, const void* w_packed,
+                        const void* b1, const void* b2, const void* res, const void* gamma2, const void* beta2, void* y,
+                        void* y_ln, mspi_stream_t stream);
+
+#ifdef __cplusplus
+}
+#endif
+#endif
diff --git a/mspi_amd/_lib.py b/mspi_amd/_lib.py
--- a/mspi_amd/_lib.py
+++ b/mspi_amd/_lib.py
@@ -106,6 +106,15 @@
         ("N", C.c_int32), ("T", C.c_int32), ("H", C.c_int32), ("W", C.c_int32),
         ("sN", C.c_int64), ("sC", C.c_int64), ("sT", C.c_int64), ("sH", C.c_int64), ("sW", C.c_int64),
         ("ldy", C.c_int64),
+    ]
+
+
+class CnxMlpLnDesc(C.Structure):
+    _fields_ = [
+        ("M", C.c_int64), ("C", C.c_int32), ("hidden", C.c_int32),
+        ("ldx", C.c_int64), ("ldr", C.c_int64), ("ldy", C.c_int64), ("ldn", C.c_int64),
+        ("ln", C.c_int32), ("eps", C.c_float), ("eps2", C.c_float),
+        ("w1_scale", C.c_float), ("w2_scale", C.c_float),
     ]
 
 
@@ -351,6 +360,12 @@
 
 X3D_EXPORTS = tuple(_X3D_SIGNATURES)
 
+_CNX_SIGNATURES = {
+    "mspi_cnx_mlp_ln_fwd": (C.c_int, [C.POINTER(CnxMlpLnDesc), _P, _P, _P, _P, _P, _P, _P, _P, _P, _P, _P, _P]),
+}
+
+CNX_EXPORTS = tuple(_CNX_SIGNATURES)
+
 _lib = None
 
 
@@ -366,7 +381,7 @@
     lib = C.CDLL(LIB_PATH)
     for name, (res, args) in list(_SIGNATURES.items()) + list(_TRAIN_SIGNATURES.items()) + list(_BLOCK_SIGNATURES.items()) + \
             list(_ENTRY_SIGNATURES.items()) + list(_ADAPTER_SIGNATURES.items()) + list(_SYNC_SIGNATURES.items()) + list(_LINEAR_SIGNATURES.items()) + \
-            list(_CONTRAST_SIGNATURES.items()) + list(_X3D_SIGNATURES.items()):
+            list(_CONTRAST_SIGNATURES.items()) + list(_X3D_SIGNATURES.items()) + list(_CNX_SIGNATURES.items()):
         fn = getattr(lib, name)
         fn.restype = res
         fn.argtypes = args
diff --git a/mspi_amd/backbones/convnext.py b/mspi_amd/backbones/convnext.py
--- a/mspi_amd/backbones/convnext.py
+++ b/mspi_amd/backbones/convnext.py
@@ -1,3 +1,5 @@
+import os
+
 import torch
 import torch.nn as nn
 
@@ -6,6 +8,10 @@
 
 DEPTHS = (3, 3, 9, 3)
 DIMS = (96, 192, 384, 768)
+
+
+def _seams():
+    return os.environ.get("MSPI_CNX_SEAMS", "1") != "0"
 
 
 class _Mlp(nn.Module):
@@ -33,6 +39,13 @@
         pk = self.pk
         return E.mlp_tail(E.dwconv(x, pk["dw"]), pk["mlp"], pk["ln"], 1e-6, res=x)
 
+    def run_ln(self, x, ln2, want_y):
+        pk = self.pk
+        if pk["mlp"][0] == "fused" and _seams():
+            return E.mlp_ln(E.dwconv(x, pk["dw"]), pk["mlp"][1], pk["ln"], ln2, res=x, want_y=want_y)
+        y = self.run(x)
+        return y, E.layernorm(y, ln2[0], ln2[1], 1e-6)
+
 
 class ConvNeXtStage(HipModule):
     def __init__(self, dim_in, dim_out, depth, downsample):
@@ -50,13 +63,14 @@
         return (ln.weight.detach().float().contiguous(), ln.bias.detach().float().contiguous(),
                 E.pack_conv(cv.weight, cv.bias, None, (1, 2, 2), (0, 0, 0)))
 
-    def run(self, x):
+    def run(self, x, x_ln=None, next_ln=None, want_y=True):
         if self.pk is not None:
             g, b, cv = self.pk
-            x = E.conv(E.layernorm(x, g, b, 1e-6), cv)
-        for blk in self.blocks:
+            x = E.conv(E.layernorm(x, g, b, 1e-6) if x_ln is None else x_ln, cv)
+        blocks = list(self.blocks)
+        for blk in blocks[:-1] if next_ln is not None else blocks:
             x = blk.run(x)
-        return x
+        return x if next_ln is None else blocks[-1].run_ln(x, next_ln, want_y)
 
 
 class ConvNeXtTinyFeatures(HipModule):
@@ -79,15 +93,20 @@
                 self.stem_1.weight.detach().float().contiguous(), self.stem_1.bias.detach().float().contiguous())
 
     @torch.no_grad()
-    def forward_cl(self, clips):
+    def forward_cl(self, clips, need=(True, True, True, True)):
         self._check_eval()
         stem, g, b = self.pk
         x = E.conv(clips, stem)
         x = x.reshape(x.N * x.T, 1, x.H, x.W)
         x = E.layernorm(x, g, b, 1e-6)
-        outs = []
-        for i in range(4):
-            x = getattr(self, "stages_%d" % i).run(x)
+        stages = [getattr(self, "stages_%d" % i) for i in range(4)]
+        outs, x_ln = [], None
+        for i, st in enumerate(stages):
+            if i < 2 and DIMS[i] in (96, 192):
+                nxt = stages[i + 1].pk
+                x, x_ln = st.run(x, x_ln, next_ln=(nxt[0], nxt[1]), want_y=bool(need[i]))
+            else:
+                x, x_ln = st.run(x, x_ln), None
             outs.append(x)
         return outs
 
diff --git a/mspi_amd/csrc/convnext_seams.hip b/mspi_amd/csrc/convnext_seams.hip
--- /dev/null
+++ b/mspi_amd/csrc/convnext_seams.hip
@@ -0,0 +1,43 @@
+#include "common.h"
+#include "../../include/mspi_cnx_hip.h"
+#include "mlp_fused_kernel.h"
+
+using namespace mspi;
+
+extern "C" int mspi_cnx_mlp_ln_fwd(const MspiCnxMlpLnDesc* d, const void* x, const void* gamma, const void* beta, const void* w_packed,
+                                   const void* b1, const void* b2, const void* res, const void* gamma2, const void* beta2, void* y,
+                                   void* y_ln, void* stream) {
+  MSPI_REQUIRE(d && x && w_packed && b1 && b2, "mspi_cnx_mlp_ln_fwd: null argument");
+  MSPI_REQUIRE(y_ln, "mspi_cnx_mlp_ln_fwd: y_ln is required (y alone: mspi_mlp_fwd)");
+  MSPI_REQUIRE(gamma2 && beta2, "mspi_cnx_mlp_ln_fwd: the second LayerNorm needs gamma2 and beta2");
+  MSPI_REQUIRE(d->C == 96 || d->C == 192, "mspi_cnx_mlp_ln_fwd: C = %d not supported (96, 192)", d->C);
+  MSPI_REQUIRE(d->hidden % 32 == 0 && d->hidden >= 32 && d->hidden <= (d->C == 96 ? 512 : 1024),
+               "mspi_cnx_mlp_ln_fwd: hidden = %d not supported with C = %d", d->hidden, d->C);
+  MSPI_REQUIRE(d->ldn >= d->C && d->ldn % 4 == 0 && (!y || (d->ldy >= d->C && d->ldy % 4 == 0)) &&
+               (!res || (d->ldr >= d->C && d->ldr % 4 == 0)),
+               "mspi_cnx_mlp_ln_fwd: row strides must be >= C and multiples of 4 floats");
+  MSPI_REQUIRE(!d->ln || (gamma && beta), "mspi_cnx_mlp_ln_fwd: LayerNorm needs gamma and beta");
+  MspiMlpDesc m;
+  m.M = d->M; m.C = d->C; m.hidden = d->hidden;
+  m.ldx = d->ldx; m.ldr = d->ldr; m.ldy = y ? d->ldy : d->ldn;
+  m.ln = d->ln; m.act = MSPI_ACT_GELU; m.eps = d->eps;
+  m.w1_scale = d->w1_scale; m.w2_scale = d->w2_scale;
+  const int variant = mspi_mlp_variant(&m);
+  if (variant < 0) return variant;
+  MlpArgs a = {};
+  a.x = (const float*)x; a.gamma = (const float*)gamma; a.beta = (const float*)beta; a.wp = (const unsigned char*)w_packed;
+  a.b1 = (const float*)b1; a.b2 = (const float*)b2; a.res = (const float*)res; a.y = (float*)y;
+  a.M = d->M; a.ldx = d->ldx; a.ldr = d->ldr; a.ldy = d->ldy;
+  a.nch = d->hidden / 32; a.ln = d->ln; a.act = MSPI_ACT_GELU; a.eps = d->eps;
+  a.inv_s1 = 1.0f / d->w1_scale; a.inv_s2 = 1.0f / d->w2_scale;
+  a.status = g_status_word;
+  a.gamma2 = (const float*)gamma2; a.beta2 = (const float*)beta2; a.y_ln = (float*)y_ln; a.ldn = d->ldn; a.eps2 = d->eps2;
+  hipStream_t s = (hipStream_t)stream;
+  switch (variant) {
+    case 96244: launch_mlp<96, 2, 4, 4, true>(a, s); break;
+    case 96134: launch_mlp<96, 1, 3, 4, true>(a, s); break;
+    case 192138: launch_mlp<192, 1, 3, 8, true>(a, s); break;
+    default: launch_mlp<192, 1, 3, 4, true>(a, s); break;
+  }
+  return check_launch("mspi_cnx_mlp_ln_fwd");
+}
diff --git a/mspi_amd/csrc/mlp_fused.hip b/mspi_amd/csrc/mlp_fused.hip
--- a/mspi_amd/csrc/mlp_fused.hip
+++ b/mspi_amd/csrc/mlp_fused.hip
@@ -1,307 +1,6 @@
 #include "common.h"
 #include <stdlib.h>
-#include <type_traits>
-
-namespace mspi {
-
-typedef _Float16 v8h __attribute__((ext_vector_type(8)));
-typedef float v16f __attribute__((ext_vector_type(16)));
-typedef __attribute__((address_space(3))) void lds_void;
-
-struct MlpArgs {
-  const float* x; const float* gamma; const float* beta; const unsigned char* wp; const float* b1; const float* b2;
-  const float* res; float* y;
-  long M, ldx, ldr, ldy;
-  int nch;
-  int ln, act;
-  float eps, inv_s1, inv_s2;
-  int* status;
-};
-
-template <int C, int TM, int NS, int NWV = 4>
-__global__ __launch_bounds__(64 * NWV, (C == 96 && TM == 1 && NWV == 4) ? 2 : 1) void mlp_fused_kernel(const MlpArgs p) {
-  constexpr int KS = C / 16, CT = C / 32;
-  constexpr int W1B = KS * 2048, W2B = 2 * CT * 2048, SB = W1B + W2B;
-  constexpr int DPW = SB / (1024 * NWV);
-  constexpr int BM = NWV * 32 * TM;
-  static_assert(SB % (1024 * NWV) == 0, "a stage is dealt in whole 1-KB pieces to the waves");
-  static_assert(C % 32 == 0 && SB % 4096 == 0, "C: multiple of 32");
-  __shared__ __attribute__((aligned(16))) unsigned char smem[NS * SB + (C == 96 ? 2048 : 4096)];
-  float* b1s = reinterpret_cast<float*>(smem + NS * SB);
-
-  const int tid = threadIdx.x, lane = tid & 63, wave = tid >> 6;
-  const int li = lane & 31, lh = lane >> 5;
-  const long row0 = (long)blockIdx.x * BM + wave * (32 * TM);
-
-  static_assert(W1B % (DPW * 1024) == 0, "the W1 / W2 boundary of a stage falls between waves");
-  auto issue_stage = [&](int j) {
-    const bool w1 = wave * DPW * 1024 < W1B;
-    const int jc = w1 ? (j + 2 < p.nch ? j + 2 : 0) : j;
-    const unsigned char* src = p.wp + (long)jc * SB + (wave * DPW) * 1024 + lane * 16;
-    unsigned char* dst = smem + (j % NS) * SB + (wave * DPW) * 1024;
-#pragma unroll
-    for (int d = 0; d < DPW; ++d)
-      __builtin_amdgcn_global_load_lds(reinterpret_cast<const float*>(src + d * 1024), (lds_void*)(dst + d * 1024), 16, 0, 0);
-  };
-  static_assert(W1B == W2B, "the prologue parks W1 of chunk 1 in a W2 half");
-  constexpr int DP0 = W1B / (1024 * NWV);
-  static_assert(W1B % (1024 * NWV) == 0, "W1 of a chunk is dealt in whole pieces");
-  auto issue_w1_01 = [&]() {
-#pragma unroll
-    for (int c = 0; c < 2; ++c) {
-      const int jc = c < p.nch ? c : 0;
-#pragma unroll
-      for (int d = 0; d < DP0; ++d)
-        __builtin_amdgcn_global_load_lds(reinterpret_cast<const float*>(p.wp + (long)jc * SB + (wave * DP0 + d) * 1024 + lane * 16),
-                                         (lds_void*)(smem + (NS - 1) * SB + c * W1B + (wave * DP0 + d) * 1024), 16, 0, 0);
-    }
-  };
-
-  float xr[TM][KS][8];
-#pragma unroll
-  for (int t = 0; t < TM; ++t) {
-    long row = row0 + t * 32 + li;
-    if (row >= p.M) row = p.M - 1;
-    const float* xp = p.x + row * p.ldx + 8 * lh;
-#pragma unroll
-    for (int ks = 0; ks < KS; ++ks) {
-      const float4 a = *reinterpret_cast<const float4*>(xp + 16 * ks);
-      const float4 b = *reinterpret_cast<const float4*>(xp + 16 * ks + 4);
-      xr[t][ks][0] = a.x; xr[t][ks][1] = a.y; xr[t][ks][2] = a.z; xr[t][ks][3] = a.w;
-      xr[t][ks][4] = b.x; xr[t][ks][5] = b.y; xr[t][ks][6] = b.z; xr[t][ks][7] = b.w;
-    }
-  }
-  static_assert(NS >= 3, "the pipeline keeps stage j-1 in use while stage j is in flight and the prologue's slot is live");
-  issue_w1_01();
-  for (int j = 0; j < NS - 1; ++j) issue_stage(j < p.nch ? j : 0);
-  for (int i = tid; i < p.nch * 32; i += 64 * NWV) b1s[i] = p.b1[i];
-
-  if (p.ln) {
-#pragma unroll
-    for (int t = 0; t < TM; ++t) {
-      float s = 0.f;
-#pragma unroll
-      for (int ks = 0; ks < KS; ++ks)
-#pragma unroll
-        for (int e = 0; e < 8; ++e) s += xr[t][ks][e];
-      s += __shfl_xor(s, 32, 64);
-      const float mean = s / (float)C;
-      float q = 0.f;
-#pragma unroll
-      for (int ks = 0; ks < KS; ++ks)
-#pragma unroll
-        for (int e = 0; e < 8; ++e) { const float d = xr[t][ks][e] - mean; q = fmaf(d, d, q); }
-      q += __shfl_xor(q, 32, 64);
-      const float rstd = rsqrtf(q / (float)C + p.eps);
-#pragma unroll
-      for (int ks = 0; ks < KS; ++ks)
-#pragma unroll
-        for (int e = 0; e < 8; ++e) xr[t][ks][e] = (xr[t][ks][e] - mean) * rstd;
-    }
-#pragma unroll
-    for (int ks = 0; ks < KS; ++ks) {
-      const float4 g0 = *reinterpret_cast<const float4*>(p.gamma + 16 * ks + 8 * lh);
-      const float4 g1 = *reinterpret_cast<const float4*>(p.gamma + 16 * ks + 8 * lh + 4);
-      const float4 c0 = *reinterpret_cast<const float4*>(p.beta + 16 * ks + 8 * lh);
-      const float4 c1 = *reinterpret_cast<const float4*>(p.beta + 16 * ks + 8 * lh + 4);
-      const float g8[8] = {g0.x, g0.y, g0.z, g0.w, g1.x, g1.y, g1.z, g1.w};
-      const float c8[8] = {c0.x, c0.y, c0.z, c0.w, c1.x, c1.y, c1.z, c1.w};
-#pragma unroll
-      for (int t = 0; t < TM; ++t)
-#pragma unroll
-        for (int e = 0; e < 8; ++e) xr[t][ks][e] = fmaf(xr[t][ks][e], g8[e], c8[e]);
-    }
-  }
-  v8h xh[TM][KS], xl[TM][KS];
-#pragma unroll
-  for (int t = 0; t < TM; ++t)
-#pragma unroll
-    for (int ks = 0; ks < KS; ++ks)
-#pragma unroll
-      for (int e = 0; e < 8; ++e) {
-        _Float16 h, l;
-        split_f16(xr[t][ks][e], h, l);
-        xh[t][ks][e] = h; xl[t][ks][e] = l;
-      }
-
-  v16f o[TM][CT];
-#pragma unroll
-  for (int t = 0; t < TM; ++t)
-#pragma unroll
-    for (int ct = 0; ct < CT; ++ct)
-#pragma unroll
-      for (int i = 0; i < 16; ++i) o[t][ct][i] = 0.f;
-
-  auto phase1 = [&](const unsigned char* w1, v16f (&h)[TM]) {
-#pragma unroll
-    for (int t = 0; t < TM; ++t)
-#pragma unroll
-      for (int i = 0; i < 16; ++i) h[t][i] = 0.f;
-#pragma unroll
-    for (int ks = 0; ks < KS; ++ks) {
-      const v8h wh = *reinterpret_cast<const v8h*>(w1 + (ks * 2 + 0) * 1024);
-      const v8h wl = *reinterpret_cast<const v8h*>(w1 + (ks * 2 + 1) * 1024);
-#pragma unroll
-      for (int t = 0; t < TM; ++t) {
-        if (!kSingleProduct) {
-          h[t] = __builtin_amdgcn_mfma_f32_32x32x16_f16(wl, xh[t][ks], h[t], 0, 0, 0);
-          h[t] = __builtin_amdgcn_mfma_f32_32x32x16_f16(wh, xl[t][ks], h[t], 0, 0, 0);
-        }
-        h[t] = __builtin_amdgcn_mfma_f32_32x32x16_f16(wh, xh[t][ks], h[t], 0, 0, 0);
-      }
-    }
-  };
-  v16f h[TM], hn[TM];
-  v8h hh[TM][2], hl[TM][2], gh[TM][2], gl[TM][2];
-  auto body = [&](auto has_p2, auto has_p1, int j, const unsigned char* st) {
-    constexpr bool P2 = decltype(has_p2)::value, P1 = decltype(has_p1)::value;
-    constexpr int T0 = P2 ? 0 : 2 * CT, T1 = P1 ? 2 * CT + KS : 2 * CT, NTR = T1 - T0;
-    auto frag = [&](int tr, int plane) {
-      const unsigned char* base = tr < 2 * CT ? st + W1B + (tr * 2) * 1024 : st + ((tr - 2 * CT) * 2) * 1024;
-      return *reinterpret_cast<const v8h*>(base + plane * 1024);
-    };
-    float bv[16];
-#pragma unroll
-    for (int q = 0; q < 4; ++q) {
-      const float4 b = *reinterpret_cast<const float4*>(b1s + j * 32 + q * 8 + 4 * lh);
-      bv[q * 4 + 0] = b.x; bv[q * 4 + 1] = b.y; bv[q * 4 + 2] = b.z; bv[q * 4 + 3] = b.w;
-    }
-    v8h wh, wl, nh, nl;
-    if (NTR > 0) { wh = frag(T0, 0); wl = frag(T0, 1); }
-#pragma unroll
-    for (int g = 0; g < 16; ++g) {
-#pragma unroll
-      for (int tr = T0 + g * NTR / 16; tr < T0 + (g + 1) * NTR / 16; ++tr) {
-        if (tr + 1 < T1) { nh = frag(tr + 1, 0); nl = frag(tr + 1, 1); }
-        __builtin_amdgcn_sched_barrier(0);
-#pragma unroll
-        for (int t = 0; t < TM; ++t) {
-          if (tr < 2 * CT) {
-            const int s = tr / CT, ct = tr % CT;
-            if (!kSingleProduct) {
-              o[t][ct] = __builtin_amdgcn_mfma_f32_32x32x16_f16(wl, hh[t][s], o[t][ct], 0, 0, 0);
-              o[t][ct] = __builtin_amdgcn_mfma_f32_32x32x16_f16(wh, hl[t][s], o[t][ct], 0, 0, 0);
-            }
-            o[t][ct] = __builtin_amdgcn_mfma_f32_32x32x16_f16(wh, hh[t][s], o[t][ct], 0, 0, 0);
-          } else {
-            const int ks = tr - 2 * CT;
-            const v16f zero = {0.f, 0.f, 0.f, 0.f, 0.f, 0.f, 0.f, 0.f, 0.f, 0.f, 0.f, 0.f, 0.f, 0.f, 0.f, 0.f};
-            if (!kSingleProduct) {
-              hn[t] = __builtin_amdgcn_mfma_f32_32x32x16_f16(wl, xh[t][ks], ks == 0 ? zero : hn[t], 0, 0, 0);
-              hn[t] = __builtin_amdgcn_mfma_f32_32x32x16_f16(wh, xl[t][ks], hn[t], 0, 0, 0);
-              hn[t] = __builtin_amdgcn_mfma_f32_32x32x16_f16(wh, xh[t][ks], hn[t], 0, 0, 0);
-            } else {
-              hn[t] = __builtin_amdgcn_mfma_f32_32x32x16_f16(wh, xh[t][ks], ks == 0 ? zero : hn[t], 0, 0, 0);
-            }
-          }
-        }
-        wh = nh; wl = nl;
-      }
-#pragma unroll
-      for (int t = 0; t < TM; ++t) {
-        const float u = fmaf(h[t][g], p.inv_s1, bv[g]);
-        const float v = gelu_erf(u);
-        _Float16 f, l;
-        split_f16(v, f, l);
-        gh[t][g >> 3][g & 7] = f;
-        gl[t][g >> 3][g & 7] = l;
-      }
-      __builtin_amdgcn_sched_barrier(0);
-    }
-#pragma unroll
-    for (int t = 0; t < TM; ++t) {
-      if (P1) h[t] = hn[t];
-#pragma unroll
-      for (int s = 0; s < 2; ++s) { hh[t][s] = gh[t][s]; hl[t][s] = gl[t][s]; }
-    }
-  };
-  using yes = std::true_type;
-  using no = std::false_type;
-
-  asm volatile("s_waitcnt vmcnt(%0)" ::"n"((NS - 1) * DPW) : "memory");
-  asm volatile("s_waitcnt lgkmcnt(0)" ::: "memory");
-  __builtin_amdgcn_s_barrier();
-  phase1(smem + (NS - 1) * SB + lane * 16, h);
-  if (p.nch > 1) body(no(), yes(), 0, smem + (NS - 1) * SB + W1B + lane * 16);
-  else body(no(), no(), 0, smem + lane * 16);
-
-  auto top = [&](int j) {
-    if (j + NS - 3 < p.nch) asm volatile("s_waitcnt vmcnt(%0)" ::"n"((NS - 2) * DPW) : "memory");
-    else asm volatile("s_waitcnt vmcnt(0)" ::: "memory");
-    asm volatile("s_waitcnt lgkmcnt(0)" ::: "memory");
-    __builtin_amdgcn_s_barrier();
-    if (j + NS - 2 < p.nch) issue_stage(j + NS - 2);
-  };
-  int j = 1;
-  for (; j + 1 < p.nch; ++j) {
-    top(j);
-    body(yes(), yes(), j, smem + ((j - 1) % NS) * SB + lane * 16);
-  }
-  if (j < p.nch) {
-    top(j);
-    body(yes(), no(), j, smem + ((j - 1) % NS) * SB + lane * 16);
-    ++j;
-  }
-  top(j);
-  {
-    const unsigned char* w2 = smem + ((j - 1) % NS) * SB + lane * 16 + W1B;
-#pragma unroll
-    for (int s = 0; s < 2; ++s)
-#pragma unroll
-      for (int ct = 0; ct < CT; ++ct) {
-        const v8h wh = *reinterpret_cast<const v8h*>(w2 + ((s * CT + ct) * 2 + 0) * 1024);
-        const v8h wl = *reinterpret_cast<const v8h*>(w2 + ((s * CT + ct) * 2 + 1) * 1024);
-#pragma unroll
-        for (int t = 0; t < TM; ++t) {
-          if (!kSingleProduct) {
-            o[t][ct] = __builtin_amdgcn_mfma_f32_32x32x16_f16(wl, hh[t][s], o[t][ct], 0, 0, 0);
-            o[t][ct] = __builtin_amdgcn_mfma_f32_32x32x16_f16(wh, hl[t][s], o[t][ct], 0, 0, 0);
-          }
-          o[t][ct] = __builtin_amdgcn_mfma_f32_32x32x16_f16(wh, hh[t][s], o[t][ct], 0, 0, 0);
-        }
-      }
-  }
-
-  bool bad = false;
-#pragma unroll
-  for (int t = 0; t < TM; ++t) {
-    const long row = row0 + t * 32 + li;
-    const bool ok = row < p.M;
-    const long rr = ok ? row : 0;
-#pragma unroll
-    for (int ct = 0; ct < CT; ++ct) {
-      float4 rv[4];
-#pragma unroll
-      for (int q = 0; q < 4; ++q) {
-        const int c = ct * 32 + q * 8 + 4 * lh;
-        rv[q] = p.res ? *reinterpret_cast<const float4*>(p.res + rr * p.ldr + c) : make_float4(0.f, 0.f, 0.f, 0.f);
-      }
-#pragma unroll
-      for (int q = 0; q < 4; ++q) {
-        const int c = ct * 32 + q * 8 + 4 * lh;
-        const float4 b = *reinterpret_cast<const float4*>(p.b2 + c);
-        float4 v;
-        v.x = fmaf(o[t][ct][q * 4 + 0], p.inv_s2, b.x) + rv[q].x;
-        v.y = fmaf(o[t][ct][q * 4 + 1], p.inv_s2, b.y) + rv[q].y;
-        v.z = fmaf(o[t][ct][q * 4 + 2], p.inv_s2, b.z) + rv[q].z;
-        v.w = fmaf(o[t][ct][q * 4 + 3], p.inv_s2, b.w) + rv[q].w;
-        bad |= nonfinite(v.x) | nonfinite(v.y) | nonfinite(v.z) | nonfinite(v.w);
-        if (ok) *reinterpret_cast<float4*>(p.y + row * p.ldy + c) = v;
-      }
-    }
-  }
-  report_nonfinite(p.status, bad);
-}
-
-template <int C, int TM, int NS, int NWV = 4>
-static int launch_mlp(const MlpArgs& a, hipStream_t s) {
-  constexpr int BM = 32 * NWV * TM;
-  const long nb = (a.M + BM - 1) / BM;
-  hipLaunchKernelGGL((mlp_fused_kernel<C, TM, NS, NWV>), dim3((unsigned)nb), dim3(64 * NWV), 0, s, a);
-  return 0;
-}
-
-}
+#include "mlp_fused_kernel.h"
 
 using namespace mspi;
 
@@ -335,7 +34,7 @@
   const int variant = mlp_select(d, gamma && beta);
   if (variant < 0) return variant;
   MSPI_REQUIRE(!res || (d->ldr >= d->C && d->ldr % 4 == 0), "mspi_mlp_fwd: row strides must be >= C and multiples of 4 floats");
-  MlpArgs a;
+  MlpArgs a = {};
   a.x = (const float*)x; a.gamma = (const float*)gamma; a.beta = (const float*)beta; a.wp = (const unsigned char*)w_packed;
   a.b1 = (const float*)b1; a.b2 = (const float*)b2; a.res = (const float*)res; a.y = (float*)y;
   a.M = d->M; a.ldx = d->ldx; a.ldr = d->ldr; a.ldy = d->ldy;
diff --git a/mspi_amd/csrc/mlp_fused_kernel.h b/mspi_amd/csrc/mlp_fused_kernel.h
--- /dev/null
+++ b/mspi_amd/csrc/mlp_fused_kernel.h
@@ -0,0 +1,348 @@
+#pragma once
+#include "common.h"
+#include <type_traits>
+
+namespace mspi {
+
+typedef _Float16 v8h __attribute__((ext_vector_type(8)));
+typedef float v16f __attribute__((ext_vector_type(16)));
+typedef __attribute__((address_space(3))) void lds_void;
+
+struct MlpArgs {
+  const float* x; const float* gamma; const float* beta; const unsigned char* wp; const float* b1; const float* b2;
+  const float* res; float* y;
+  long M, ldx, ldr, ldy;
+  int nch;
+  int ln, act;
+  float eps, inv_s1, inv_s2;
+  int* status;
+  const float* gamma2; const float* beta2; float* y_ln;
+  long ldn;
+  float eps2;
+};
+
+template <int C, int TM, int NS, int NWV = 4, bool LN2 = false>
+__global__ __launch_bounds__(64 * NWV, (C == 96 && TM == 1 && NWV == 4) ? 2 : 1) void mlp_fused_kernel(const MlpArgs p) {
+  constexpr int KS = C / 16, CT = C / 32;
+  constexpr int W1B = KS * 2048, W2B = 2 * CT * 2048, SB = W1B + W2B;
+  constexpr int DPW = SB / (1024 * NWV);
+  constexpr int BM = NWV * 32 * TM;
+  static_assert(SB % (1024 * NWV) == 0, "a stage is dealt in whole 1-KB pieces to the waves");
+  static_assert(C % 32 == 0 && SB % 4096 == 0, "C: multiple of 32");
+  __shared__ __attribute__((aligned(16))) unsigned char smem[NS * SB + (C == 96 ? 2048 : 4096)];
+  float* b1s = reinterpret_cast<float*>(smem + NS * SB);
+
+  const int tid = threadIdx.x, lane = tid & 63, wave = tid >> 6;
+  const int li = lane & 31, lh = lane >> 5;
+  const long row0 = (long)blockIdx.x * BM + wave * (32 * TM);
+
+  static_assert(W1B % (DPW * 1024) == 0, "the W1 / W2 boundary of a stage falls between waves");
+  auto issue_stage = [&](int j) {
+    const bool w1 = wave * DPW * 1024 < W1B;
+    const int jc = w1 ? (j + 2 < p.nch ? j + 2 : 0) : j;
+    const unsigned char* src = p.wp + (long)jc * SB + (wave * DPW) * 1024 + lane * 16;
+    unsigned char* dst = smem + (j % NS) * SB + (wave * DPW) * 1024;
+#pragma unroll
+    for (int d = 0; d < DPW; ++d)
+      __builtin_amdgcn_global_load_lds(reinterpret_cast<const float*>(src + d * 1024), (lds_void*)(dst + d * 1024), 16, 0, 0);
+  };
+  static_assert(W1B == W2B, "the prologue parks W1 of chunk 1 in a W2 half");
+  constexpr int DP0 = W1B / (1024 * NWV);
+  static_assert(W1B % (1024 * NWV) == 0, "W1 of a chunk is dealt in whole pieces");
+  auto issue_w1_01 = [&]() {
+#pragma unroll
+    for (int c = 0; c < 2; ++c) {
+      const int jc = c < p.nch ? c : 0;
+#pragma unroll
+      for (int d = 0; d < DP0; ++d)
+        __builtin_amdgcn_global_load_lds(reinterpret_cast<const float*>(p.wp + (long)jc * SB + (wave * DP0 + d) * 1024 + lane * 16),
+                                         (lds_void*)(smem + (NS - 1) * SB + c * W1B + (wave * DP0 + d) * 1024), 16, 0, 0);
+    }
+  };
+
+  float xr[TM][KS][8];
+#pragma unroll
+  for (int t = 0; t < TM; ++t) {
+    long row = row0 + t * 32 + li;
+    if (row >= p.M) row = p.M - 1;
+    const float* xp = p.x + row * p.ldx + 8 * lh;
+#pragma unroll
+    for (int ks = 0; ks < KS; ++ks) {
+      const float4 a = *reinterpret_cast<const float4*>(xp + 16 * ks);
+      const float4 b = *reinterpret_cast<const float4*>(xp + 16 * ks + 4);
+      xr[t][ks][0] = a.x; xr[t][ks][1] = a.y; xr[t][ks][2] = a.z; xr[t][ks][3] = a.w;
+      xr[t][ks][4] = b.x; xr[t][ks][5] = b.y; xr[t][ks][6] = b.z; xr[t][ks][7] = b.w;
+    }
+  }
+  static_assert(NS >= 3, "the pipeline keeps stage j-1 in use while stage j is in flight and the prologue's slot is live");
+  issue_w1_01();
+  for (int j = 0; j < NS - 1; ++j) issue_stage(j < p.nch ? j : 0);
+  for (int i = tid; i < p.nch * 32; i += 64 * NWV) b1s[i] = p.b1[i];
+
+  if (p.ln) {
+#pragma unroll
+    for (int t = 0; t < TM; ++t) {
+      float s = 0.f;
+#pragma unroll
+      for (int ks = 0; ks < KS; ++ks)
+#pragma unroll
+        for (int e = 0; e < 8; ++e) s += xr[t][ks][e];
+      s += __shfl_xor(s, 32, 64);
+      const float mean = s / (float)C;
+      float q = 0.f;
+#pragma unroll
+      for (int ks = 0; ks < KS; ++ks)
+#pragma unroll
+        for (int e = 0; e < 8; ++e) { const float d = xr[t][ks][e] - mean; q = fmaf(d, d, q); }
+      q += __shfl_xor(q, 32, 64);
+      const float rstd = rsqrtf(q / (float)C + p.eps);
+#pragma unroll
+      for (int ks = 0; ks < KS; ++ks)
+#pragma unroll
+        for (int e = 0; e < 8; ++e) xr[t][ks][e] = (xr[t][ks][e] - mean) * rstd;
+    }
+#pragma unroll
+    for (int ks = 0; ks < KS; ++ks) {
+      const float4 g0 = *reinterpret_cast<const float4*>(p.gamma + 16 * ks + 8 * lh);
+      const float4 g1 = *reinterpret_cast<const float4*>(p.gamma + 16 * ks + 8 * lh + 4);
+      const float4 c0 = *reinterpret_cast<const float4*>(p.beta + 16 * ks + 8 * lh);
+      const float4 c1 = *reinterpret_cast<const float4*>(p.beta + 16 * ks + 8 * lh + 4);
+      const float g8[8] = {g0.x, g0.y, g0.z, g0.w, g1.x, g1.y, g1.z, g1.w};
+      const float c8[8] = {c0.x, c0.y, c0.z, c0.w, c1.x, c1.y, c1.z, c1.w};
+#pragma unroll
+      for (int t = 0; t < TM; ++t)
+#pragma unroll
+        for (int e = 0; e < 8; ++e) xr[t][ks][e] = fmaf(xr[t][ks][e], g8[e], c8[e]);
+    }
+  }
+  v8h xh[TM][KS], xl[TM][KS];
+#pragma unroll
+  for (int t = 0; t < TM; ++t)
+#pragma unroll
+    for (int ks = 0; ks < KS; ++ks)
+#pragma unroll
+      for (int e = 0; e < 8; ++e) {
+        _Float16 h, l;
+        split_f16(xr[t][ks][e], h, l);
+        xh[t][ks][e] = h; xl[t][ks][e] = l;
+      }
+
+  v16f o[TM][CT];
+#pragma unroll
+  for (int t = 0; t < TM; ++t)
+#pragma unroll
+    for (int ct = 0; ct < CT; ++ct)
+#pragma unroll
+      for (int i = 0; i < 16; ++i) o[t][ct][i] = 0.f;
+
+  auto phase1 = [&](const unsigned char* w1, v16f (&h)[TM]) {
+#pragma unroll
+    for (int t = 0; t < TM; ++t)
+#pragma unroll
+      for (int i = 0; i < 16; ++i) h[t][i] = 0.f;
+#pragma unroll
+    for (int ks = 0; ks < KS; ++ks) {
+      const v8h wh = *reinterpret_cast<const v8h*>(w1 + (ks * 2 + 0) * 1024);
+      const v8h wl = *reinterpret_cast<const v8h*>(w1 + (ks * 2 + 1) * 1024);
+#pragma unroll
+      for (int t = 0; t < TM; ++t) {
+        if (!kSingleProduct) {
+          h[t] = __builtin_amdgcn_mfma_f32_32x32x16_f16(wl, xh[t][ks], h[t], 0, 0, 0);
+          h[t] = __builtin_amdgcn_mfma_f32_32x32x16_f16(wh, xl[t][ks], h[t], 0, 0, 0);
+        }
+        h[t] = __builtin_amdgcn_mfma_f32_32x32x16_f16(wh, xh[t][ks], h[t], 0, 0, 0);
+      }
+    }
+  };
+  v16f h[TM], hn[TM];
+  v8h hh[TM][2], hl[TM][2], gh[TM][2], gl[TM][2];
+  auto body = [&](auto has_p2, auto has_p1, int j, const unsigned char* st) {
+    constexpr bool P2 = decltype(has_p2)::value, P1 = decltype(has_p1)::value;
+    constexpr int T0 = P2 ? 0 : 2 * CT, T1 = P1 ? 2 * CT + KS : 2 * CT, NTR = T1 - T0;
+    auto frag = [&](int tr, int plane) {
+      const unsigned char* base = tr < 2 * CT ? st + W1B + (tr * 2) * 1024 : st + ((tr - 2 * CT) * 2) * 1024;
+      return *reinterpret_cast<const v8h*>(base + plane * 1024);
+    };
+    float bv[16];
+#pragma unroll
+    for (int q = 0; q < 4; ++q) {
+      const float4 b = *reinterpret_cast<const float4*>(b1s + j * 32 + q * 8 + 4 * lh);
+      bv[q * 4 + 0] = b.x; bv[q * 4 + 1] = b.y; bv[q * 4 + 2] = b.z; bv[q * 4 + 3] = b.w;
+    }
+    v8h wh, wl, nh, nl;
+    if (NTR > 0) { wh = frag(T0, 0); wl = frag(T0, 1); }
+#pragma unroll
+    for (int g = 0; g < 16; ++g) {
+#pragma unroll
+      for (int tr = T0 + g * NTR / 16; tr < T0 + (g + 1) * NTR / 16; ++tr) {
+        if (tr + 1 < T1) { nh = frag(tr + 1, 0); nl = frag(tr + 1, 1); }
+        __builtin_amdgcn_sched_barrier(0);
+#pragma unroll
+        for (int t = 0; t < TM; ++t) {
+          if (tr < 2 * CT) {
+            const int s = tr / CT, ct = tr % CT;
+            if (!kSingleProduct) {
+              o[t][ct] = __builtin_amdgcn_mfma_f32_32x32x16_f16(wl, hh[t][s], o[t][ct], 0, 0, 0);
+              o[t][ct] = __builtin_amdgcn_mfma_f32_32x32x16_f16(wh, hl[t][s], o[t][ct], 0, 0, 0);
+            }
+            o[t][ct] = __builtin_amdgcn_mfma_f32_32x32x16_f16(wh, hh[t][s], o[t][ct], 0, 0, 0);
+          } else {
+            const int ks = tr - 2 * CT;
+            const v16f zero = {0.f, 0.f, 0.f, 0.f, 0.f, 0.f, 0.f, 0.f, 0.f, 0.f, 0.f, 0.f, 0.f, 0.f, 0.f, 0.f};
+            if (!kSingleProduct) {
+              hn[t] = __builtin_amdgcn_mfma_f32_32x32x16_f16(wl, xh[t][ks], ks == 0 ? zero : hn[t], 0, 0, 0);
+              hn[t] = __builtin_amdgcn_mfma_f32_32x32x16_f16(wh, xl[t][ks], hn[t], 0, 0, 0);
+              hn[t] = __builtin_amdgcn_mfma_f32_32x32x16_f16(wh, xh[t][ks], hn[t], 0, 0, 0);
+            } else {
+              hn[t] = __builtin_amdgcn_mfma_f32_32x32x16_f16(wh, xh[t][ks], ks == 0 ? zero : hn[t], 0, 0, 0);
+            }
+          }
+        }
+        wh = nh; wl = nl;
+      }
+#pragma unroll
+      for (int t = 0; t < TM; ++t) {
+        const float u = fmaf(h[t][g], p.inv_s1, bv[g]);
+        const float v = gelu_erf(u);
+        _Float16 f, l;
+        split_f16(v, f, l);
+        gh[t][g >> 3][g & 7] = f;
+        gl[t][g >> 3][g & 7] = l;
+      }
+      __builtin_amdgcn_sched_barrier(0);
+    }
+#pragma unroll
+    for (int t = 0; t < TM; ++t) {
+      if (P1) h[t] = hn[t];
+#pragma unroll
+      for (int s = 0; s < 2; ++s) { hh[t][s] = gh[t][s]; hl[t][s] = gl[t][s]; }
+    }
+  };
+  using yes = std::true_type;
+  using no = std::false_type;
+
+  asm volatile("s_waitcnt vmcnt(%0)" ::"n"((NS - 1) * DPW) : "memory");
+  asm volatile("s_waitcnt lgkmcnt(0)" ::: "memory");
+  __builtin_amdgcn_s_barrier();
+  phase1(smem + (NS - 1) * SB + lane * 16, h);
+  if (p.nch > 1) body(no(), yes(), 0, smem + (NS - 1) * SB + W1B + lane * 16);
+  else body(no(), no(), 0, smem + lane * 16);
+
+  auto top = [&](int j) {
+    if (j + NS - 3 < p.nch) asm volatile("s_waitcnt vmcnt(%0)" ::"n"((NS - 2) * DPW) : "memory");
+    else asm volatile("s_waitcnt vmcnt(0)" ::: "memory");
+    asm volatile("s_waitcnt lgkmcnt(0)" ::: "memory");
+    __builtin_amdgcn_s_barrier();
+    if (j + NS - 2 < p.nch) issue_stage(j + NS - 2);
+  };
+  int j = 1;
+  for (; j + 1 < p.nch; ++j) {
+    top(j);
+    body(yes(), yes(), j, smem + ((j - 1) % NS) * SB + lane * 16);
+  }
+  if (j < p.nch) {
+    top(j);
+    body(yes(), no(), j, smem + ((j - 1) % NS) * SB + lane * 16);
+    ++j;
+  }
+  top(j);
+  {
+    const unsigned char* w2 = smem + ((j - 1) % NS) * SB + lane * 16 + W1B;
+#pragma unroll
+    for (int s = 0; s < 2; ++s)
+#pragma unroll
+      for (int ct = 0; ct < CT; ++ct) {
+        const v8h wh = *reinterpret_cast<const v8h*>(w2 + ((s * CT + ct) * 2 + 0) * 1024);
+        const v8h wl = *reinterpret_cast<const v8h*>(w2 + ((s * CT + ct) * 2 + 1) * 1024);
+#pragma unroll
+        for (int t = 0; t < TM; ++t) {
+          if (!kSingleProduct) {
+            o[t][ct] = __builtin_amdgcn_mfma_f32_32x32x16_f16(wl, hh[t][s], o[t][ct], 0, 0, 0);
+            o[t][ct] = __builtin_amdgcn_mfma_f32_32x32x16_f16(wh, hl[t][s], o[t][ct], 0, 0, 0);
+          }
+          o[t][ct] = __builtin_amdgcn_mfma_f32_32x32x16_f16(wh, hh[t][s], o[t][ct], 0, 0, 0);
+        }
+      }
+  }
+
+  bool bad = false;
+#pragma unroll
+  for (int t = 0; t < TM; ++t) {
+    const long row = row0 + t * 32 + li;
+    const bool ok = row < p.M;
+    const long rr = ok ? row : 0;
+#pragma unroll
+    for (int ct = 0; ct < CT; ++ct) {
+      float4 rv[4];
+#pragma unroll
+      for (int q = 0; q < 4; ++q) {
+        const int c = ct * 32 + q * 8 + 4 * lh;
+        rv[q] = p.res ? *reinterpret_cast<const float4*>(p.res + rr * p.ldr + c) : make_float4(0.f, 0.f, 0.f, 0.f);
+      }
+#pragma unroll
+      for (int q = 0; q < 4; ++q) {
+        const int c = ct * 32 + q * 8 + 4 * lh;
+        const float4 b = *reinterpret_cast<const float4*>(p.b2 + c);
+        float4 v;
+        v.x = fmaf(o[t][ct][q * 4 + 0], p.inv_s2, b.x) + rv[q].x;
+        v.y = fmaf(o[t][ct][q * 4 + 1], p.inv_s2, b.y) + rv[q].y;
+        v.z = fmaf(o[t][ct][q * 4 + 2], p.inv_s2, b.z) + rv[q].z;
+        v.w = fmaf(o[t][ct][q * 4 + 3], p.inv_s2, b.w) + rv[q].w;
+        bad |= nonfinite(v.x) | nonfinite(v.y) | nonfinite(v.z) | nonfinite(v.w);
+        if (ok && (!LN2 || p.y)) *reinterpret_cast<float4*>(p.y + row * p.ldy + c) = v;
+        if (LN2) { o[t][ct][q * 4 + 0] = v.x; o[t][ct][q * 4 + 1] = v.y; o[t][ct][q * 4 + 2] = v.z; o[t][ct][q * 4 + 3] = v.w; }
+      }
+    }
+    if (LN2) {
+      auto fold = [&](auto term) {
+        float pm[8];
+#pragma unroll
+        for (int m = 0; m < 8; ++m) {
+          pm[m] = 0.f;
+#pragma unroll
+          for (int jj = 0; 2 * jj + m / 4 < CT; ++jj) pm[m] += term(2 * jj + m / 4, m % 4);
+        }
+        const float a0 = pm[0] + pm[4], a1 = pm[1] + pm[5], a2 = pm[2] + pm[6], a3 = pm[3] + pm[7];
+        const float b0 = a0 + a2, b1 = a1 + a3;
+        float r = b0 + b1;
+        r += __shfl_xor(r, 32, 64);
+        return r;
+      };
+      const float s = fold([&](int ct, int q) {
+        return (o[t][ct][q * 4 + 0] + o[t][ct][q * 4 + 1]) + (o[t][ct][q * 4 + 2] + o[t][ct][q * 4 + 3]);
+      });
+      const float mean = s / (float)C;
+      const float q2 = fold([&](int ct, int q) {
+        const float a = o[t][ct][q * 4 + 0] - mean, b = o[t][ct][q * 4 + 1] - mean, c = o[t][ct][q * 4 + 2] - mean,
+                    d = o[t][ct][q * 4 + 3] - mean;
+        return (a * a + b * b) + (c * c + d * d);
+      });
+      const float rstd = rsqrtf(q2 / (float)C + p.eps2);
+#pragma unroll
+      for (int ct = 0; ct < CT; ++ct)
+#pragma unroll
+        for (int q = 0; q < 4; ++q) {
+          const int c = ct * 32 + q * 8 + 4 * lh;
+          const float4 g = *reinterpret_cast<const float4*>(p.gamma2 + c);
+          const float4 b = *reinterpret_cast<const float4*>(p.beta2 + c);
+          float4 v;
+          v.x = (o[t][ct][q * 4 + 0] - mean) * rstd * g.x + b.x;
+          v.y = (o[t][ct][q * 4 + 1] - mean) * rstd * g.y + b.y;
+          v.z = (o[t][ct][q * 4 + 2] - mean) * rstd * g.z + b.z;
+          v.w = (o[t][ct][q * 4 + 3] - mean) * rstd * g.w + b.w;
+          if (ok) *reinterpret_cast<float4*>(p.y_ln + row * p.ldn + c) = v;
+        }
+    }
+  }
+  report_nonfinite(p.status, bad);
+}
+
+template <int C, int TM, int NS, int NWV = 4, bool LN2 = false>
+static int launch_mlp(const MlpArgs& a, hipStream_t s) {
+  constexpr int BM = 32 * NWV * TM;
+  const long nb = (a.M + BM - 1) / BM;
+  hipLaunchKernelGGL((mlp_fused_kernel<C, TM, NS, NWV, LN2>), dim3((unsigned)nb), dim3(64 * NWV), 0, s, a);
+  return 0;
+}
+
+}
diff --git a/mspi_amd/engine.py b/mspi_amd/engine.py
--- a/mspi_amd/engine.py
+++ b/mspi_amd/engine.py
@@ -20,7 +20,7 @@
            "layernorm_bwd", "dwconv_wgrad", "conv_wgrad_entry", "conv_wgrad_entry_variant", "conv_wgrad_t16",
            "conv_wgrad_t16_variant", "attention_bwd", "layernorm_bwd_wide", "linear_wgrad",
            "linear_wgrad_variant", "neg_cosine_bwd", "layernorm_act_bwd", "mean_rows_bwd", "dwconv3_wgrad", "bn_gate_act",
-           "gate_swish_bwd", "se_train_fwd", "se_train_bwd", "relu_mask_add", "ACT_NONE", "ACT_RELU", "ACT_GELU", "ACT_SIGMOID", "ACT_SWISH"]
+           "gate_swish_bwd", "se_train_fwd", "se_train_bwd", "relu_mask_add", "mlp_ln", "ACT_NONE", "ACT_RELU", "ACT_GELU", "ACT_SIGMOID", "ACT_SWISH"]
 
 
 AUTOTUNE = {"on": _os.environ.get("MSPI_AUTOTUNE", "0") == "1", "cache": {}, "reps": 3}
@@ -790,6 +790,36 @@
     return out
 
 
+def mlp_ln(x, pk, ln, ln2, res=None, want_y=True, eps=1e-6, eps2=1e-6):
+    lib = _lib.load()
+    _need_gpu(x.buf)
+    if pk.fallback is not None or (not pk.checked and _tuning()):
+        y = mlp(x, pk, res=res, ln=ln, eps=eps)
+        return (y if want_y else None), layernorm(y, ln2[0], ln2[1], eps2)
+    if x.C != pk.c or not x.dense:
+        raise MspiError("mlp_ln: input has %d channels (dense=%s), packed for %d" % (x.C, x.dense, pk.c))
+    if pk.w.device != x.buf.device:
+        raise MspiError("mlp_ln: packed weights live on %s, the input on %s" % (pk.w.device, x.buf.device))
+    if pk.act != ACT_GELU:
+        raise MspiError("mlp_ln: packed with activation %d, the seam kernel has GELU" % pk.act)
+    if res is not None and (res.M != x.M or not res.dense):
+        raise MspiError("mlp_ln: residual rows %d != rows %d (or residual not dense)" % (res.M, x.M))
+    y = alloc(x.N, x.T, x.H, x.W, pk.c, x.buf.device) if want_y else None
+    y_ln = alloc(x.N, x.T, x.H, x.W, pk.c, x.buf.device)
+    d = _lib.CnxMlpLnDesc()
+    d.M, d.C, d.hidden = x.M, pk.c, pk.hidden
+    d.ldx, d.ldr, d.ldy, d.ldn = x.ld, (res.ld if res is not None else 0), (y.ld if want_y else 0), y_ln.ld
+    d.ln, d.eps, d.eps2 = (1 if ln is not None else 0), eps, eps2
+    d.w1_scale, d.w2_scale = pk.s1, pk.s2
+    with _Timed("mlp_ln_fused", 4.0 * x.M * pk.c * pk.hidden, 4.0 * x.M * pk.c * (2 + (res is not None) + bool(want_y)),
+                "M=%d C=%d hidden=%d y=%d" % (x.M, pk.c, pk.hidden, bool(want_y))):
+        check(lib.mspi_cnx_mlp_ln_fwd(C.byref(d), x.ptr, ln[0].data_ptr() if ln is not None else None,
+                                      ln[1].data_ptr() if ln is not None else None, pk.w.data_ptr(), pk.b1.data_ptr(),
+                                      pk.b2.data_ptr(), res.ptr if res is not None else None, ln2[0].data_ptr(), ln2[1].data_ptr(),
+                                      y.ptr if want_y else None, y_ln.ptr, _stream()), "mspi_cnx_mlp_ln_fwd")
+    return y, y_ln
+
+
 def layernorm_for_gemm(x, gamma, beta, eps, *packs):
     if sp_supported(x.C) and x.C >= 256 and all(p.k == (1, 1, 1) and p.stride == (1, 1, 1) and p.ldw == x.C and p.prec == PREC_F16X3
                                                  for p in packs):
diff --git a/mspi_amd/model/model_utils.py b/mspi_amd/model/model_utils.py
--- a/mspi_amd/model/model_utils.py
+++ b/mspi_amd/model/model_utils.py
@@ -294,7 +294,7 @@
 
     def run(self, clips):
         s0, s1 = self.pk
-        _, _, o1, o0 = self.encoder.forward_cl(clips)
+        _, _, o1, o0 = self.encoder.forward_cl(clips, need=(False, False, True, True))
         return E.conv(o1, s1), E.conv(o0, s0)
 
     def forward(self, x):
```

Measured after the change: 693.3 clips/s, median of 6. Within noise of the previous version (+0.5%).
